# NilanEkanayake/TiTok-Video

Hardware: AMD Instinct MI355X
Metric: video clips/sec encode+decode (whole node) (higher is better)
Workload: dtype bf16

## Files before the change

include/titok_hip.h:

```cpp
#ifndef TITOK_HIP_H
#define TITOK_HIP_H

#include <stdint.h>

#ifdef __cplusplus
extern "C" {
#endif

#define TTV_OK 0
#define TTV_ERR_INVALID 1
#define TTV_ERR_LAUNCH 2
#define TTV_ERR_UNSUPPORTED 3

#define TTV_BF16 0
#define TTV_F32 1

#define TTV_ENCODER 0
#define TTV_DECODER 1

#define TTV_MAX_FSQ 8
#define TTV_MAX_TOKEN 64
#define TTV_MAX_CLIPS_PER_LAUNCH 64

const char* ttv_error_string(void);
// ... 143 lines not shown
typedef struct ttv_tower_weights {
  const void* proj_in_w;
  const void* proj_in_b;
  const float* mask_token;
  const float* ln_pre_t;
  const float* ln_pre_p;
  const float* ln_post;
  const void* proj_out_w;
  const void* proj_out_b;
  const ttv_layer_weights* layers;
  const void* proj_out_pn;
  int32_t f32_split3;
} ttv_tower_weights;

typedef struct ttv_batch {
  int32_t n_clips;
  int32_t total_rows;
  int32_t sum_tokens;
  int32_t sum_patches;
  int32_t max_patches_per_clip;
  int32_t n_qblocks;
  const int32_t* cu_seqlens;
  const int32_t* latent_rows;
  const int32_t* patch_rows;
  const int32_t* clip_desc;
  const int32_t* qblocks;
  const float* rope_cs;
  const int32_t* blocks64;
  const int32_t* row_seq;
  int32_t n_blocks64;
  int32_t qblocks_paired;
  int32_t qblocks_all_full;
  const int32_t* items64;
  int32_t n_items64;
  const int32_t* rope_ids;
  const float* rope_base;
  const int32_t* qblocks_latent;
  int32_t n_qblocks_latent;
  const int32_t* qblocks_patch;
  int32_t n_qblocks_patch;
} ttv_batch;

int ttv_rope_table_build(const float* base_cos, const float* base_sin, int n_ids, int n_freqs, const int32_t* clip_desc,
                         const int32_t* cu_seqlens, const int32_t* row_seq, float* rope_cs, int total_rows, void* stream);

int64_t ttv_tower_workspace_bytes(const ttv_tower_dims* dims, const ttv_batch* batch);

int ttv_encoder_forward(const ttv_tower_dims* dims, const ttv_tower_weights* w, const ttv_batch* batch,
                        const void* const* clips, const ttv_fsq_params* fsq, float* z, void* codes, int32_t* indices,
                        float* bounded, void* workspace, int64_t workspace_bytes, void* stream);

int ttv_decoder_forward(const ttv_tower_dims* dims, const ttv_tower_weights* w, const ttv_batch* batch, const void* codes,
                        void* const* clips_out, void* workspace, int64_t workspace_bytes, void* stream);

typedef struct ttv_layer_weights_t {
  const void* to_qkv_t;
  const void* out_proj_t;
  const void* w12_t;
  const void* w3_t;
} ttv_layer_weights_t;
typedef struct ttv_tower_weights_t {
  const void* proj_in_t;
  const void* proj_out_t;
  const ttv_layer_weights_t* layers;
} ttv_tower_weights_t;
typedef struct ttv_layer_grads {
  float* pre_ln; float* to_qkv; float* out_proj; float* ffd_norm; float* w12; float* w3; float* attn_post_ln; float* ffd_post_ln;
} ttv_layer_grads;
typedef struct ttv_tower_grads {
  float* proj_in_w; float* proj_in_b; float* mask_token; float* ln_pre_t; float* ln_pre_p; float* ln_post; float* proj_out_w;
  float* proj_out_b;
  const ttv_layer_grads* layers;
  void** layer_done_events;
} ttv_tower_grads;

int64_t ttv_tower_tape_bytes(const ttv_tower_dims* dims, const ttv_batch* batch);
int64_t ttv_tower_bwd_workspace_bytes(const ttv_tower_dims* dims, const ttv_batch* batch);
int ttv_encoder_forward_train(const ttv_tower_dims* dims, const ttv_tower_weights* w, const ttv_batch* batch, const void* const* clips,
                              float* z, void* tape, int64_t tape_bytes, void* stream);
int ttv_encoder_backward(const ttv_tower_dims* dims, const ttv_tower_weights* w, const ttv_tower_weights_t* wt, const ttv_batch* batch,
                         const float* dz, void* tape, const ttv_tower_grads* grads, void* const* dclips, void* workspace,
                         int64_t workspace_bytes, void* stream);
int ttv_decoder_forward_train(const ttv_tower_dims* dims, const ttv_tower_weights* w, const ttv_batch* batch, const void* codes,
                              void* const* clips_out, void* tape, int64_t tape_bytes, void* workspace, int64_t workspace_bytes,
                              void* stream);
int ttv_decoder_backward(const ttv_tower_dims* dims, const ttv_tower_weights* w, const ttv_tower_weights_t* wt, const ttv_batch* batch,
                         const void* codes, const void* const* dclips_out, void* tape, const ttv_tower_grads* grads, float* dcodes,
                         void* workspace, int64_t workspace_bytes, void* stream);
int ttv_fsq_backward(const ttv_fsq_params* p, const float* z, const void* dcodes, int dcodes_dtype, float* dz, int rows, void* stream);

int ttv_opt_grad_sumsq(const void* table, const int32_t* chunks, int n_chunks, int dtype, float* partials, void* stream);
int ttv_opt_adamw_step(const void* table, const int32_t* chunks, int n_chunks, int dtype, const float* partials, int n_partials, float lr,
                       float beta1, float beta2, float one_minus_beta1, float one_minus_beta2, float eps, float weight_decay,
                       float bias_correction1, float bias_correction2_sqrt, float max_norm, float* out_norm, void* stream);

int ttv_opt_param_norms(const void* table, const int32_t* chunks, int n_chunks, int n_entries, const float* partials, float* norms,
                        void* stream);

int ttv_opt_ema_update(const void* table, const int32_t* chunks, int n_chunks, int dtype, float weight, void* stream);
int ttv_opt_ema_exchange(const void* table, const int32_t* chunks, int n_chunks, int dtype, int mode, void* stream);

int64_t ttv_linear_wgrad_workspace_bytes(int L, int N, int K);
int ttv_linear_wgrad(const void* dy, int lddy, const void* x, int ldx, float* dw, int lddw, int L, int N, int K, int dtype,
                     void* workspace, int64_t workspace_bytes, void* stream);
int ttv_rmsnorm_backward_chain(const void* x, int ldx, const void* dy, int lddy, const float* gain1, float* dgain1, float* dx, int lddx,
                               const float* y, int ldy, const float* gain2, float* dgain2, float out_scale, void* cast_out, int ldc, int rows,
// ... 109 lines not shown
  const void* pool_proj_w; const void* pool_proj_b;
  const float* pool_norm2_w; const float* pool_norm2_b;
  const void* pool_fc1_w; const void* pool_fc1_b;
  const void* pool_fc2_w; const void* pool_fc2_b;
} ttv_vjepa_weights;

int ttv_jedi_preprocess(void* const* clips, const int32_t* dims, int n_clips, int dtype, void* out, void* stream);
int64_t ttv_vjepa_workspace_bytes(int n);
int ttv_vjepa_features(const ttv_vjepa_weights* w, const void* x, int n, float* feats, int finetuned, void* workspace,
                       int64_t workspace_bytes, void* stream);

#define TTV_VJEPA_EPI_STORE 0
#define TTV_VJEPA_EPI_GELU 1
#define TTV_VJEPA_EPI_RESID 2
int ttv_vjepa_layernorm(const float* x, int ldx, int rows, int width, const float* w1, const float* b1, float eps1, const float* w2,
                        const float* b2, float eps2, float* y32, int ld32, void* y16, int ld16, void* stream);
int ttv_vjepa_linear(const void* x, int ldx, const void* w, int ldw, const void* bias, int M, int N, int K, int epilogue,
                     const float* resid, int ldr, int resid_rows, void* y, int ldy, void* stream);
int ttv_vjepa_pool_attention(const void* q, const void* kv, int n, int rows, void* out, void* stream);

#define TTV_KC_ATTENTION 1
#define TTV_KC_GEMM_QKV 2
#define TTV_KC_GEMM_GEGLU 3
#define TTV_KC_GEMM_RESID 4
#define TTV_KC_GEMM_STORE 5
#define TTV_KC_RMSNORM 6
#define TTV_KC_PATCH 7
#define TTV_KC_ROWS 8
int ttv_prof_begin(int kernel_class, int max_records);
enum {
  TTV_DBG_NO_STORES = 1,
  TTV_DBG_K256_NO_PANEL_DMA = 2,
  TTV_DBG_MLP_NO_WEIGHT_DMA = 2,
  TTV_DBG_K256_NO_TILE_RELOAD = 4,
  TTV_DBG_MLP_NO_GEGLU = 4,
  TTV_DBG_K256_NO_EPILOGUE_MATH = 8,
  TTV_DBG_MLP_TILES8 = 8,
  TTV_DBG_MLP_NO_P2 = 16,
  TTV_DBG_MLP_PAIRS_ONLY = 32,
  TTV_DBG_MLP_TILES4 = 64,
  TTV_DBG_GEMM_TILE160 = 128,
  TTV_DBG_GEMM_TILE128 = 256,
  TTV_DBG_GEMM_T256 = 512,
  TTV_DBG_MLP_TILES9 = 512,
  TTV_DBG_GEMM_NO_T256 = 1024,
  TTV_DBG_MX_UNFUSED_QUANT = 2048,
  TTV_DBG_SPLIT3_NO_IMAGES = 4096,
  TTV_DBG_SPLIT3_NO_DMA = 8192,
  TTV_DBG_K256_GENERAL = 16384,
  TTV_DBG_QKV256_OFF = 32768,
  TTV_DBG_QKV256_WS = 131072,
  TTV_DBG_ENC_ALL_ROWS = 524288,
  TTV_DBG_ATTN_NO_SWP = 1048576,
  TTV_DBG_DEC_ALL_BLOCKS = 2097152
};
int ttv_debug_set(int flags);
int ttv_debug_stamps(void* device_buffer);
int ttv_prof_end(double* total_ms, int* count);

#ifdef __cplusplus
}
#endif
#endif
```

titok_video_amd/_lib.py:

```python
from __future__ import annotations

import ctypes as C
import os
import threading

import torch

from . import switches

TTV_BF16, TTV_F32 = 0, 1
TTV_ENCODER, TTV_DECODER = 0, 1
TTV_MAX_FSQ = 8
TTV_MAX_TOKEN = 64
TTV_MAX_CLIPS_PER_LAUNCH = 64
TTV_DISC_HEAD_GENERATOR, TTV_DISC_HEAD_DISCRIMINATOR = 0, 1

DBG_NO_STORES = 1
DBG_K256_NO_PANEL_DMA = 2
DBG_MLP_NO_WEIGHT_DMA = 2
DBG_K256_NO_TILE_RELOAD = 4
DBG_MLP_NO_GEGLU = 4
DBG_K256_NO_EPILOGUE_MATH = 8
DBG_MLP_TILES8 = 8
DBG_MLP_NO_P2 = 16
DBG_MLP_PAIRS_ONLY = 32
DBG_MLP_TILES4 = 64
DBG_GEMM_TILE160 = 128
DBG_GEMM_TILE128 = 256
DBG_GEMM_T256 = 512
DBG_MLP_TILES9 = 512
DBG_GEMM_NO_T256 = 1024
DBG_MX_UNFUSED_QUANT = 2048
DBG_SPLIT3_NO_IMAGES = 4096
DBG_SPLIT3_NO_DMA = 8192
DBG_K256_GENERAL = 16384
DBG_QKV256_OFF = 32768
DBG_QKV256_WS = 131072
DBG_ENC_ALL_ROWS = 524288
DBG_ATTN_NO_SWP = 1048576
DBG_DEC_ALL_BLOCKS = 2097152

_HERE = os.path.dirname(os.path.abspath(__file__))
LIB_PATH = switches.text("TTV_LIB_PATH") or os.path.join(_HERE, "libtitok_hip.so")

i32, i64, f32, vp = C.c_int32, C.c_int64, C.c_float, C.c_void_p


class FsqParams(C.Structure):
    _fields_ = [("n", i32), ("levels", i32 * TTV_MAX_FSQ), ("basis", i32 * TTV_MAX_FSQ),
                ("half_l", f32 * TTV_MAX_FSQ), ("offset", f32 * TTV_MAX_FSQ), ("shift", f32 * TTV_MAX_FSQ),
                ("half_width", f32 * TTV_MAX_FSQ)]


class TowerDims(C.Structure):
    _fields_ = [("kind", i32), ("dtype", i32), ("width", i32), ("layers", i32), ("q_heads", i32), ("kv_heads", i32),
                ("head_dim", i32), ("inner", i32), ("patch_t", i32), ("patch_h", i32), ("patch_w", i32),
                ("pix_channels", i32), ("token_size", i32), ("eps", f32), ("alpha", f32)]


class NextQkv(C.Structure):
    _fields_ = [("qkv", vp), ("ld", i32), ("rope_cs", vp), ("rows", i32), ("rope_q_end", i32), ("rope_k_begin", i32), ("rope_k_end", i32)]


class LayerWeights(C.Structure):
    _fields_ = [("pre_ln", vp), ("to_qkv", vp), ("out_proj", vp), ("ffd_norm", vp), ("w12", vp), ("w3", vp),
                ("attn_post_ln", vp), ("ffd_post_ln", vp), ("to_qkv_pn", vp), ("w12_pn", vp), ("mlp_pack", vp), ("mlp_pack_qkv_rows", i32), ("qkv_q_prescaled", i32),
                ("to_qkv_qs", vp), ("to_qkv_f8", vp), ("to_qkv_f8_scale", vp), ("w12_f8", vp), ("w12_f8_scale", vp),
                ("to_qkv_mx", vp), ("w12_mx", vp), ("out_proj_f8", vp), ("out_proj_f8_scale", vp), ("out_proj_mx", vp),
                ("w3_f8", vp), ("w3_f8_scale", vp), ("w3_mx", vp)]


class TowerWeights(C.Structure):
    _fields_ = [("proj_in_w", vp), ("proj_in_b", vp), ("mask_token", vp), ("ln_pre_t", vp), ("ln_pre_p", vp),
                ("ln_post", vp), ("proj_out_w", vp), ("proj_out_b", vp), ("layers", C.POINTER(LayerWeights)), ("proj_out_pn", vp),
                ("f32_split3", i32)]


class Batch(C.Structure):
    _fields_ = [("n_clips", i32), ("total_rows", i32), ("sum_tokens", i32), ("sum_patches", i32),
                ("max_patches_per_clip", i32), ("n_qblocks", i32), ("cu_seqlens", vp), ("latent_rows", vp),
                ("patch_rows", vp), ("clip_desc", vp), ("qblocks", vp), ("rope_cs", vp), ("blocks64", vp), ("row_seq", vp),
                ("n_blocks64", i32), ("qblocks_paired", i32), ("qblocks_all_full", i32), ("items64", vp), ("n_items64", i32),
                ("rope_ids", vp), ("rope_base", vp), ("qblocks_latent", vp), ("n_qblocks_latent", i32), ("qblocks_patch", vp),
                ("n_qblocks_patch", i32)]


class LayerWeightsT(C.Structure):
    _fields_ = [("to_qkv_t", vp), ("out_proj_t", vp), ("w12_t", vp), ("w3_t", vp)]


class TowerWeightsT(C.Structure):
    _fields_ = [("proj_in_t", vp), ("proj_out_t", vp), ("layers", C.POINTER(LayerWeightsT))]


class LayerGrads(C.Structure):
    _fields_ = [("pre_ln", vp), ("to_qkv", vp), ("out_proj", vp), ("ffd_norm", vp), ("w12", vp), ("w3", vp),
                ("attn_post_ln", vp), ("ffd_post_ln", vp)]


class TowerGrads(C.Structure):
    _fields_ = [("proj_in_w", vp), ("proj_in_b", vp), ("mask_token", vp), ("ln_pre_t", vp), ("ln_pre_p", vp), ("ln_post", vp),
                ("proj_out_w", vp), ("proj_out_b", vp), ("layers", C.POINTER(LayerGrads)), ("layer_done_events", C.POINTER(vp))]


class LpipsWeights(C.Structure):
    _fields_ = [("w", vp * 13), ("wd", vp * 13), ("b", vp * 13), ("lin", vp * 5)]


TTV_I3D_CONVS = 58
TTV_I3D_FEATURES = 400


class I3dWeights(C.Structure):
    _fields_ = [("w", vp * TTV_I3D_CONVS), ("scale", vp * TTV_I3D_CONVS), ("shift", vp * TTV_I3D_CONVS)]


TTV_VJEPA_WIDTH = 1024
TTV_VJEPA_TOKENS = 1568
TTV_VJEPA_PATCH_K = 1536
TTV_VJEPA_EPI_STORE, TTV_VJEPA_EPI_GELU, TTV_VJEPA_EPI_RESID = 0, 1, 2


class VjepaLayer(C.Structure):
    _fields_ = [("norm1_w", vp), ("norm1_b", vp), ("qkv_w", vp), ("qkv_b", vp), ("proj_w", vp), ("proj_b", vp), ("norm2_w", vp),
                ("norm2_b", vp), ("fc1_w", vp), ("fc1_b", vp), ("fc2_w", vp), ("fc2_b", vp)]


class VjepaWeights(C.Structure):
    _fields_ = [("width", i32), ("heads", i32), ("depth", i32), ("patch_w", vp), ("patch_b", vp), ("pos_embed", vp),
                ("layers", C.POINTER(VjepaLayer)), ("norm_w", vp), ("norm_b", vp), ("query_tokens", vp), ("pool_q", vp),
                ("pool_norm1_w", vp), ("pool_norm1_b", vp), ("pool_kv_w", vp), ("pool_kv_b", vp), ("pool_proj_w", vp),
                ("pool_proj_b", vp), ("pool_norm2_w", vp), ("pool_norm2_b", vp), ("pool_fc1_w", vp), ("pool_fc1_b", vp),
                ("pool_fc2_w", vp), ("pool_fc2_b", vp)]


_lib = None
_lock = threading.Lock()

SYMBOLS = {
    "ttv_error_string": (C.c_char_p, []),
    "ttv_version": (C.c_int, []),
    "ttv_fsq_forward": (C.c_int, [C.POINTER(FsqParams), vp, C.c_int, C.c_int, vp, C.c_int, vp, vp, vp]),
    "ttv_fsq_indices_to_codes": (C.c_int, [C.POINTER(FsqParams), vp, C.c_int, vp, C.c_int, vp]),
    "ttv_vq_codebook_norms": (C.c_int, [vp, C.c_int, C.c_int, C.c_int, C.c_int, vp, vp]),
    "ttv_vq_workspace_bytes": (C.c_int64, [C.c_int]),
    "ttv_vq_l2_argmin": (C.c_int, [vp, C.c_int, C.c_int, vp, C.c_int, vp, C.c_int, C.c_int, C.c_int, vp, vp, vp, C.c_int64, vp]),
    "ttv_vq_lookup": (C.c_int, [vp, C.c_int, C.c_int, vp, C.c_int, C.c_int, vp, C.c_int, vp]),
    "ttv_vq_lookup_backward": (C.c_int, [vp, C.c_int, C.c_int, vp, C.c_int, C.c_int, vp, C.c_int, vp]),
    "ttv_vq_train_workspace_bytes": (C.c_int64, [C.c_int, C.c_int]),
    "ttv_vq_commit_forward": (C.c_int, [vp, C.c_int, C.c_int, vp, C.c_int, vp, C.c_int, C.c_int, C.c_int, vp, vp, C.c_int64, vp]),
    "ttv_vq_commit_backward": (C.c_int, [vp, C.c_int, vp, C.c_int, vp, C.c_int, C.c_int, C.c_int, C.c_int, C.c_double, vp, C.c_int, vp]),
    "ttv_vq_ema_stats": (C.c_int, [vp, C.c_int, C.c_int, vp, C.c_int, C.c_int, C.c_int, vp, f32, C.c_uint64, vp, C.c_int, C.c_int, vp, vp, C.c_int64, vp]),
    "ttv_vq_ema_update": (C.c_int, [vp, vp, vp, vp, vp, C.c_int, vp, vp, C.c_int, C.c_int, f32, f32, f32, f32, vp, C.c_int64, vp]),
    "ttv_quant_rows_fp8": (C.c_int, [vp, C.c_int, C.c_int, vp, f32, vp, C.c_int, vp, C.c_int, C.c_int, vp]),
    "ttv_linear_fp8": (C.c_int, [vp, C.c_int, vp, vp, C.c_int, vp, vp, C.c_int, C.c_int, C.c_int, C.c_int, C.c_int, vp, C.c_int, C.c_int, vp]),
    "ttv_split3_pack": (C.c_int, [vp, C.c_int, vp, C.c_int, C.c_int, C.c_int, vp]),
    "ttv_linear_split3": (C.c_int, [vp, C.c_int, vp, C.c_int, vp, vp, C.c_int, C.c_int, C.c_int, C.c_int, vp]),
    "ttv_mx_scale_bytes_per_row": (C.c_int64, [C.c_int]),
    "ttv_quant_mx_fp8": (C.c_int, [vp, C.c_int, C.c_int, vp, C.c_int, vp, vp, C.c_int, C.c_int, vp]),
    "ttv_linear_fp8_mx": (C.c_int, [vp, C.c_int, vp, vp, vp, C.c_int, vp, vp, vp, C.c_int, C.c_int, C.c_int, C.c_int, C.c_int, vp, C.c_int, C.c_int,
                                    vp, C.c_int, f32, vp]),
    "ttv_rmsnorm": (C.c_int, [vp, C.c_int, C.c_int, vp, vp, C.c_int, C.c_int, vp, vp, C.c_int, C.c_int, f32, vp]),
    "ttv_rope_apply": (C.c_int, [vp, C.c_int, C.c_int, C.c_int, C.c_int, vp, vp]),
    "ttv_linear": (C.c_int, [vp, C.c_int, vp, C.c_int, vp, vp, vp, C.c_int, C.c_int, C.c_int, C.c_int, C.c_int, vp]),
    "ttv_linear_qkv_rope": (C.c_int, [vp, C.c_int, vp, C.c_int, vp, C.c_int, C.c_int, C.c_int, C.c_int, vp, C.c_int, vp]),
    "ttv_linear_geglu": (C.c_int, [vp, C.c_int, vp, C.c_int, vp, C.c_int, C.c_int, C.c_int, C.c_int, C.c_int, vp]),
    "ttv_linear_residual": (C.c_int, [vp, C.c_int, vp, C.c_int, vp, C.c_int, f32, vp, C.c_int, C.c_int, C.c_int, C.c_int,
                                      C.c_int, C.c_int, vp]),
    "ttv_linear_residual_norm": (C.c_int, [vp, C.c_int, vp, C.c_int, vp, C.c_int, f32, vp, f32, vp, C.c_int, C.c_int, C.c_int,
                                           C.c_int, C.c_int, vp]),
    "ttv_mlp_pack_bytes": (C.c_int64, [C.c_int, C.c_int]),
    "ttv_mlp_pack": (C.c_int, [vp, vp, vp, vp, C.c_int, C.c_int, C.c_int, C.c_int, vp, vp]),
    "ttv_layer_tail_fused": (C.c_int, [vp, C.c_int, vp, f32, vp, C.c_int, vp, C.c_int, vp, C.c_int, vp, f32, f32, C.c_int, C.c_int,
                                       C.c_int, vp, vp]),
    "ttv_mlp_fused": (C.c_int, [vp, C.c_int, vp, C.c_int, vp, C.c_int, vp, f32, f32, C.c_int, C.c_int, C.c_int, vp]),
    "ttv_fill_const_rows": (C.c_int, [vp, C.c_int, C.c_int, vp, C.c_int, C.c_int, vp, vp, f32, vp]),
    "ttv_decoder_embed": (C.c_int, [vp, C.c_int, vp, vp, vp, vp, vp, C.c_int, C.c_int, vp, C.c_int, C.c_int, f32, vp]),
    "ttv_attention": (C.c_int, [vp, C.c_int, vp, C.c_int, vp, vp, C.c_int, C.c_int, C.c_int, C.c_int, C.c_int, C.c_int, vp]),
    "ttv_attention64": (C.c_int, [vp, C.c_int, vp, C.c_int, vp, vp, C.c_int, C.c_int, C.c_int, C.c_int, C.c_int, C.c_int, vp]),
    "ttv_patch_gather": (C.c_int, [C.POINTER(vp), vp, C.c_int, C.c_int, C.c_int, C.c_int, C.c_int, C.c_int, vp, C.c_int,
                                   C.c_int, C.c_int, vp]),
    "ttv_patch_scatter": (C.c_int, [vp, C.c_int, vp, C.c_int, C.c_int, C.c_int, C.c_int, C.c_int, C.c_int, C.POINTER(vp),
                                    C.c_int, C.c_int, vp]),
    "ttv_tower_workspace_bytes": (i64, [C.POINTER(TowerDims), C.POINTER(Batch)]),
    "ttv_encoder_forward": (C.c_int, [C.POINTER(TowerDims), C.POINTER(TowerWeights), C.POINTER(Batch), C.POINTER(vp),
                                      C.POINTER(FsqParams), vp, vp, vp, vp, vp, i64, vp]),
    "ttv_decoder_forward": (C.c_int, [C.POINTER(TowerDims), C.POINTER(TowerWeights), C.POINTER(Batch), vp, C.POINTER(vp),
                                      vp, i64, vp]),
    "ttv_tower_tape_bytes": (i64, [C.POINTER(TowerDims), C.POINTER(Batch)]),
    "ttv_tower_bwd_workspace_bytes": (i64, [C.POINTER(TowerDims), C.POINTER(Batch)]),
    "ttv_encoder_forward_train": (C.c_int, [C.POINTER(TowerDims), C.POINTER(TowerWeights), C.POINTER(Batch), C.POINTER(vp), vp, vp,
                                            i64, vp]),
    "ttv_encoder_backward": (C.c_int, [C.POINTER(TowerDims), C.POINTER(TowerWeights), C.POINTER(TowerWeightsT), C.POINTER(Batch), vp,
                                       vp, C.POINTER(TowerGrads), C.POINTER(vp), vp, i64, vp]),
    "ttv_decoder_forward_train": (C.c_int, [C.POINTER(TowerDims), C.POINTER(TowerWeights), C.POINTER(Batch), vp, C.POINTER(vp), vp,
                                            i64, vp, i64, vp]),
    "ttv_decoder_backward": (C.c_int, [C.POINTER(TowerDims), C.POINTER(TowerWeights), C.POINTER(TowerWeightsT), C.POINTER(Batch), vp,
                                       C.POINTER(vp), vp, C.POINTER(TowerGrads), vp, vp, i64, vp]),
    "ttv_fsq_backward": (C.c_int, [C.POINTER(FsqParams), vp, vp, C.c_int, vp, C.c_int, vp]),
    "ttv_rmsnorm_backward_chain": (C.c_int, [vp, C.c_int, vp, C.c_int, vp, vp, vp, C.c_int, vp, C.c_int, vp, vp, C.c_float, vp, C.c_int,
                                              C.c_int, C.c_int, C.c_float, C.c_int, vp]),
    "ttv_opt_grad_sumsq": (C.c_int, [vp, vp, C.c_int, C.c_int, vp, vp]),
    "ttv_opt_adamw_step": (C.c_int, [vp, vp, C.c_int, C.c_int, vp, C.c_int] + [C.c_float] * 10 + [vp, vp]),
    "ttv_opt_param_norms": (C.c_int, [vp, vp, C.c_int, C.c_int, vp, vp, vp]),
    "ttv_opt_ema_update": (C.c_int, [vp, vp, C.c_int, C.c_int, C.c_float, vp]),
    "ttv_opt_ema_exchange": (C.c_int, [vp, vp, C.c_int, C.c_int, C.c_int, vp]),
    "ttv_linear_wgrad_workspace_bytes": (C.c_int64, [C.c_int, C.c_int, C.c_int]),
    "ttv_linear_wgrad": (C.c_int, [vp, C.c_int, vp, C.c_int, vp, C.c_int, C.c_int, C.c_int, C.c_int, C.c_int, vp, C.c_int64, vp]),
    "ttv_rmsnorm_backward": (C.c_int, [vp, C.c_int, vp, C.c_int, vp, vp, C.c_int, vp, C.c_int, C.c_int, f32, C.c_int, vp]),
    "ttv_attention_backward": (C.c_int, [vp, C.c_int, vp, C.c_int, vp, C.c_int, vp, vp, vp, vp, C.c_int, vp, vp, C.c_int, vp, C.c_int,
                                         C.c_int, C.c_int, C.c_int, vp, vp]),
    "ttv_attention_lse": (C.c_int, [vp, C.c_int, vp, C.c_int, vp, vp, C.c_int, C.c_int, C.c_int, C.c_int, C.c_int, C.c_int, vp, vp]),
    "ttv_codebook_histogram": (C.c_int, [vp, C.c_int, vp, C.c_int, vp]),
    "ttv_rope_table_build": (C.c_int, [vp, vp, C.c_int, C.c_int, vp, vp, vp, vp, C.c_int, vp]),
    "ttv_l1_loss": (C.c_int, [vp, vp, vp, vp, C.c_int, C.c_int, vp, vp]),
    "ttv_clip_from_u8": (C.c_int, [vp, C.c_int, C.c_int, C.c_int, vp, C.c_int, vp]),
    "ttv_clip_resample_u8": (C.c_int, [vp, vp, vp, C.c_int, C.c_int, vp]),
    "ttv_recon_panels_u8": (C.c_int, [vp, vp, vp, C.c_int, C.c_int, vp, vp]),
    "ttv_sq_err_accumulate": (C.c_int, [vp, vp, vp, C.c_int, C.c_int, C.c_int, vp, vp]),
    "ttv_ssim_workspace_bytes": (C.c_int64, [vp, C.c_int]),
    "ttv_ssim_accumulate": (C.c_int, [vp, vp, vp, C.c_int, C.c_int, C.c_int, vp, vp, C.c_int64, vp]),
    "ttv_lpips_tape_bytes": (C.c_int64, [C.c_int, C.c_int, C.c_int, C.c_int]),
    "ttv_lpips_workspace_bytes": (C.c_int64, [C.c_int, C.c_int, C.c_int, C.c_int]),
    "ttv_lpips_forward": (C.c_int, [C.POINTER(LpipsWeights), vp, vp, C.c_int, C.c_int, C.c_int, C.c_int, vp, vp, vp, vp, C.c_int64, vp]),
    "ttv_lpips_backward": (C.c_int, [C.POINTER(LpipsWeights), vp, C.c_int, C.c_int, C.c_int, C.c_int, vp, vp, vp, vp, C.c_int64, vp]),
    "ttv_lpips_eval_workspace_bytes": (C.c_int64, [C.c_int, C.c_int, C.c_int, C.c_int]),
    "ttv_lpips_eval_accumulate": (C.c_int, [C.POINTER(LpipsWeights), vp, vp, vp, C.c_int, C.c_int, C.c_int, C.c_int, C.c_int, vp, vp, vp,
                                            C.c_int64, vp]),
    "ttv_lpips_conv_workspace_bytes": (C.c_int64, [C.c_int] * 6),
    "ttv_lpips_conv3x3": (C.c_int, [vp, C.c_int, C.c_int, C.c_int, C.c_int, C.c_int, vp, vp, C.c_int, vp, vp, C.c_int, vp, C.c_int64, vp]),
    "ttv_lpips_maxpool": (C.c_int, [vp, C.c_int, C.c_int, C.c_int, C.c_int, vp, C.c_int, vp]),
    "ttv_lpips_maxpool_backward": (C.c_int, [vp, vp, vp, C.c_int, C.c_int, C.c_int, C.c_int, vp, C.c_int, vp]),
    "ttv_lpips_crops_forward": (C.c_int, [vp, vp, vp, C.c_int, vp, C.c_int, C.c_int, vp, vp, C.c_int, vp]),
    "ttv_lpips_crops_backward": (C.c_int, [vp, vp, vp, C.c_int, vp, C.c_int, C.c_int, vp, C.c_int, vp]),
    "ttv_gp_noise_add": (C.c_int, [vp, C.c_int, vp, C.c_int, C.c_int, C.c_uint64, C.c_uint64, f32, C.c_int, vp]),
    "ttv_disc_head": (C.c_int, [vp, vp, C.c_int, C.c_int, C.c_int, C.c_int, C.c_int, f32, f32, vp, vp, vp]),
    "ttv_i3d_workspace_bytes": (C.c_int64, [C.c_int]),
    "ttv_fvd_preprocess": (C.c_int, [vp, vp, C.c_int, C.c_int, C.c_int, vp, vp]),
    "ttv_i3d_features": (C.c_int, [C.POINTER(I3dWeights), vp, C.c_int, vp, vp, C.c_int64, vp]),
    "ttv_i3d_conv3d": (C.c_int, [vp] + [C.c_int] * 7 + [vp, vp, vp, C.c_int, C.c_int, vp, C.c_int, C.c_int, vp]),
    "ttv_i3d_maxpool3d": (C.c_int, [vp] + [C.c_int] * 11 + [vp, vp]),
# ... 66 lines not shown
```

titok_video_amd/csrc/ttv_api.hip:

```cpp
#include <stdarg.h>
#include <stdio.h>
#include <stdlib.h>
#include <string.h>

#include "ttv_common.h"
#include "ttv_kernels.h"

static thread_local char g_err[512] = "";

void ttv_set_error(const char* fmt, ...) {
  va_list ap;
  va_start(ap, fmt);
  vsnprintf(g_err, sizeof(g_err), fmt, ap);
  va_end(ap);
}

int g_ttv_prof_class = 0;
bool ttv_sw_enc_latent_last() { static const bool v = ttv_env_flag("TTV_ENC_LATENT_LAST", true); return v; }
bool ttv_enc_latent_rows_only(const ttv_tower_dims* d, const ttv_batch* b) {
  return ttv_sw_enc_latent_last() && !(g_ttv_debug & TTV_DBG_ENC_ALL_ROWS) && d->kind == TTV_ENCODER && b->latent_rows && b->sum_tokens > 0 &&
         b->sum_tokens < b->total_rows;
}
bool ttv_sw_keel_f32sum() { static const bool v = ttv_env_flag("TTV_KEEL_F32SUM", false); return v; }
bool ttv_sw_fused_patch() { static const bool v = ttv_env_flag("TTV_FUSED_PATCH", true); return v; }
bool ttv_sw_attn_pipe() { static const bool v = ttv_env_flag("TTV_ATTN_PIPE", false); return v; }
float ttv_sw_attn_thr() { static const float v = ttv_env_float("TTV_ATTN_THR", 8.0f); return v; }
thread_local int g_ttv_debug = 0;
long long* g_ttv_stamps = nullptr;
static hipEvent_t* g_prof_start = nullptr;
static hipEvent_t* g_prof_stop = nullptr;
static int g_prof_cap = 0, g_prof_n = 0;

TtvProfScope::TtvProfScope(int cls, hipStream_t stream) : slot(-1), s(stream) {
  if (g_ttv_prof_class != 0 && cls == g_ttv_prof_class && g_prof_n < g_prof_cap) {
    slot = g_prof_n++;
    (void)hipEventRecord(g_prof_start[slot], s);
  }
}
TtvProfScope::~TtvProfScope() {
  if (slot >= 0) (void)hipEventRecord(g_prof_stop[slot], s);
}

struct TowerWs {
  char *x, *xn, *qkv, *ao, *h, *pa, *pb;
  char *xl, *aol;
  char *f8, *f8mx;
  float* y32;
  float* rstd;
  int64_t total;
};

static TowerWs carve(const ttv_tower_dims* d, const ttv_batch* b, char* base) {
  const int64_t e = dtype_bytes(d->dtype);
  const int64_t L = b->total_rows, P = b->sum_patches;
  const int64_t g = (int64_t)d->kv_heads * d->head_dim;
  const int64_t pd = patch_dim(d);
  int64_t off = 0;
  TowerWs w;
  auto take = [&](int64_t bytes) { char* p = base ? base + off : nullptr; off += align256(bytes); return p; };
  w.x = take(L * d->width * e);
  w.xn = take(L * d->width * e);
  w.qkv = take(L * (2 * d->width + 2 * g) * e);
  w.ao = take(L * d->width * e);
  w.y32 = (float*)take(L * d->width * 4);
  w.h = take(L * d->inner * e);
  w.pa = take(P * pd * e);
  w.pb = take(P * d->width * e);
  w.rstd = (float*)take(L * 4);
  w.xl = take((int64_t)b->sum_tokens * d->width * e);
  w.aol = take((int64_t)b->sum_tokens * d->width * e);
  w.f8 = w.f8mx = nullptr;
  if (d->dtype == TTV_BF16 && d->width != 256 && d->width % 128 == 0) {
    const int64_t wide = d->width > d->inner ? d->width : d->inner;
    w.f8 = take(L * wide);
    w.f8mx = take(L * (wide / 128 + 4) * 4);
  }
  w.total = off;
  return w;
// ... 34 lines not shown
  const int L = b->total_rows, dm = d->width, g = d->kv_heads * d->head_dim, dt = d->dtype, nq = 2 * dm + 2 * g, I = d->inner;
  const float alpha = keel_alpha(d, i);
  static const bool fused_env = ttv_env_flag("TTV_MX_FUSED_QUANT", true);
  const bool fused_q = fused_env && !(g_ttv_debug & TTV_DBG_MX_UNFUSED_QUANT);
  if (!rstd_valid) TTV_TRY(ttvk_row_rstd(ws.x, dt, dm, ws.rstd, L, dm, d->eps, s));
  if (!xq_valid) TTV_TRY(ttvk_quant_mx_fp8(ws.x, dt, dm, ws.f8, dm, ws.f8mx, nullptr, L, dm, s));
  xq_valid = false;
  const GemmArgs a = gemm_rope_qk(gemm_args(dt, ws.f8, dm, lw.to_qkv_f8, dm, L, nq, dm, ws.qkv, nq), b->rope_cs, dm, g);
  TTV_TRY(ttvk_gemm_fp8(EPI_QKV_ROPE, a, ws.rstd, lw.to_qkv_f8_scale, s, ws.f8mx, lw.to_qkv_mx));
  const bool q_scaled = lw.qkv_q_prescaled != 0;
  if (fused_q && q_scaled && !c.pair && !c.pipe && d->head_dim == 64) {
    TTV_TRY(ttvk_attention_mxout(ws.qkv, nq, ws.f8, ws.f8mx, (int)ttvk_mx_scale_ld(dm), b->cu_seqlens, b->qblocks, b->n_qblocks, d->q_heads,
                                 d->kv_heads, s));
  } else {
    TTV_TRY(tower_attention(c, q_scaled, b->qblocks, b->n_qblocks, c.pair | (c.pipe ? c.all_full | c.pipe : 0)));
    TTV_TRY(ttvk_quant_mx_fp8(ws.ao, dt, dm, ws.f8, dm, ws.f8mx, nullptr, L, dm, s));
  }
  const GemmArgs o = gemm_resid(gemm_args(dt, ws.f8, dm, lw.out_proj_f8, dm, L, dm, dm, ws.x, dm), ws.x, dm, alpha);
  TTV_TRY(ttvk_gemm_fp8(EPI_RESID_T, o, nullptr, lw.out_proj_f8_scale, s, ws.f8mx, lw.out_proj_mx));
  if (i > 0) {
    TTV_TRY(ttvk_rmsnorm(ws.x, dt, dm, nullptr, ws.x, dt, dm, nullptr, lw.attn_post_ln, L, dm, d->eps, s, ws.rstd, fused_q ? ws.f8 : nullptr,
                         fused_q ? ws.f8mx : nullptr));
    if (!fused_q) TTV_TRY(ttvk_quant_mx_fp8(ws.x, dt, dm, ws.f8, dm, ws.f8mx, nullptr, L, dm, s));
  } else {
    TTV_TRY(ttvk_row_rstd(ws.x, dt, dm, ws.rstd, L, dm, d->eps, s));
    TTV_TRY(ttvk_quant_mx_fp8(ws.x, dt, dm, ws.f8, dm, ws.f8mx, nullptr, L, dm, s));
  }
  GemmArgs f = gemm_args(dt, ws.f8, dm, lw.w12_f8, dm, L, I, dm, ws.h, I);
  char* const hq = ws.h;
  char* const hq_mx = ws.xn;
  const bool h_fused = fused_q && (int64_t)ttvk_mx_scale_ld(I) <= (int64_t)dm * 2;
  if (h_fused) { f.yq = hq; f.yq_mx = hq_mx; }
  TTV_TRY(ttvk_gemm_fp8(EPI_GEGLU, f, ws.rstd, lw.w12_f8_scale, s, ws.f8mx, lw.w12_mx));
  if (!h_fused) TTV_TRY(ttvk_quant_mx_fp8(ws.h, dt, I, ws.f8, I, ws.f8mx, nullptr, L, I, s));
  const GemmArgs f3 = gemm_resid(gemm_args(dt, h_fused ? hq : ws.f8, I, lw.w3_f8, I, L, dm, I, ws.x, dm), ws.x, dm, alpha);
  TTV_TRY(ttvk_gemm_fp8(EPI_RESID_T, f3, nullptr, lw.w3_f8_scale, s, h_fused ? hq_mx : ws.f8mx, lw.w3_mx));
  rstd_valid = false;
  if (i > 0) {
    TTV_TRY(ttvk_rmsnorm(ws.x, dt, dm, nullptr, ws.x, dt, dm, nullptr, lw.ffd_post_ln, L, dm, d->eps, s, ws.rstd, fused_q ? ws.f8 : nullptr,
                         fused_q ? ws.f8mx : nullptr));
    rstd_valid = true;
    xq_valid = fused_q;
  }
  return TTV_OK;
}

static bool rows_f8(int dt, int dm, const void* img, const void* row_scale, const void* mx, const void* folded) {
  return dt == TTV_BF16 && img && row_scale && !mx && dm % 128 == 0 && !(dm == 256 && folded);
}

struct PreNormW { const float* gain; const void *w, *w_pn, *w_f8; const float* w_f8_scale; bool f8; };

static int prenorm_proj(const LayerCtx& c, GemmEpilogue epi, const char* x, int rows, const PreNormW& p, int N, char* y, int y_image,
                        bool rstd_valid) {
  const ttv_tower_dims* d = c.d;
  const TowerWs& ws = c.ws;
  const int dm = d->width, dt = d->dtype;
  GemmArgs a = gemm_args(dt, nullptr, dm, nullptr, dm, rows, N, dm, y, N);
  if (epi == EPI_QKV_ROPE) a = gemm_rope_qk(a, c.b->rope_cs, dm, d->kv_heads * d->head_dim);
  if (p.f8) {
    float* const f8_scales = reinterpret_cast<float*>(ws.xn + align256((int64_t)c.b->total_rows * dm));
    TTV_TRY(ttvk_quant_rows_fp8(x, dt, dm, p.gain, d->eps, ws.xn, dm, f8_scales, rows, dm, c.s));
    a.x = ws.xn; a.w = p.w_f8;
    return ttvk_gemm_fp8(epi, a, f8_scales, p.w_f8_scale, c.s);
  }
  const bool fold256 = dt == TTV_BF16 && dm == 256 && p.w_pn;
  const bool fold_gen = c.gen_ok && p.w_pn;
  const bool fold = fold256 || fold_gen;
  if (fold_gen && !rstd_valid) TTV_TRY(ttvk_row_rstd(x, dt, dm, ws.rstd, rows, dm, d->eps, c.s));
  if (!fold) TTV_TRY(ttvk_rmsnorm(x, dt, dm, nullptr, ws.xn, dt, dm, nullptr, p.gain, rows, dm, d->eps, c.s, nullptr, nullptr, nullptr, c.s3img));
  a.split3 = c.split3; a.x_image = c.s3img && !fold; a.y_image = y_image;
  a.prenorm = fold256; a.eps = d->eps;
  a.row_scale = fold_gen ? ws.rstd : nullptr;
  a.x = fold ? x : ws.xn; a.w = fold ? p.w_pn : p.w;
  if (epi == EPI_QKV_ROPE) { a.rope_ids = c.b->rope_ids; a.rope_base = c.b->rope_ids ? c.b->rope_base : nullptr; }
  return ttvk_gemm(epi, a, c.s);
}

static int keel_tail(const LayerCtx& c, GemmArgs o, int layer, const float* post_gain, bool want_rstd, bool& rstd_valid) {
  const ttv_tower_dims* d = c.d;
  const int dm = d->width, dt = d->dtype;
  char* const cx = (char*)o.y;
  o = gemm_resid(o, cx, dm, keel_alpha(d, layer));
  o.split3 = c.split3; o.x_image = c.s3img;
  if (layer == 0) return ttvk_gemm(EPI_RESID_T, o, c.s);
  if (ttvk_gemm_supports_resid_norm(dt, dm, o.K)) {
    o.norm_gain = post_gain; o.eps = d->eps;
    return ttvk_gemm(EPI_RESID_NORM, o, c.s);
  }
  float* const next_rstd = want_rstd ? c.ws.rstd : nullptr;
  if (dt == TTV_BF16 && !ttv_sw_keel_f32sum()) {
    TTV_TRY(ttvk_gemm(EPI_RESID_T, o, c.s));
    TTV_TRY(ttvk_rmsnorm(cx, dt, dm, nullptr, cx, dt, dm, nullptr, post_gain, o.M, dm, d->eps, c.s, next_rstd));
  } else {
    o.y = c.ws.y32;
    TTV_TRY(ttvk_gemm(EPI_RESID_F32, o, c.s));
    TTV_TRY(ttvk_rmsnorm(c.ws.y32, TTV_F32, dm, nullptr, cx, dt, dm, nullptr, post_gain, o.M, dm, d->eps, c.s, next_rstd));
  }
  rstd_valid = want_rstd;
  return TTV_OK;
}

static int run_layers(const ttv_tower_dims* d, const ttv_tower_weights* w, const ttv_batch* b, const TowerWs& ws, hipStream_t s) {
  const int L = b->total_rows, dm = d->width, g = d->kv_heads * d->head_dim, dt = d->dtype;
  const int split3 = (dt == TTV_F32 && w->f32_split3) ? 1 : 0;
  const bool gen_ok = (dt == TTV_BF16 && dm != 256) || split3;
  static const bool s3img_env = ttv_env_flag("TTV_SPLIT3_IMAGES", true);
  const int s3img = (split3 && s3img_env && !(g_ttv_debug & TTV_DBG_SPLIT3_NO_IMAGES)) ? 1 : 0;
  const int nq = 2 * dm + 2 * g;
  const int64_t row_bytes = (int64_t)dm * dtype_bytes(dt);
  bool qkv_ready = false;
  bool rstd_valid = false;
  bool xq_valid = false;
  const bool lat_last = ttv_enc_latent_rows_only(d, b) && b->qblocks_latent && b->n_qblocks_latent > 0;
  static const bool pat_env = ttv_env_flag("TTV_DEC_PATCH_LAST", true);
  const bool pat_last = pat_env && !(g_ttv_debug & TTV_DBG_DEC_ALL_BLOCKS) && d->kind == TTV_DECODER && d->layers >= 2 && b->qblocks_patch &&
                        b->n_qblocks_patch > 0 && !split3 && !b->qblocks_paired;
  bool compacted = false;
  const LayerCtx ctx = {d, b, ws, s, split3, s3img, gen_ok, b->qblocks_paired ? TTV_ATTN_PAIRED : 0, b->qblocks_all_full ? TTV_ATTN_ALLFULL : 0,
                        ttv_sw_attn_pipe() ? TTV_ATTN_PIPE : 0};
  for (int i = 0; i < d->layers; ++i) {
    const ttv_layer_weights& lw = w->layers[i];
    const bool last = i == d->layers - 1;
    if (dt == TTV_BF16 && dm != 256 && dm % 128 == 0 && d->inner % 128 == 0 && !ttv_sw_keel_f32sum() && lw.to_qkv_f8 && lw.to_qkv_mx && lw.w12_f8 &&
        lw.w12_mx && lw.out_proj_f8 && lw.out_proj_mx && lw.w3_f8 && lw.w3_mx &&
        !(lat_last && last)) {
      TTV_TRY(run_layer_mx(ctx, lw, i, rstd_valid, xq_valid));
      qkv_ready = false;
      continue;
    }
    xq_valid = false;
    const bool f8_qkv = rows_f8(dt, dm, lw.to_qkv_f8, lw.to_qkv_f8_scale, lw.to_qkv_mx, lw.to_qkv_pn);
    const bool f8_w12 = rows_f8(dt, dm, lw.w12_f8, lw.w12_f8_scale, lw.w12_mx, lw.w12_pn);
    if (!qkv_ready) {
      const void* w_plain = (dt == TTV_BF16 && lw.to_qkv_qs) ? lw.to_qkv_qs : lw.to_qkv;
      const PreNormW qw = {lw.pre_ln, w_plain, lw.to_qkv_pn, lw.to_qkv_f8, lw.to_qkv_f8_scale, f8_qkv};
      TTV_TRY(prenorm_proj(ctx, EPI_QKV_ROPE, ws.x, L, qw, nq, ws.qkv, s3img ? 2 : 0, rstd_valid));
    }
    const bool q_scaled = dt == TTV_BF16 && (lw.to_qkv_pn ? lw.qkv_q_prescaled != 0 : lw.to_qkv_qs != nullptr);
    rstd_valid = false;
    qkv_ready = false;
    const bool lat_now = lat_last && last;
    if (lat_now)
      TTV_TRY(tower_attention(ctx, q_scaled, b->qblocks_latent, b->n_qblocks_latent, ctx.all_full));
    else if (pat_last && last && dt == TTV_BF16 && !ctx.pipe)
      TTV_TRY(tower_attention(ctx, q_scaled, b->qblocks_patch, b->n_qblocks_patch, ctx.all_full));
    else if (q_scaled && b->items64 && b->n_items64 > 0 && d->head_dim == 64)
      TTV_TRY(ttvk_attention64(ws.qkv, nq, ws.ao, dm, b->cu_seqlens, b->items64, b->n_items64, d->q_heads, d->kv_heads,
                               TTV_ATTN_GATE | TTV_ATTN_QSCALED, s));
    else
      TTV_TRY(tower_attention(ctx, q_scaled, b->qblocks, b->n_qblocks, ctx.pair | ctx.all_full | ctx.pipe));
    char* cx = ws.x;
    char* cao = ws.ao;
    int Lc = L;
    if (lat_now) {
      TTV_TRY(gather_rows(ws.x, ws.xl, b->latent_rows, b->sum_tokens, row_bytes, s));
      TTV_TRY(gather_rows(ws.ao, ws.aol, b->latent_rows, b->sum_tokens, row_bytes, s));
      cx = ws.xl; cao = ws.aol; Lc = b->sum_tokens;
      compacted = true;
    }
    static const bool use_fused_mlp = ttv_env_flag("TTV_FUSED_MLP", true);
    static const bool use_fused_qkv = ttv_env_flag("TTV_FUSED_QKV", false);
    const float alpha = keel_alpha(d, i);
    if (use_fused_mlp && ttvk_mlp_fused_supported(dt, dm, d->inner) && lw.mlp_pack) {
      MlpNextQkv nx = {};
      const bool back = use_fused_qkv && !last && lw.mlp_pack_qkv_rows == nq && nq % 64 == 0 && dm % 64 == 0 && g % 64 == 0;
      if (back) { nx.qkv = ws.qkv; nx.ld = nq; nx.rope_cs = b->rope_cs; nx.rows = nq; nx.rope_q_end = dm; nx.rope_k_begin = 2 * dm; nx.rope_k_end = 2 * dm + g; }
      TTV_TRY(ttvk_mlp_fused(cao, dm, i == 0 ? nullptr : lw.attn_post_ln, alpha, cx, dm, lw.mlp_pack, d->inner, cx, dm, i == 0 ? nullptr : lw.ffd_post_ln,
                             alpha, d->eps, Lc, back ? &nx : nullptr, s));
      qkv_ready = back;
      continue;
    }
    TTV_TRY(keel_tail(ctx, gemm_args(dt, cao, dm, lw.out_proj, dm, Lc, dm, dm, cx, dm), i, lw.attn_post_ln, gen_ok && lw.w12_pn && !f8_w12, rstd_valid));
    const PreNormW fw = {lw.ffd_norm, lw.w12, lw.w12_pn, lw.w12_f8, lw.w12_f8_scale, f8_w12};
    TTV_TRY(prenorm_proj(ctx, EPI_GEGLU, cx, Lc, fw, d->inner, ws.h, s3img, rstd_valid));
    rstd_valid = false;
    const ttv_layer_weights* nl = last ? nullptr : &w->layers[i + 1];
    const bool next_rstd = gen_ok && nl && nl->to_qkv_pn && !rows_f8(dt, dm, nl->to_qkv_f8, nl->to_qkv_f8_scale, nl->to_qkv_mx, nl->to_qkv_pn);
    TTV_TRY(keel_tail(ctx, gemm_args(dt, ws.h, d->inner, lw.w3, d->inner, Lc, dm, d->inner, cx, dm), i, lw.ffd_post_ln, next_rstd, rstd_valid));
  }
  if (compacted)
    TTV_TRY(scatter_rows(ws.xl, ws.x, b->latent_rows, b->sum_tokens, row_bytes, s));
  return TTV_OK;
}

static bool fused_patch_ok(const ttv_tower_dims* d, const ttv_batch* b, int dt) {
  auto pow2 = [](int v) { return v > 0 && (v & (v - 1)) == 0; };
  return ttv_sw_fused_patch() && dt == TTV_BF16 && d->patch_w == 8 && pow2(d->patch_t) && pow2(d->patch_h) &&
         b->n_clips <= TTV_MAX_CLIPS_PER_LAUNCH && b->row_seq && patch_dim(d) % 64 == 0;
}

extern "C" {

const char* ttv_error_string(void) { return g_err; }
int ttv_version(void) { return 100; }

int ttv_fsq_forward(const ttv_fsq_params* p, const void* z, int z_dtype, int rows, void* codes, int codes_dtype, int32_t* indices,
                    float* bounded, void* stream) {
// ... 225 lines not shown
  TTV_CHECK_ARG(dtype == TTV_BF16 && head_dim == 64, "attention64: bf16, head_dim 64 only");
  return ttvk_attention64(qkvg, ld, out, ldo, cu_seqlens, items, n_items, q_heads, kv_heads, flags, (hipStream_t)stream);
}

int ttv_patch_gather(const void* const* clips, const int32_t* clip_desc, int clip0, int n_clips, int patch_t, int patch_h, int patch_w,
                     int channels, void* patches, int ld, int dtype, int max_patches_per_clip, void* stream) {
  TTV_CHECK_ARG(n_clips == 0 || (clips && clip_desc && patches), "patch_gather: null buffer");
  return ttvk_patch_copy(false, (void* const*)clips, clip_desc, clip0, n_clips, patch_t, patch_h, patch_w, channels, patches, ld, dtype, max_patches_per_clip, (hipStream_t)stream);
}

int ttv_patch_scatter(const void* patches, int ld, const int32_t* clip_desc, int clip0, int n_clips, int patch_t, int patch_h, int patch_w,
                      int channels, void* const* clips, int dtype, int max_patches_per_clip, void* stream) {
  TTV_CHECK_ARG(n_clips == 0 || (clips && clip_desc && patches), "patch_scatter: null buffer");
  return ttvk_patch_copy(true, clips, clip_desc, clip0, n_clips, patch_t, patch_h, patch_w, channels, (void*)patches, ld, dtype, max_patches_per_clip, (hipStream_t)stream);
}

int64_t ttv_tower_workspace_bytes(const ttv_tower_dims* dims, const ttv_batch* batch) {
  if (check_dims(dims, batch) != TTV_OK) return -1;
  return carve(dims, batch, nullptr).total;
}

int ttv_encoder_forward(const ttv_tower_dims* d, const ttv_tower_weights* w, const ttv_batch* b, const void* const* clips,
                        const ttv_fsq_params* fsq, float* z, void* codes, int32_t* indices, float* bounded, void* workspace,
                        int64_t workspace_bytes, void* stream) {
  TTV_TRY(check_dims(d, b));
  TTV_CHECK_ARG(d->kind == TTV_ENCODER, "encoder_forward: dims.kind is not TTV_ENCODER");
  TTV_CHECK_ARG(w && w->layers && clips && workspace, "encoder_forward: null argument");
  TTV_CHECK_ARG(fsq || z, "encoder_forward: neither fsq nor z requested");
  TTV_CHECK_ARG(!fsq || (codes && indices), "encoder_forward: fsq needs codes and indices buffers");
  hipStream_t s = (hipStream_t)stream;
  TowerWs ws = carve(d, b, (char*)workspace);
  TTV_CHECK_ARG(ws.total <= workspace_bytes, "encoder_forward: workspace too small (%lld < %lld)", (long long)workspace_bytes, (long long)ws.total);
  const int dm = d->width, dt = d->dtype, P = b->sum_patches, pd = patch_dim(d);

  const bool gather = fused_patch_ok(d, b, dt) && pd != 256;
  if (!gather) TTV_TRY(patch_copy_all(false, (void* const*)clips, d, b, ws.pa, dt, s));
  GemmArgs a = gemm_args(dt, ws.pa, pd, w->proj_in_w, pd, P, dm, pd, ws.pb, dm);
  a.bias = w->proj_in_b; a.add_scalar = w->mask_token;
  a.split3 = (dt == TTV_F32 && w->f32_split3) ? 1 : 0;
  if (gather) {
    a.gather = 1; a.clips = (void* const*)clips; a.n_clips = b->n_clips; a.clip_desc = b->clip_desc; a.patch_rows = b->patch_rows;
    a.row_seq = b->row_seq; a.patch_t = d->patch_t; a.patch_h = d->patch_h; a.patch_w = d->patch_w;
  }
  TTV_TRY(ttvk_gemm(EPI_STORE, a, s));
  TTV_TRY(ttvk_rmsnorm(ws.pb, dt, dm, nullptr, ws.x, dt, dm, b->patch_rows, w->ln_pre_p, P, dm, d->eps, s));
  TTV_TRY(ttvk_fill_const_rows(ws.x, dt, dm, b->latent_rows, b->sum_tokens, dm, w->mask_token, w->ln_pre_t, d->eps, s));

  TTV_TRY(run_layers(d, w, b, ws, s));

  TTV_TRY(ttvk_enc_tail(ws.x, dt, dm, b->latent_rows, b->sum_tokens, dm, w->ln_post, d->eps, w->proj_out_w, w->proj_out_b, d->token_size, fsq, z, codes, indices, bounded, s));
  return TTV_OK;
}

int ttv_decoder_forward(const ttv_tower_dims* d, const ttv_tower_weights* w, const ttv_batch* b, const void* codes,
                        void* const* clips_out, void* workspace, int64_t workspace_bytes, void* stream) {
  TTV_TRY(check_dims(d, b));
  TTV_CHECK_ARG(d->kind == TTV_DECODER, "decoder_forward: dims.kind is not TTV_DECODER");
  TTV_CHECK_ARG(w && w->layers && codes && clips_out && workspace, "decoder_forward: null argument");
  hipStream_t s = (hipStream_t)stream;
  TowerWs ws = carve(d, b, (char*)workspace);
  TTV_CHECK_ARG(ws.total <= workspace_bytes, "decoder_forward: workspace too small (%lld < %lld)", (long long)workspace_bytes, (long long)ws.total);
  const int dm = d->width, dt = d->dtype, P = b->sum_patches, pd = patch_dim(d);

  TTV_TRY(ttvk_dec_embed(codes, d->token_size, w->proj_in_w, w->proj_in_b, w->mask_token, w->ln_pre_t, ws.x, dt, dm, b->latent_rows, b->sum_tokens, dm, d->eps, s));
  TTV_TRY(ttvk_fill_const_rows(ws.x, dt, dm, b->patch_rows, P, dm, w->mask_token, w->ln_pre_p, d->eps, s));

  TTV_TRY(run_layers(d, w, b, ws, s));

  GemmArgs a = gemm_args(dt, nullptr, dm, w->proj_out_w, dm, P, pd, dm, ws.pa, pd);
  a.split3 = (dt == TTV_F32 && w->f32_split3) ? 1 : 0;
  a.bias = w->proj_out_b;
  if (dt == TTV_BF16 && dm == 256 && w->proj_out_pn && pd % 8 == 0) {
    a.x = ws.x; a.x_rows = b->patch_rows; a.w = w->proj_out_pn; a.prenorm = 1; a.eps = d->eps;
  } else {
    TTV_TRY(ttvk_rmsnorm(ws.x, dt, dm, b->patch_rows, ws.pb, dt, dm, nullptr, w->ln_post, P, dm, d->eps, s));
    a.x = ws.pb;
  }
  if (fused_patch_ok(d, b, dt) && dm == 256) {
    a.clips = clips_out; a.n_clips = b->n_clips; a.clip_desc = b->clip_desc; a.patch_rows = b->patch_rows; a.row_seq = b->row_seq;
    a.patch_t = d->patch_t; a.patch_h = d->patch_h; a.patch_w = d->patch_w;
    return ttvk_gemm(EPI_STORE_PATCH, a, s);
  }
  TTV_TRY(ttvk_gemm(EPI_STORE, a, s));
  return patch_copy_all(true, clips_out, d, b, ws.pa, dt, s);
}

int ttv_rope_table_build(const float* base_cos, const float* base_sin, int n_ids, int n_freqs, const int32_t* clip_desc, const int32_t* cu_seqlens,
                         const int32_t* row_seq, float* rope_cs, int total_rows, void* stream) {
  TTV_CHECK_ARG(total_rows == 0 || (base_cos && base_sin && clip_desc && cu_seqlens && row_seq && rope_cs), "rope_table_build: null buffer");
  TTV_CHECK_ARG(n_freqs >= 1 && 3 * n_freqs <= 32 && n_ids >= 1, "rope_table_build: bad table shape");
  return ttvk_rope_build(base_cos, base_sin, n_ids, n_freqs, clip_desc, cu_seqlens, row_seq, rope_cs, total_rows, (hipStream_t)stream);
}

int ttv_l1_loss(void* const* recon, void* const* target, void* const* grad, const int32_t* sizes, int n_clips, int dtype, float* loss,
                void* stream) {
  return for_clip_groups(n_clips, [&](int c0, int n) {
    return ttvk_l1_loss(recon + c0, target + c0, grad ? grad + c0 : nullptr, sizes + c0, n, n_clips, dtype, loss, (hipStream_t)stream);
  });
}

int ttv_clip_from_u8(const void* frames_thwc, int T, int H, int W, void* clip_cthw, int dtype, void* stream) {
  TTV_CHECK_ARG(frames_thwc && clip_cthw && T > 0 && H > 0 && W > 0, "clip_from_u8: bad argument");
  return ttvk_clip_from_u8(frames_thwc, (long long)T * H * W, clip_cthw, dtype, (hipStream_t)stream);
}

int ttv_clip_resample_u8(void* const* frames_thwc, void* const* clips_cthw, const int32_t* geom, int n_clips, int dtype, void* stream) {
  return ttvk_clip_resample_u8(frames_thwc, clips_cthw, geom, n_clips, dtype, (hipStream_t)stream);
}

int ttv_sq_err_accumulate(void* const* recon, void* const* target, const int32_t* sizes, int n_clips, int dtype, int clamp, double* acc,
                          void* stream) {
  return for_clip_groups(n_clips, [&](int c0, int n) { return ttvk_sq_err(recon + c0, target + c0, sizes + c0, n, dtype, clamp, acc, (hipStream_t)stream); });
}

int64_t ttv_ssim_workspace_bytes(const int32_t* dims, int n_clips) { return ttvk_ssim_workspace_bytes(dims, n_clips); }

int ttv_ssim_accumulate(void* const* recon, void* const* target, const int32_t* dims, int n_clips, int dtype, int clamp, double* acc,
                        void* workspace, int64_t workspace_bytes, void* stream) {
  return ttvk_ssim(recon, target, dims, n_clips, dtype, clamp, acc, workspace, workspace_bytes, (hipStream_t)stream);
}
// ... 156 lines not shown
```

titok_video_amd/csrc/ttv_attn.hip:

```cpp
#include <stdlib.h>

#include "ttv_common.h"
#include "ttv_kernels.h"

#define QB 128
#define KB 64
#ifndef ATTN_LAZY
#define ATTN_LAZY 1
#endif
#ifndef ATTN_DMA_LATE
#define ATTN_DMA_LATE 1
#endif
#ifndef ATTN_PRIO
#define ATTN_PRIO 0
#endif
#define ATTN_LAZY_LOG2 30
#define ATTN_LAZY_BIG 1073741824.0f
typedef float f32x2 __attribute__((ext_vector_type(2)));

typedef __attribute__((address_space(3))) bf16x4 lds_bf16x4;

__device__ __forceinline__ bf16x4 lds_read_tr16(const char* lds_ptr) {
  return __builtin_amdgcn_ds_read_tr16_b64_v4bf16((lds_bf16x4*)(lds_ptr));
}
// ... 1293 lines not shown
      }
#undef S3_VFRAG
    }
  }
#undef S3_GLOAD
#undef S3_LSTORE
#undef S3_DMA_TILE
#undef S3_DMA
  if (!wave_live) return;

  const float l_tot = l_run + __shfl_xor(l_run, 32, 64);
  const float inv_l = 1.0f / l_tot;
  if (qrow < q_lim) {
    float* orow = out + (size_t)(s0 + qrow) * ldo + head * 64;
    const float* grow = gbase + (size_t)qrow * ld;
#pragma unroll
    for (int dt = 0; dt < 2; ++dt)
#pragma unroll
      for (int g = 0; g < 4; ++g) {
        const int d0 = dt * 32 + 8 * g + 4 * h;
        f32x4 v = {o_acc[dt][4 * g] * inv_l, o_acc[dt][4 * g + 1] * inv_l, o_acc[dt][4 * g + 2] * inv_l, o_acc[dt][4 * g + 3] * inv_l};
        if (GATE) {
          const f32x4 gt = *reinterpret_cast<const f32x4*>(grow + d0);
#pragma unroll
          for (int e = 0; e < 4; ++e) v[e] *= 1.0f / (1.0f + expf(-gt[e]));
        }
        if (out_image) {
          uint2 hi, lo;
          split4_f32(__builtin_bit_cast(uint4, v), hi, lo);
          *reinterpret_cast<uint4*>(orow + d0) = make_uint4(hi.x, hi.y, lo.x, lo.y);
        } else {
          *reinterpret_cast<f32x4*>(orow + d0) = v;
        }
      }
  }
}

int ttvk_attention_mxout(const void* qkvg, int ld, void* out_q, void* out_mx, int ld_mx, const int* cu_seqlens, const int* qblocks,
                         int n_qblocks, int q_heads, int kv_heads, hipStream_t s) {
  if (n_qblocks == 0) return TTV_OK;
  TTV_CHECK_ARG(kv_heads > 0 && q_heads % kv_heads == 0, "attention_mxout: q_heads %% kv_heads");
  const int d_model = q_heads * 64, gqa = kv_heads * 64, rep = q_heads / kv_heads;
  TTV_CHECK_ARG(ld >= 2 * d_model + 2 * gqa && ld % 8 == 0 && d_model % 128 == 0 && ld_mx == (int)(4 * ((d_model / 128 + 3) / 4 * 4)),
                "attention_mxout: bad leading dims (d_model %% 128, ld_mx = 4 * round_up(d_model / 128, 4))");
  TTV_CHECK_ARG(qkvg && out_q && out_mx && (uintptr_t)qkvg % 16 == 0 && (uintptr_t)out_q % 8 == 0, "attention_mxout: null / unaligned pointers");
  static const float defer_thr = ttv_sw_attn_thr();
  TtvProfScope prof(TTV_KC_ATTENTION, s);
  hipLaunchKernelGGL((k_attn_bf16<true, 1, true, false, true>), dim3(n_qblocks), dim3(256), 0, s, (const bf16_t*)qkvg, ld, (bf16_t*)nullptr, ld_mx,
                     cu_seqlens, qblocks, n_qblocks, d_model, gqa, rep, 1.0f, (float*)out_mx, (bf16_t*)out_q, defer_thr, g_ttv_stamps);
  TTV_CHECK_LAUNCH("attention_mxout");
  return TTV_OK;
}

int ttvk_attention(const void* qkvg, int ld, void* out, int ldo, const int* cu_seqlens, const int* qblocks, int n_qblocks,
                   int q_heads, int kv_heads, int head_dim, int flags, int dtype, hipStream_t s, float* lse_out, void* out_raw) {
  const int gate_mul = flags & 1, paired = (flags >> 1) & 1, prescaled = (flags >> 2) & 1;
  TTV_CHECK_ARG(!prescaled || dtype == TTV_BF16, "attention: pre-scaled q is a bf16 path option");
  TTV_CHECK_ARG(!out_raw || (dtype == TTV_BF16 && gate_mul), "attention: the second (ungated) output is a bf16 + gate option");
  if (n_qblocks == 0) return TTV_OK;
  TTV_CHECK_ARG(head_dim == 64, "attention: head_dim %d unsupported (the reference fixes 64, utils.py:8)", head_dim);
  TTV_CHECK_ARG(kv_heads > 0 && q_heads % kv_heads == 0, "attention: q_heads %% kv_heads");
  const int d_model = q_heads * 64, gqa = kv_heads * 64, rep = q_heads / kv_heads;
  TTV_CHECK_ARG(ld >= 2 * d_model + 2 * gqa && ld % 8 == 0 && ldo % 4 == 0, "attention: bad leading dims");
  TTV_CHECK_ARG((uintptr_t)qkvg % 16 == 0 && (uintptr_t)out % (dtype == TTV_F32 ? 16 : 8) == 0, "attention: unaligned pointers");
  dim3 grid(n_qblocks);
  const float scale = 0.125f;
  TtvProfScope prof(TTV_KC_ATTENTION, s);
  if (dtype == TTV_BF16) {
    const float c_exp = scale * 1.44269504088896340736f;
    const float c_eff = prescaled ? 1.0f : c_exp;
    static const float defer_thr = ttv_sw_attn_thr();
#define ATTN_LAUNCH(G_, NE_, P_, T_, grid_, threads_)                                                                                   \
  hipLaunchKernelGGL((k_attn_bf16<G_, NE_, (P_) && (NE_) == 1, T_>), grid_, dim3(threads_), 0, s, (const bf16_t*)qkvg, ld, (bf16_t*)out, ldo, \
                     cu_seqlens, qblocks, n_qblocks, d_model, gqa, rep, c_eff, lse_out, (bf16_t*)out_raw, defer_thr, g_ttv_stamps)
#define ATTN_PICK(NE_, grid_, threads_)                                                  \
  do {                                                                                   \
    if (tape) { if (gate_mul) ATTN_LAUNCH(true, NE_, false, true, grid_, threads_); else ATTN_LAUNCH(false, NE_, false, true, grid_, threads_); }  \
    else if (gate_mul) { if (prescaled) ATTN_LAUNCH(true, NE_, true, false, grid_, threads_); else ATTN_LAUNCH(true, NE_, false, false, grid_, threads_); }   \
    else { if (prescaled) ATTN_LAUNCH(false, NE_, true, false, grid_, threads_); else ATTN_LAUNCH(false, NE_, false, false, grid_, threads_); }          \
  } while (0)
    const bool tape = lse_out != nullptr || out_raw != nullptr;
    TTV_CHECK_ARG(!tape || !prescaled, "attention: the training-tape outputs need unscaled q");
    static const bool swp_env = ttv_env_flag("TTV_ATTN_SWP", true);
    if (swp_env && !(flags & TTV_ATTN_PIPE) && (flags & TTV_ATTN_ALLFULL) && prescaled && !paired && !tape && !(g_ttv_debug & TTV_DBG_ATTN_NO_SWP)) {
      return ttvk_attention_swp(qkvg, ld, out, ldo, cu_seqlens, qblocks, n_qblocks, q_heads, kv_heads, gate_mul, s);
    }
    if ((flags & TTV_ATTN_PIPE) && (flags & TTV_ATTN_ALLFULL) && prescaled && !paired && !tape) {
      static const float pipe_thr = ttv_env_float("TTV_ATTN_PIPE_THR", ATTN_PIPE_THR);
      if (gate_mul) hipLaunchKernelGGL((k_attn_pipe<true>), grid, dim3(256), 0, s, (const bf16_t*)qkvg, ld, (bf16_t*)out, ldo, cu_seqlens, qblocks, d_model, gqa, rep, pipe_thr, g_ttv_stamps);
      else hipLaunchKernelGGL((k_attn_pipe<false>), grid, dim3(256), 0, s, (const bf16_t*)qkvg, ld, (bf16_t*)out, ldo, cu_seqlens, qblocks, d_model, gqa, rep, pipe_thr, g_ttv_stamps);
    } else if (paired) {
      const int rows = ttv_cdiv(n_qblocks, 8), pairs = ttv_cdiv(rows, 2);
      dim3 g2(pairs * 8);
      ATTN_PICK(2, g2, 512);
    } else {
      ATTN_PICK(1, grid, 256);
    }
#undef ATTN_PICK
#undef ATTN_LAUNCH
  } else if (dtype == TTV_F32) {
    const float c_exp = scale * 1.44269504088896340736f;
    if (flags & TTV_ATTN_SPLIT3) {
      TTV_CHECK_ARG(!lse_out, "attention: the split-bf16 kernel is an inference path (no tape outputs)");
      const int img = (flags & TTV_ATTN_SPLIT_OUT) ? 1 : 0;
      if (flags & TTV_ATTN_SPLIT_IN) {
        if (gate_mul) hipLaunchKernelGGL((k_attn_split3<true, true>), grid, dim3(256), 0, s, (const float*)qkvg, ld, (float*)out, ldo, cu_seqlens, qblocks, d_model, gqa, rep, c_exp, img);
        else hipLaunchKernelGGL((k_attn_split3<false, true>), grid, dim3(256), 0, s, (const float*)qkvg, ld, (float*)out, ldo, cu_seqlens, qblocks, d_model, gqa, rep, c_exp, img);
      } else if (gate_mul) hipLaunchKernelGGL((k_attn_split3<true>), grid, dim3(256), 0, s, (const float*)qkvg, ld, (float*)out, ldo, cu_seqlens, qblocks, d_model, gqa, rep, c_exp, img);
      else hipLaunchKernelGGL((k_attn_split3<false>), grid, dim3(256), 0, s, (const float*)qkvg, ld, (float*)out, ldo, cu_seqlens, qblocks, d_model, gqa, rep, c_exp, img);
    } else if (gate_mul)
      hipLaunchKernelGGL((k_attn_f32<true>), grid, dim3(256), 0, s, (const float*)qkvg, ld, (float*)out, ldo, cu_seqlens, qblocks, d_model, gqa, rep, c_exp, lse_out);
    else
      hipLaunchKernelGGL((k_attn_f32<false>), grid, dim3(256), 0, s, (const float*)qkvg, ld, (float*)out, ldo, cu_seqlens, qblocks, d_model, gqa, rep, c_exp, lse_out);
  } else {
    ttv_set_error("attention: bad dtype");
    return TTV_ERR_INVALID;
  }
  TTV_CHECK_LAUNCH("attention");
  return TTV_OK;
}
```

titok_video_amd/csrc/ttv_attn_swp.hip:

```cpp
#include <stdlib.h>

#include "ttv_common.h"
#include "ttv_kernels.h"

#define SWP_KB 64
#define SWP_NS 3
#ifndef SWP_OCC
#define SWP_OCC 3
#endif

typedef __attribute__((address_space(3))) bf16x4 swp_lds_bf16x4;
__device__ __forceinline__ bf16x4 swp_read_tr16(const char* lds_ptr) {
  return __builtin_amdgcn_ds_read_tr16_b64_v4bf16((swp_lds_bf16x4*)(lds_ptr));
}

#ifdef SWP_STAMPS
#define SWP_STAMP_DECL unsigned long long st_prev__ = 0, st_acc__[6] = {0, 0, 0, 0, 0, 0}
#define SWP_STAMP_START()                                                                              \
  do {                                                                                                 \
    __builtin_amdgcn_sched_barrier(0);                                                                 \
    asm volatile("s_memtime %0\n\ts_waitcnt lgkmcnt(0)" : "=s"(st_prev__)::"memory");                  \
    __builtin_amdgcn_sched_barrier(0);                                                                 \
  } while (0)
#define SWP_STAMP(seg_)                                                                                \
  do {                                                                                                 \
    unsigned long long t__;                                                                            \
    __builtin_amdgcn_sched_barrier(0);                                                                 \
    asm volatile("s_memtime %0\n\ts_waitcnt lgkmcnt(0)" : "=s"(t__)::"memory");                        \
    __builtin_amdgcn_sched_barrier(0);                                                                 \
    st_acc__[seg_] += t__ - st_prev__;                                                                 \
    st_prev__ = t__;                                                                                   \
  } while (0)
#else
#define SWP_STAMP_DECL
#define SWP_STAMP_START()
#define SWP_STAMP(seg_)
#endif

template <bool GATE>
__global__ __launch_bounds__(256, SWP_OCC) void k_attn_swp(const bf16_t* __restrict__ qkvg, int ld, bf16_t* __restrict__ out, int ldo,
                                                     const int* __restrict__ cu, const int* __restrict__ qblocks, int d_model, int gqa,
                                                     int rep, long long* __restrict__ stamps) {
  __shared__ __attribute__((aligned(16))) uint4 kl[SWP_NS][SWP_KB * 8];
  __shared__ __attribute__((aligned(16))) uint4 vl[SWP_NS][SWP_KB * 8];

#ifdef SWP_STAMPS
  unsigned long long st_entry__;
  asm volatile("s_memtime %0\n\ts_waitcnt lgkmcnt(0)" : "=s"(st_entry__)::"memory");
#endif
  const int tid = threadIdx.x, lane = tid & 63;
  const int wave = __builtin_amdgcn_readfirstlane(tid >> 6);
  const int r = lane & 31, h = lane >> 5;
  const int tix = blockIdx.x;
  const int seq = qblocks[4 * tix], q0 = qblocks[4 * tix + 1], head = qblocks[4 * tix + 2];
  if (seq < 0) return;
  const int s0 = cu[seq], S = cu[seq + 1] - s0;
  const int kvh = head / rep;
  const bf16_t* qbase = qkvg + (size_t)s0 * ld + head * 64;
  const bf16_t* gbase = qkvg + (size_t)s0 * ld + d_model + head * 64;
  const bf16_t* kbase = qkvg + (size_t)s0 * ld + 2 * d_model + kvh * 64;
  const bf16_t* vbase = kbase + gqa;
  const int nkt = (S + SWP_KB - 1) / SWP_KB;

  const uint32_t kl_lds = (uint32_t)(uintptr_t)(__attribute__((address_space(3))) void*)&kl[0][0];
  const uint32_t vl_lds = (uint32_t)(uintptr_t)(__attribute__((address_space(3))) void*)&vl[0][0];
  const int drow = wave * 8 + (lane >> 3);
  const int kc = ((lane & 7) ^ ((drow >> 1) & 7)) * 8;
  const int vc = ((lane & 7) ^ (((drow >> 1) & 1) << 2)) * 8;
  const uint32_t dK = (uint32_t)(drow * ld + kc) * 2u;
  const uint32_t dV = (uint32_t)(drow * ld + vc) * 2u;
#define SWP_DMA16(voff_, base_, dst_)                                                                            \
  do {                                                                                                           \
    unsigned keep__;                                                                                             \
    asm volatile("s_mov_b32 %0, m0\n\ts_mov_b32 m0, %3\n\ts_nop 0\n\tglobal_load_lds_dwordx4 %1, %2\n\ts_mov_b32 m0, %0" \
                 : "=&s"(keep__) : "v"(voff_), "s"(base_), "s"(dst_) : "memory");                                 \
  } while (0)
#define SWP_DMA_TILE(base_, lds_, kt_, slot_, d_, c_)                                                            \
  do {                                                                                                           \
    const int key0__ = (kt_) * SWP_KB;                                                                           \
    if (key0__ >= S) break;                                                                                      \
    const bf16_t* b__ = (base_) + (size_t)key0__ * ld;                                                           \
    const uint32_t dst__ = (lds_) + (slot_) * (SWP_KB * 128) + wave * 1024;                                      \
    if (key0__ + SWP_KB <= S) {                                                                                  \
      const bf16_t* b32__ = b__ + (size_t)32 * ld;                                                               \
      unsigned keep__;                                                                                           \
      asm volatile("s_mov_b32 %0, m0\n\ts_mov_b32 m0, %4\n\ts_nop 0\n\tglobal_load_lds_dwordx4 %1, %2\n\t"         \
                   "s_add_u32 m0, %4, 0x1000\n\ts_nop 0\n\tglobal_load_lds_dwordx4 %1, %3\n\ts_mov_b32 m0, %0"      \
                   : "=&s"(keep__) : "v"(d_), "s"(b__), "s"(b32__), "s"(dst__) : "memory", "scc");                   \
    } else {                                                                                                     \
      const int lim__ = S - 1 - key0__;                                                                          \
      const int g0__ = drow < lim__ ? drow : lim__, g1__ = drow + 32 < lim__ ? drow + 32 : lim__;                \
      SWP_DMA16((uint32_t)(g0__ * ld + (c_)) * 2u, b__, dst__);                                                  \
      SWP_DMA16((uint32_t)(g1__ * ld + (c_)) * 2u, b__, dst__ + 4096);                                           \
    }                                                                                                            \
  } while (0)
#define SWP_DMA_K(kt_, slot_) SWP_DMA_TILE(kbase, kl_lds, kt_, slot_, dK, kc)
#define SWP_DMA_V(kt_, slot_) SWP_DMA_TILE(vbase, vl_lds, kt_, slot_, dV, vc)

  SWP_DMA_K(0, 0);
  SWP_DMA_V(0, 0);
  SWP_DMA_K(1, 1);
  SWP_DMA_K(2, 2);
  SWP_DMA_V(1, 1);
  const int qrow = q0 + wave * 32 + r;
  const int qrc = qrow < S ? qrow : S - 1;
  bf16x8 qf[4];
#pragma unroll
  for (int ks = 0; ks < 4; ++ks) qf[ks] = *reinterpret_cast<const bf16x8*>(qbase + (size_t)qrc * ld + ks * 16 + h * 8);

  const int ksw = (r >> 1) & 7;
  const char* const kbase_lds = reinterpret_cast<const char*>(&kl[0][0]);
  const char* const vbase_lds = reinterpret_cast<const char*>(&vl[0][0]);
  const char* const ka0 = kbase_lds + r * 128 + (((0 * 2 + h) ^ ksw) << 4);
  const char* const ka1 = kbase_lds + r * 128 + (((1 * 2 + h) ^ ksw) << 4);
  const char* const ka2 = kbase_lds + r * 128 + (((2 * 2 + h) ^ ksw) << 4);
  const char* const ka3 = kbase_lds + r * 128 + (((3 * 2 + h) ^ ksw) << 4);
  const int gi = lane & 15, tq = gi >> 2, tp = gi & 3, g16 = (lane >> 4) & 1;
  const int vsw = (tq >> 1) & 1;
  const int vlane = (4 * h + tq) * 128 + (g16 * 2 + (tp >> 1)) * 16 + (tp & 1) * 8;
  const char* const va0 = vbase_lds + vlane + (vsw ? 64 : 0);
  const char* const va1 = vbase_lds + vlane + (vsw ? 0 : 64);
  const f32x16 zero16 = {0.f, 0.f, 0.f, 0.f, 0.f, 0.f, 0.f, 0.f, 0.f, 0.f, 0.f, 0.f, 0.f, 0.f, 0.f, 0.f};

  f32x16 o0 = zero16, o1 = zero16;
  float l_run = 0.f;
  f32x16 sA0, sA1, sB0, sB1;
  bf16x8 kf00, kf01, kf02, kf03, kf10, kf11, kf12, kf13;
  bf16x8 vf00, vf01, vf02, vf03, vf10, vf11, vf12, vf13;
  bf16x8 pa0, pa1, pa2, pa3, pb0, pb1, pb2, pb3;
  float sum_a, sum_b;

#define SWP_LOADK_H(J_, so_)                                                                                     \
  do {                                                                                                           \
    if ((J_) == 0) {                                                                                             \
      kf00 = *reinterpret_cast<const bf16x8*>(ka0 + (so_));                                                      \
      kf01 = *reinterpret_cast<const bf16x8*>(ka1 + (so_));                                                      \
      kf02 = *reinterpret_cast<const bf16x8*>(ka2 + (so_));                                                      \
      kf03 = *reinterpret_cast<const bf16x8*>(ka3 + (so_));                                                      \
    } else {                                                                                                     \
      kf10 = *reinterpret_cast<const bf16x8*>(ka0 + (so_) + 4096);                                               \
      kf11 = *reinterpret_cast<const bf16x8*>(ka1 + (so_) + 4096);                                               \
      kf12 = *reinterpret_cast<const bf16x8*>(ka2 + (so_) + 4096);                                               \
      kf13 = *reinterpret_cast<const bf16x8*>(ka3 + (so_) + 4096);                                               \
    }                                                                                                            \
  } while (0)
#define SWP_VFRAG(va_, OFF_)                                                                                     \
  ({                                                                                                             \
    const bf16x4 lo__ = swp_read_tr16((va_) + (OFF_)), hi__ = swp_read_tr16((va_) + (OFF_) + 1024);              \
    (bf16x8){lo__[0], lo__[1], lo__[2], lo__[3], hi__[0], hi__[1], hi__[2], hi__[3]};                            \
  })
#define SWP_LOADV_H(J_, so_)                                                                                     \
  do {                                                                                                           \
    if ((J_) == 0) {                                                                                             \
      vf00 = SWP_VFRAG(va0, (so_));        vf10 = SWP_VFRAG(va1, (so_));                                         \
      vf01 = SWP_VFRAG(va0, (so_) + 2048); vf11 = SWP_VFRAG(va1, (so_) + 2048);                                  \
    } else {                                                                                                     \
      vf02 = SWP_VFRAG(va0, (so_) + 4096); vf12 = SWP_VFRAG(va1, (so_) + 4096);                                  \
      vf03 = SWP_VFRAG(va0, (so_) + 6144); vf13 = SWP_VFRAG(va1, (so_) + 6144);                                  \
    }                                                                                                            \
  } while (0)
#define SWP_EXP8(s_, Q_, f_, FIRST_)                                                                             \
  do {                                                                                                           \
    float p__[8];                                                                                                \
    _Pragma("unroll") for (int e__ = 0; e__ < 8; ++e__) p__[e__] = __builtin_amdgcn_exp2f(s_[8 * (Q_) + e__]);   \
    if (FIRST_) { sum_a = p__[0]; sum_b = p__[1]; } else { sum_a += p__[0]; sum_b += p__[1]; }                   \
    _Pragma("unroll") for (int e__ = 2; e__ < 8; e__ += 2) { sum_a += p__[e__]; sum_b += p__[e__ + 1]; }         \
    f_ = (bf16x8){(bf16_t)p__[0], (bf16_t)p__[1], (bf16_t)p__[2], (bf16_t)p__[3], (bf16_t)p__[4], (bf16_t)p__[5],  \
                  (bf16_t)p__[6], (bf16_t)p__[7]};                                                               \
     \
    asm volatile("" : "+v"(f_), "+v"(sum_a), "+v"(sum_b));                                                       \
  } while (0)
#define SWP_MASK(c0_, c1_, kt_)                                                                                  \
  do {                                                                                                           \
    if ((kt_) == nkt - 1 && nkt * SWP_KB > S) {                                                                  \
      int h4__ = 4 * h;                                                                                          \
      asm volatile("" : "+v"(h4__));       \
      _Pragma("unroll") for (int e__ = 0; e__ < 16; ++e__) {                                                     \
        const int key__ = (kt_) * SWP_KB + (e__ & 3) + 8 * (e__ >> 2) + h4__;                                    \
        if (key__ >= S) c0_[e__] = -INFINITY;                                                                    \
        if (key__ + 32 >= S) c1_[e__] = -INFINITY;                                                               \
      }                                                                                                          \
    }                                                                                                            \
  } while (0)
#define SWP_SCORES_H(d_, k0_, k1_, k2_, k3_)                                                                     \
  do {                                                                                                           \
    d_ = __builtin_amdgcn_mfma_f32_32x32x16_bf16(k0_, qf[0], zero16, 0, 0, 0);                                   \
    d_ = __builtin_amdgcn_mfma_f32_32x32x16_bf16(k1_, qf[1], d_, 0, 0, 0);                                       \
    d_ = __builtin_amdgcn_mfma_f32_32x32x16_bf16(k2_, qf[2], d_, 0, 0, 0);                                       \
    d_ = __builtin_amdgcn_mfma_f32_32x32x16_bf16(k3_, qf[3], d_, 0, 0, 0);                                       \
  } while (0)
#define SWP_PV_H(va_, vb_, vc_, vd_, f0_, f1_)                                                                   \
  do {                                                                                                           \
    o0 = __builtin_amdgcn_mfma_f32_32x32x16_bf16(va_, f0_, o0, 0, 0, 0);                                         \
    o1 = __builtin_amdgcn_mfma_f32_32x32x16_bf16(vb_, f0_, o1, 0, 0, 0);                                         \
    o0 = __builtin_amdgcn_mfma_f32_32x32x16_bf16(vc_, f1_, o0, 0, 0, 0);                                         \
    o1 = __builtin_amdgcn_mfma_f32_32x32x16_bf16(vd_, f1_, o1, 0, 0, 0);                                         \
  } while (0)
#define SWP_GAPS4(NDS_)                                                                                          \
  do {                                                                                                           \
    _Pragma("unroll") for (int i__ = 0; i__ < 4; ++i__) {                                                        \
      __builtin_amdgcn_sched_group_barrier(0x008, 1, 0);                                                         \
      __builtin_amdgcn_sched_group_barrier(0x100, NDS_, 0);                                                      \
      __builtin_amdgcn_sched_group_barrier(0x400, 2, 0);                                                         \
      __builtin_amdgcn_sched_group_barrier(0x002, 3, 0);                                                         \
    }                                                                                                            \
    __builtin_amdgcn_sched_barrier(0);                                                                           \
  } while (0)

#define SWP_TOP(t_)                                                                                              \
  do {                                                                                                           \
    if ((t_) + 3 < nkt) asm volatile("s_waitcnt vmcnt(4) lgkmcnt(0)" ::: "memory");                              \
    else if ((t_) + 1 < nkt) asm volatile("s_waitcnt vmcnt(2) lgkmcnt(0)" ::: "memory");                         \
    else asm volatile("s_waitcnt vmcnt(0) lgkmcnt(0)" ::: "memory");                                             \
    SWP_STAMP(0);                                                                                                \
    asm volatile("s_barrier" ::: "memory");       \
    SWP_STAMP(1);                                                                                                \
  } while (0)

#define SWP_ITER(t_, so0_, so1_, so2_, cur1_, nxt0_, nxt1_, pc0_, pc1_, pc2_, pc3_, pn0_, pn1_)                  \
  do {                                                                                                           \
    const int tt__ = (t_);                                                                                       \
    SWP_TOP(tt__);                                                                                               \
          \
    SWP_LOADV_H(0, so0_);                                                                                        \
    SWP_SCORES_H(nxt0_, kf00, kf01, kf02, kf03);                                                                 \
    SWP_EXP8(cur1_, 0, pc2_, false);                                                                             \
    SWP_GAPS4(2);                                                                                                \
    SWP_DMA_V(tt__ + 2, (so2_) >> 13);                                                                           \
    __builtin_amdgcn_sched_barrier(0);                                                                           \
    SWP_LOADV_H(1, so0_);                                                                                        \
    SWP_SCORES_H(nxt1_, kf10, kf11, kf12, kf13);                                                                 \
    SWP_EXP8(cur1_, 1, pc3_, false);                                                                             \
    SWP_GAPS4(2);                                                                                                \
    SWP_STAMP(2);                                                                                                \
    l_run += sum_a + sum_b;                                                                                      \
    if (tt__ + 1 == nkt - 1 && nkt * SWP_KB > S) {                                                               \
      asm volatile("s_nop 7\n\ts_nop 7\n\ts_nop 3" ::: "memory");      \
      SWP_MASK(nxt0_, nxt1_, tt__ + 1);                                                                          \
    }                                                                                                            \
    SWP_STAMP(3);                                                                                                \
     \
    SWP_LOADK_H(0, so2_);                                                                                        \
    SWP_PV_H(vf00, vf10, vf01, vf11, pc0_, pc1_);                                                                \
    SWP_EXP8(nxt0_, 0, pn0_, true);                                                                              \
    SWP_GAPS4(1);                                                                                                \
    SWP_DMA_K(tt__ + 4, (so1_) >> 13);                                                                           \
    __builtin_amdgcn_sched_barrier(0);                                                                           \
    SWP_LOADK_H(1, so2_);                                                                                        \
    SWP_PV_H(vf02, vf12, vf03, vf13, pc2_, pc3_);                                                                \
    SWP_EXP8(nxt0_, 1, pn1_, false);                                                                             \
    SWP_GAPS4(1);                                                                                                \
    SWP_STAMP(4);                                                                                                \
  } while (0)

  __builtin_amdgcn_s_waitcnt(0x0F70);
  __syncthreads();
  SWP_LOADK_H(0, 0);
  SWP_LOADK_H(1, 0);
  SWP_SCORES_H(sA0, kf00, kf01, kf02, kf03);
  SWP_SCORES_H(sA1, kf10, kf11, kf12, kf13);
  SWP_MASK(sA0, sA1, 0);
  __syncthreads();
  SWP_DMA_K(3, 0);
  SWP_LOADK_H(0, SWP_KB * 128);
  SWP_LOADK_H(1, SWP_KB * 128);
  SWP_EXP8(sA0, 0, pa0, true);
  SWP_EXP8(sA0, 1, pa1, false);
  SWP_STAMP_DECL;
  SWP_STAMP_START();
#ifdef SWP_STAMPS
  const unsigned long long st_loop_start__ = st_prev__;
  unsigned long long st_real0__;
  asm volatile("s_memrealtime %0\n\ts_waitcnt lgkmcnt(0)" : "=s"(st_real0__)::"memory");
#endif

#define SWP_LAST(t_, so0_, cur1_, pc0_, pc1_, pc2_, pc3_)                                                        \
  do {                                                                                                           \
    SWP_TOP(t_);                                                                                                 \
    SWP_LOADV_H(0, so0_);                                                                                        \
    SWP_PV_H(vf00, vf10, vf01, vf11, pc0_, pc1_);                                                                \
    SWP_EXP8(cur1_, 0, pc2_, false);                                                                             \
    SWP_GAPS4(2);                                                                                                \
    SWP_LOADV_H(1, so0_);                                                                                        \
    SWP_EXP8(cur1_, 1, pc3_, false);                                                                             \
    __builtin_amdgcn_sched_barrier(0);                                                                           \
    SWP_STAMP(2);                                                                                                \
    l_run += sum_a + sum_b;                                                                                      \
    SWP_PV_H(vf02, vf12, vf03, vf13, pc2_, pc3_);                                                                \
    SWP_STAMP(4);                                                                                                \
  } while (0)

  {
    int t = 0;
    int so0 = 0, so1 = SWP_KB * 128, so2 = 2 * SWP_KB * 128;
    for (;;) {
      if (t == nkt - 1) break;
      SWP_ITER(t, so0, so1, so2, sA1, sB0, sB1, pa0, pa1, pa2, pa3, pb0, pb1);
      ++t;
      if (t == nkt - 1) {
        sA1 = sB1; pa0 = pb0; pa1 = pb1; so0 = so1;
        break;
      }
      SWP_ITER(t, so1, so2, so0, sB1, sA0, sA1, pb0, pb1, pb2, pb3, pa0, pa1);
      ++t;
      const int so = so0;
      so0 = so2;
      so2 = so1;
      so1 = so;
    }
    SWP_LAST(t, so0, sA1, pa0, pa1, pa2, pa3);
  }
#ifdef SWP_STAMPS
  const unsigned long long st_loop_end__ = st_prev__;
  unsigned long long st_real1__;
  asm volatile("s_memrealtime %0\n\ts_waitcnt lgkmcnt(0)" : "=s"(st_real1__)::"memory");
  st_acc__[5] = st_real1__ - st_real0__;
#endif

  float l_tot = l_run + __shfl_xor(l_run, 32, 64);
  const bool out_of_range = !(l_tot > 8.6736174e-19f && l_tot < 1.1529215e18f);
  if (__syncthreads_or(out_of_range)) {
    float m_run = -INFINITY;
    l_run = 0.f;
    o0 = zero16;
    o1 = zero16;
    for (int kt = 0; kt < nkt; ++kt) {
      __syncthreads();
      SWP_DMA_K(kt, 0);
      SWP_DMA_V(kt, 0);
      __builtin_amdgcn_s_waitcnt(0x0F70);
      __syncthreads();
      SWP_LOADK_H(0, 0);
      SWP_LOADK_H(1, 0);
      SWP_SCORES_H(sA0, kf00, kf01, kf02, kf03);
      SWP_SCORES_H(sA1, kf10, kf11, kf12, kf13);
      SWP_MASK(sA0, sA1, kt);
      float mx = fmaxf(sA0[0], sA1[0]);
#pragma unroll
      for (int e = 1; e < 16; ++e) mx = fmaxf(mx, fmaxf(sA0[e], sA1[e]));
      mx = fmaxf(mx, __shfl_xor(mx, 32, 64));
      const float m_new = fmaxf(m_run, mx);
      const float alpha = __builtin_amdgcn_exp2f(m_run - m_new);
      float ps = 0.f;
#pragma unroll
      for (int e = 0; e < 16; ++e) {
        sA0[e] = __builtin_amdgcn_exp2f(sA0[e] - m_new);
        sA1[e] = __builtin_amdgcn_exp2f(sA1[e] - m_new);
        ps += sA0[e] + sA1[e];
        o0[e] *= alpha;
        o1[e] *= alpha;
      }
      l_run = l_run * alpha + ps;
      m_run = m_new;
#define SWP_PACKS(c_, Q_)                                                                                         \
  ((bf16x8){(bf16_t)c_[8 * Q_ + 0], (bf16_t)c_[8 * Q_ + 1], (bf16_t)c_[8 * Q_ + 2], (bf16_t)c_[8 * Q_ + 3], (bf16_t)c_[8 * Q_ + 4], \
            (bf16_t)c_[8 * Q_ + 5], (bf16_t)c_[8 * Q_ + 6], (bf16_t)c_[8 * Q_ + 7]})
      pa0 = SWP_PACKS(sA0, 0); pa1 = SWP_PACKS(sA0, 1); pa2 = SWP_PACKS(sA1, 0); pa3 = SWP_PACKS(sA1, 1);
#undef SWP_PACKS
      SWP_LOADV_H(0, 0);
      SWP_LOADV_H(1, 0);
      SWP_PV_H(vf00, vf10, vf01, vf11, pa0, pa1);
      SWP_PV_H(vf02, vf12, vf03, vf13, pa2, pa3);
    }
    l_tot = l_run + __shfl_xor(l_run, 32, 64);
  }

  const float inv_l = __builtin_amdgcn_rcpf(l_tot);
  {
    bf16_t* orow = out + (size_t)(s0 + qrc) * ldo + head * 64;
    const bf16_t* grow = gbase + (size_t)qrc * ld;
    const bool store = qrow < S;
#pragma unroll
    for (int dt = 0; dt < 2; ++dt)
#pragma unroll
      for (int gp = 0; gp < 2; ++gp) {
        uint2 pk[2];
#pragma unroll
        for (int gg = 0; gg < 2; ++gg) {
          const int g = 2 * gp + gg;
          const int d0 = dt * 32 + 8 * g + 4 * h;
          const f32x16& oa = dt ? o1 : o0;
          f32x4 v = {oa[4 * g] * inv_l, oa[4 * g + 1] * inv_l, oa[4 * g + 2] * inv_l, oa[4 * g + 3] * inv_l};
          if (GATE) {
            const f32x4 gt = Vec4<bf16_t>::load(grow + d0);
#pragma unroll
            for (int e = 0; e < 4; ++e) v[e] *= __builtin_amdgcn_rcpf(1.0f + __builtin_amdgcn_exp2f(gt[e] * -1.44269504088896340736f));
          }
          const bf16x4 b4 = {(bf16_t)v[0], (bf16_t)v[1], (bf16_t)v[2], (bf16_t)v[3]};
          pk[gg] = __builtin_bit_cast(uint2, b4);
        }
        const auto sx = __builtin_amdgcn_permlane32_swap(pk[0].x, pk[1].x, false, false);
        const auto sy = __builtin_amdgcn_permlane32_swap(pk[0].y, pk[1].y, false, false);
        const uint4 o16 = {sx[0], sy[0], sx[1], sy[1]};
        if (store) *reinterpret_cast<uint4*>(orow + dt * 32 + 16 * gp + 8 * h) = o16;
      }
  }
#ifdef SWP_STAMPS
  if (stamps && blockIdx.x % 37 == 0 && lane == 0) {
    unsigned long long st_end__;
    asm volatile("s_waitcnt vmcnt(0)\n\ts_memtime %0\n\ts_waitcnt lgkmcnt(0)" : "=s"(st_end__)::"memory");
    long long* dst = stamps + ((size_t)(blockIdx.x / 37) * 4 + wave) * 8;
    for (int i = 0; i < 6; ++i) dst[i] = (long long)st_acc__[i];
    dst[6] = (long long)(st_loop_start__ - st_entry__);
    dst[7] = (long long)(st_end__ - st_loop_end__);
  }
#endif
}

int ttvk_attention_swp(const void* qkvg, int ld, void* out, int ldo, const int* cu_seqlens, const int* qblocks, int n_qblocks,
                       int q_heads, int kv_heads, int gate_mul, hipStream_t s) {
  const int d_model = q_heads * 64, gqa = kv_heads * 64, rep = q_heads / kv_heads;
  dim3 grid(n_qblocks);
  if (gate_mul)
    hipLaunchKernelGGL((k_attn_swp<true>), grid, dim3(256), 0, s, (const bf16_t*)qkvg, ld, (bf16_t*)out, ldo, cu_seqlens, qblocks, d_model,
                       gqa, rep, g_ttv_stamps);
  else
    hipLaunchKernelGGL((k_attn_swp<false>), grid, dim3(256), 0, s, (const bf16_t*)qkvg, ld, (bf16_t*)out, ldo, cu_seqlens, qblocks, d_model,
                       gqa, rep, g_ttv_stamps);
  TTV_CHECK_LAUNCH("attention_swp");
  return TTV_OK;
}
```

titok_video_amd/csrc/ttv_gemm.hip:

```cpp
#include <stdlib.h>

#include "ttv_common.h"
#include "ttv_kernels.h"

struct GemmDev {
  const void* x; const void* w; void* y;
  const void* bias; const float* add_scalar; const void* resid; const float* rope_cs;
  int ldx, ldw, ldy, ldr;
  int M, N, K;
  int w_rows;
  float alpha;
  int rope_q_end, rope_k_begin, rope_k_end;
  float eps;
  int debug;
  const float* norm_gain;
  ClipPtrs clips;
  const int* clip_desc; const int* patch_rows; const int* row_seq;
  const int* x_rows;
  const float* row_scale;
  const int* rope_ids; const float* rope_base;
  const float* x_scale; const float* w_scale;
  float* sum_f32; int ld_sum;
  void* y2; int ldy2; const float* norm_gain2;
  int split3;
  int x_image, y_image;
  const uint8_t* x_mx; const uint8_t* w_mx;
  int ld_mx;
  uint8_t* yq; uint8_t* yq_mx; int ld_yq_mx, yq_nkp;
  int clip0, pt_shift, ph_shift;
  long long* stamps;
  int resid_rows;
};

struct PatchDst {
  bf16_t* base;
  int thw, hw, w;
};

__device__ __forceinline__ float gelu_erf(float v) { return 0.5f * v * (1.0f + erff(v * 0.70710678118654752440f)); }
__device__ __forceinline__ float gelu_erf_as(float v) {
  const float x = fabsf(v) * 0.70710678118654752440f;
  const float t = __builtin_amdgcn_rcpf(fmaf(0.3275911f, x, 1.0f));
  const float poly = t * fmaf(t, fmaf(t, fmaf(t, fmaf(t, 1.061405429f, -1.453152027f), 1.421413741f), -0.284496736f), 0.254829592f);
  const float e = __builtin_amdgcn_exp2f(x * x * -1.44269504088896340736f);
  const float erf_abs = fmaf(-poly, e, 1.0f);
  return 0.5f * v * (1.0f + __builtin_copysignf(erf_abs, v));
}

__device__ __forceinline__ uint2 pack_bf16x4(f32x4 v) {
  bf16x4 b = {(bf16_t)v[0], (bf16_t)v[1], (bf16_t)v[2], (bf16_t)v[3]};
  return __builtin_bit_cast(uint2, b);
}

__device__ __forceinline__ uint4 split4_bf16(uint4 v) {
  const float x0 = __uint_as_float(v.x), x1 = __uint_as_float(v.y), x2 = __uint_as_float(v.z), x3 = __uint_as_float(v.w);
  const bf16_t h0 = (bf16_t)x0, h1 = (bf16_t)x1, h2 = (bf16_t)x2, h3 = (bf16_t)x3;
  const bf16_t l0 = (bf16_t)(x0 - (float)h0), l1 = (bf16_t)(x1 - (float)h1), l2 = (bf16_t)(x2 - (float)h2), l3 = (bf16_t)(x3 - (float)h3);
  const bf16x4 hv = {h0, h1, h2, h3}, lv = {l0, l1, l2, l3};
  const uint2 hp = __builtin_bit_cast(uint2, hv), lp = __builtin_bit_cast(uint2, lv);
  return make_uint4(hp.x, hp.y, lp.x, lp.y);
}

template <int EPI, typename T, int NI, int NJ>
__device__ __forceinline__ void epilogue_tile(const GemmDev& p, const int (&tok)[NJ], const int (&feat)[NI],
                                              f32x4 (&acc)[NI][NJ], f32x4 (&acc2)[NI][NJ], int kq, const PatchDst* pd = nullptr) {
  if (p.debug & TTV_DBG_NO_STORES) {
#pragma unroll
    for (int i = 0; i < NI; ++i)
#pragma unroll
      for (int j = 0; j < NJ; ++j) asm volatile("" ::"v"(acc[i][j][0]), "v"(acc[i][j][3]), "v"(acc2[i][j][1]));
    return;
  }
  int tc[NJ], fc[NI];
  bool tv[NJ], fv[NI];
#pragma unroll
  for (int j = 0; j < NJ; ++j) { tv[j] = tok[j] < p.M; tc[j] = tv[j] ? tok[j] : p.M - 1; }
#pragma unroll
  for (int i = 0; i < NI; ++i) { fv[i] = feat[i] < p.N; fc[i] = fv[i] ? feat[i] : p.N - 4; }

  if (p.row_scale) {
#pragma unroll
    for (int j = 0; j < NJ; ++j) {
      const float rs = p.row_scale[tc[j]];
#pragma unroll
// ... 1709 lines not shown
        const int kc = kb * 4 + kq;
#pragma unroll
        for (int i = 0; i < 4; ++i) {
          const int arow = (DUAL ? (i < 2 ? wf * 32 + i * 16 : 64 + wf * 32 + (i - 2) * 16) : wf * 64 + i * 16) + l15;
          a[i] = __builtin_bit_cast(f32x4, lds[buf][arow * 8 + (kc ^ ((arow >> 1) & 7))]);
        }
#pragma unroll
        for (int j = 0; j < NJ; ++j) {
          const int brow = wt * (16 * NJ) + j * 16 + l15;
          b[j] = __builtin_bit_cast(f32x4, lds[buf][TF * 8 + brow * 8 + (kc ^ ((brow >> 1) & 7))]);
        }
#pragma unroll
        for (int jj = 0; jj < 4; ++jj)
#pragma unroll
          for (int i = 0; i < 4; ++i)
#pragma unroll
            for (int j = 0; j < NJ; ++j) acc[i][j] = __builtin_amdgcn_mfma_f32_16x16x4f32(a[i][jj], b[j][jj], acc[i][j], 0, 0, 0);
      }
    }
    __builtin_amdgcn_s_waitcnt(0x0F70);
    __syncthreads();
  }
#undef GS_STAGE
#undef GS_DMA

  int tok[NJ];
#pragma unroll
  for (int j = 0; j < NJ; ++j) tok[j] = tbase + wt * (16 * NJ) + j * 16 + l15;
  if (DUAL) {
    int feat[2];
    f32x4 ax[2][NJ], ag[2][NJ];
#pragma unroll
    for (int i = 0; i < 2; ++i) {
      feat[i] = fbase + wf * 32 + i * 16 + kq * 4;
#pragma unroll
      for (int j = 0; j < NJ; ++j) { ax[i][j] = acc[i][j]; ag[i][j] = acc[i + 2][j]; }
    }
    epilogue_tile<EPI, float, 2, NJ>(p, tok, feat, ax, ag, kq);
  } else {
    int feat[4];
#pragma unroll
    for (int i = 0; i < 4; ++i) feat[i] = fbase + wf * 64 + i * 16 + kq * 4;
    epilogue_tile<EPI, float, 4, NJ>(p, tok, feat, acc, acc, kq);
  }
}

static int gemm_token_tile(int M, int nf, int debug) {
  if (debug & TTV_DBG_GEMM_TILE160) return 160;
  if (debug & TTV_DBG_GEMM_TILE128) return 128;
  const long cost128 = (long)ttv_cdiv(nf * ttv_cdiv(M, 128), 512) * 128, cost160 = (long)ttv_cdiv(nf * ttv_cdiv(M, 160), 512) * 160;
  return cost160 < cost128 ? 160 : 128;
}

template <int EPI>
static int launch(const GemmDev& d, int dtype, bool prenorm, hipStream_t s) {
  if (dtype == TTV_BF16 && d.K == 256 && d.N % 8 == 0 && !((d.debug & TTV_DBG_K256_GENERAL) && !prenorm && EPI != EPI_STORE_PATCH)) {
    const int fo = (EPI == EPI_GEGLU) ? 32 : 64;
    const int n_panels = ttv_cdiv(d.N, fo), n_tiles = ttv_cdiv(d.M, K256_TT);
    const int total = n_panels * n_tiles;
    static const int grid_env = ttv_env_int("TTV_K256_GRID", 0);
    int grid = total < 512 ? total : 512;
    if (grid_env > 0) grid = total < grid_env ? total : grid_env;
    else if (total > 512)
      for (int g = 512; g >= 416; --g)
        if (total % g == 0) { grid = g; break; }
    static const int qkv256_env = ttv_env_int("TTV_QKV256", 1);
    if constexpr (EPI == EPI_QKV_ROPE) {
      const int n_groups = (n_panels + 3) / 4;
      if (qkv256_env && !(d.debug & TTV_DBG_QKV256_OFF) && d.N % 64 == 0 && d.rope_q_end % 64 == 0 && d.rope_k_begin % 64 == 0 && d.rope_k_end % 64 == 0 &&
          !d.row_scale && !d.bias && !d.add_scalar && (uint64_t)d.w_rows * (uint64_t)d.ldw * 2u < (1ull << 32)) {
        if ((qkv256_env >= 2 || (d.debug & TTV_DBG_QKV256_WS)) && n_groups <= 32) {
          const int tgs = ttv_cdiv(d.M, 32), per_xcd = ttv_cdiv(tgs, 8);
          int q = n_groups * ttv_cdiv(per_xcd, 8);
          q = q > 32 ? 32 : q;
          if (prenorm) hipLaunchKernelGGL((k_qkv256ws<true>), dim3(8 * q), dim3(512), 0, s, d, n_panels, n_groups);
          else hipLaunchKernelGGL((k_qkv256ws<false>), dim3(8 * q), dim3(512), 0, s, d, n_panels, n_groups);
          TTV_CHECK_LAUNCH("qkv256ws");
          return TTV_OK;
        }
        if (prenorm) hipLaunchKernelGGL((k_qkv256<true>), dim3(grid), dim3(256), 0, s, d, n_panels, total);
        else hipLaunchKernelGGL((k_qkv256<false>), dim3(grid), dim3(256), 0, s, d, n_panels, total);
        TTV_CHECK_LAUNCH("qkv256");
        return TTV_OK;
      }
    }
    if (prenorm) hipLaunchKernelGGL((k_gemm_k256<EPI, true>), dim3(grid), dim3(256), 0, s, d, n_panels, total);
    else hipLaunchKernelGGL((k_gemm_k256<EPI, false>), dim3(grid), dim3(256), 0, s, d, n_panels, total);
    TTV_CHECK_LAUNCH("gemm_k256");
    return TTV_OK;
  }
  if (prenorm || EPI == EPI_STORE_PATCH) {
    ttv_set_error("gemm: folded pre-norm / patch scatter need the bf16 K=256 kernel");
    return TTV_ERR_UNSUPPORTED;
  }
  if (dtype == TTV_BF16) {
    const int ft = (EPI == EPI_GEGLU) ? 64 : TF;
    const int nf = ttv_cdiv(d.N, ft), nt = ttv_cdiv(d.M, TT), nt160 = ttv_cdiv(d.M, 160);
    const bool t160 = gemm_token_tile(d.M, nf, d.debug) == 160;
    static const bool use_dma = ttv_env_flag("TTV_GEMM_DMA", true);
    const bool dma_ok = use_dma && d.K % BK == 0 && (uint64_t)d.M * (uint64_t)d.ldx * 2u < (1ull << 32) && (uint64_t)d.w_rows * (uint64_t)d.ldw * 2u < (1ull << 32);
    static const int t256_env = ttv_env_int("TTV_GEMM_T256", -1);
    if constexpr (EPI == EPI_STORE || EPI == EPI_QKV_ROPE || EPI == EPI_GEGLU || EPI == EPI_RESID_T || EPI == EPI_RESID_F32) {
      const int fo = (EPI == EPI_GEGLU) ? 128 : T256_F;
      const long tiles256 = (long)ttv_cdiv(d.N, fo) * ttv_cdiv(d.M, T256_T);
      const bool forced = (d.debug & TTV_DBG_GEMM_T256) || t256_env == 1;
      const bool ok256 = dma_ok && d.N % fo == 0 && d.K >= 2 * BK && !(d.debug & TTV_DBG_GEMM_NO_T256) && (forced || tiles256 >= 256);
      if (ok256 && (forced || (t256_env < 0 && T256_DEFAULT))) {
        hipLaunchKernelGGL((k_gemm_bf16_t256<EPI>), dim3((unsigned)tiles256), dim3(512), 0, s, d, ttv_cdiv(d.N, fo));
        TTV_CHECK_LAUNCH("gemm_t256");
        return TTV_OK;
      }
    }
    if (t160) {
      if (dma_ok) hipLaunchKernelGGL((k_gemm_bf16_dma<EPI, 5>), dim3(nf * nt160), dim3(256), 0, s, d, nf);
      else hipLaunchKernelGGL((k_gemm_bf16<EPI, false, 5>), dim3(nf * nt160), dim3(256), 0, s, d, nf);
    } else {
      if (dma_ok) hipLaunchKernelGGL((k_gemm_bf16_dma<EPI, 4>), dim3(nf * nt), dim3(256), 0, s, d, nf);
      else hipLaunchKernelGGL((k_gemm_bf16<EPI>), dim3(nf * nt), dim3(256), 0, s, d, nf);
    }
  } else {
    if ((uint64_t)d.M * (uint64_t)d.ldx >= (1ull << 31) || (uint64_t)d.w_rows * (uint64_t)d.ldw >= (1ull << 31)) {
      ttv_set_error("gemm (fp32): operand too large for 32-bit element offsets");
      return TTV_ERR_UNSUPPORTED;
    }
    const int nf = ttv_cdiv(d.N, (EPI == EPI_GEGLU) ? 64 : F_TF), nt = ttv_cdiv(d.M, F_TT), nt160 = ttv_cdiv(d.M, 160);
    const bool t160 = gemm_token_tile(d.M, nf, d.debug) == 160;
    static const bool s3dma_env = ttv_env_flag("TTV_SPLIT3_DMA", true);
    const bool s3dma = d.split3 && d.x_image && s3dma_env && !(d.debug & TTV_DBG_SPLIT3_NO_DMA) && d.K % 32 == 0 && d.ldx % 4 == 0 && d.ldw % 4 == 0 &&
                       (uint64_t)d.M * (uint64_t)d.ldx * 4u < (1ull << 32) && (uint64_t)d.w_rows * (uint64_t)d.ldw * 4u < (1ull << 32);
    if (s3dma) {
      if (t160) hipLaunchKernelGGL((k_gemm_split_dma<EPI, 5>), dim3(nf * nt160), dim3(256), 0, s, d, nf);
      else hipLaunchKernelGGL((k_gemm_split_dma<EPI, 4>), dim3(nf * nt), dim3(256), 0, s, d, nf);
    } else if (d.split3) {
      if (t160) hipLaunchKernelGGL((k_gemm_f32<EPI, true, 5>), dim3(nf * nt160), dim3(256), 0, s, d, nf);
      else hipLaunchKernelGGL((k_gemm_f32<EPI, true, 4>), dim3(nf * nt), dim3(256), 0, s, d, nf);
    } else if (s3dma_env && !(d.debug & TTV_DBG_SPLIT3_NO_DMA) && d.K % 32 == 0 && d.ldx % 4 == 0 && d.ldw % 4 == 0 &&
               (uint64_t)d.M * (uint64_t)d.ldx * 4u < (1ull << 32) && (uint64_t)d.w_rows * (uint64_t)d.ldw * 4u < (1ull << 32)) {
// ... 36 lines not shown
  const int ft = (epi == EPI_GEGLU) ? 64 : TF;
  const int nf = ttv_cdiv(d.N, ft), nt = ttv_cdiv(d.M, TT), nt160 = ttv_cdiv(d.M, 160);
  const bool t160 = gemm_token_tile(d.M, nf, 0) == 160;
  const int kc = epi == EPI_STORE ? TTV_KC_GEMM_STORE : epi == EPI_QKV_ROPE ? TTV_KC_GEMM_QKV : epi == EPI_GEGLU ? TTV_KC_GEMM_GEGLU : TTV_KC_GEMM_RESID;
  TtvProfScope prof(kc, s);
#define F8_LAUNCH(E_, MX_)                                                                                         \
  do {                                                                                                              \
    if (t160) hipLaunchKernelGGL((k_gemm_fp8_dma<E_, 5, MX_>), dim3(nf * nt160), dim3(256), 0, s, d, nf);           \
    else hipLaunchKernelGGL((k_gemm_fp8_dma<E_, 4, MX_>), dim3(nf * nt), dim3(256), 0, s, d, nf);                   \
  } while (0)
  if (mx) {
    if (epi == EPI_STORE) F8_LAUNCH(EPI_STORE, true); else if (epi == EPI_QKV_ROPE) F8_LAUNCH(EPI_QKV_ROPE, true);
    else if (epi == EPI_GEGLU) F8_LAUNCH(EPI_GEGLU, true); else F8_LAUNCH(EPI_RESID_T, true);
  } else {
    if (epi == EPI_STORE) F8_LAUNCH(EPI_STORE, false); else if (epi == EPI_QKV_ROPE) F8_LAUNCH(EPI_QKV_ROPE, false); else F8_LAUNCH(EPI_GEGLU, false);
  }
#undef F8_LAUNCH
  TTV_CHECK_LAUNCH("gemm_fp8");
  return TTV_OK;
}

bool ttvk_gemm_supports_resid_norm(int dtype, int N, int K) { return dtype == TTV_BF16 && N == 256 && K % 8 == 0; }

int ttvk_gemm(GemmEpilogue epi, const GemmArgs& a, hipStream_t s) {
  if (a.M == 0 || a.N == 0) return TTV_OK;
  const int esz = dtype_bytes(a.dtype);
  const int vec = 16 / esz;
  TTV_CHECK_ARG(a.dtype == TTV_BF16 || a.dtype == TTV_F32, "gemm: bad dtype %d", a.dtype);
  TTV_CHECK_ARG(a.K > 0 && a.K % vec == 0, "gemm: K=%d must be a multiple of %d", a.K, vec);
  TTV_CHECK_ARG(a.N % 4 == 0, "gemm: N=%d must be a multiple of 4", a.N);
  TTV_CHECK_ARG(a.ldx % vec == 0 && a.ldw % vec == 0 && a.ldy % vec == 0, "gemm: leading dims must keep 16-byte row alignment");
  TTV_CHECK_ARG(((uintptr_t)a.x % 16 == 0) && ((uintptr_t)a.w % 16 == 0) && ((uintptr_t)a.y % 16 == 0), "gemm: pointers must be 16-byte aligned");
  GemmDev d;
  d.x = a.x; d.w = a.w; d.y = a.y; d.bias = a.bias; d.add_scalar = a.add_scalar; d.resid = a.resid; d.rope_cs = a.rope_cs; d.rope_ids = a.rope_ids; d.rope_base = a.rope_base;
  d.ldx = a.ldx; d.ldw = a.ldw; d.ldy = a.ldy; d.ldr = a.ldr;
  d.M = a.M; d.N = a.N; d.K = a.K; d.alpha = a.alpha;
  d.w_rows = (epi == EPI_GEGLU) ? 2 * a.N : a.N;
  d.rope_q_end = a.rope_q_end; d.rope_k_begin = a.rope_k_begin; d.rope_k_end = a.rope_k_end;
  d.eps = a.eps;
  d.debug = g_ttv_debug;
  d.sum_f32 = a.sum_f32; d.ld_sum = a.ld_sum; d.y2 = a.y2; d.ldy2 = a.ldy2; d.norm_gain2 = a.norm_gain2;
  d.split3 = (a.split3 && a.dtype == TTV_F32) ? 1 : 0;
  d.x_image = d.split3 && a.x_image; d.y_image = d.split3 ? a.y_image : 0;
  TTV_CHECK_ARG(!d.y_image || (d.y_image == 1 && (epi == EPI_STORE || epi == EPI_GEGLU)) || (d.y_image == 2 && epi == EPI_QKV_ROPE),
                "gemm: a split-image output is a STORE / GEGLU option (y_image 1) or the to_qkv layout (y_image 2)");
  d.x_mx = d.w_mx = nullptr; d.ld_mx = 0;
  d.norm_gain = a.norm_gain;
  d.clip_desc = a.clip_desc; d.patch_rows = a.patch_rows; d.row_seq = a.row_seq; d.clip0 = 0; d.pt_shift = d.ph_shift = 0;
  d.x_rows = a.x_rows;
  d.x_scale = nullptr; d.w_scale = nullptr;
  d.row_scale = a.row_scale;
  d.stamps = g_ttv_stamps;
  d.resid_rows = a.resid_rows;
  TTV_CHECK_ARG(!a.row_scale || ((a.dtype == TTV_BF16 || a.split3) && (epi == EPI_STORE || epi == EPI_QKV_ROPE || epi == EPI_GEGLU)),
                "gemm: row_scale is a STORE / QKV_ROPE / GEGLU option of the bf16 and the split-bf16 kernels");
  TTV_CHECK_ARG(!a.x_rows || (a.dtype == TTV_BF16 && a.K == 256 && a.N % 8 == 0 && epi != EPI_RESID_NORM), "gemm: x_rows needs the bf16 K=256 kernel");
  if (epi == EPI_STORE_PATCH || a.gather) {
    auto lg2 = [](int v) { int s = 0; while ((1 << s) < v) ++s; return (1 << s) == v ? s : -1; };
    TTV_CHECK_ARG(a.dtype == TTV_BF16 && (a.gather || a.K == 256) && a.patch_w == 8 && lg2(a.patch_t) >= 0 && lg2(a.patch_h) >= 0,
                  "gemm: patch gather/scatter needs bf16, patch_w == 8 and power-of-two patch_t / patch_h (scatter: K == 256)");
    TTV_CHECK_ARG(!a.gather || (epi == EPI_STORE && a.K % 64 == 0 && a.K != 256), "gemm: patch gather is an EPI_STORE option of the general-K kernel");
    TTV_CHECK_ARG(a.clips && a.n_clips > 0 && a.n_clips <= TTV_MAX_CLIPS_PER_LAUNCH && a.clip_desc && a.patch_rows && a.row_seq,
                  "gemm: patch scatter needs clips (<= %d), clip_desc, patch_rows and row_seq", TTV_MAX_CLIPS_PER_LAUNCH);
    for (int i = 0; i < a.n_clips; ++i) d.clips.p[i] = a.clips[i];
    d.pt_shift = lg2(a.patch_t); d.ph_shift = lg2(a.patch_h);
  }
  const bool pn = a.prenorm != 0;
  const int kc = (epi == EPI_STORE || epi == EPI_STORE_PATCH) ? TTV_KC_GEMM_STORE : epi == EPI_QKV_ROPE ? TTV_KC_GEMM_QKV : epi == EPI_GEGLU ? TTV_KC_GEMM_GEGLU : TTV_KC_GEMM_RESID;
  TtvProfScope prof(kc, s);
  switch (epi) {
    case EPI_STORE:
      if (a.gather) {
        const int nf = ttv_cdiv(d.N, TF), nt = ttv_cdiv(d.M, TT), nt160 = ttv_cdiv(d.M, 160);
        if (gemm_token_tile(d.M, nf, d.debug) == 160)
          hipLaunchKernelGGL((k_gemm_bf16<EPI_STORE, true, 5>), dim3(nf * nt160), dim3(256), 0, s, d, nf);
        else
          hipLaunchKernelGGL((k_gemm_bf16<EPI_STORE, true>), dim3(nf * nt), dim3(256), 0, s, d, nf);
        TTV_CHECK_LAUNCH("gemm_gather");
        return TTV_OK;
      }
      return launch<EPI_STORE>(d, a.dtype, pn, s);
    case EPI_STORE_PATCH: return launch<EPI_STORE_PATCH>(d, a.dtype, pn, s);
    case EPI_QKV_ROPE:
      TTV_CHECK_ARG(a.rope_cs && a.rope_q_end % 128 == 0 && a.rope_k_begin % 128 == 0 && a.rope_k_end % 128 == 0, "gemm: rotary ranges must be multiples of 128 columns");
      return launch<EPI_QKV_ROPE>(d, a.dtype, pn, s);
    case EPI_GEGLU: return launch<EPI_GEGLU>(d, a.dtype, pn, s);
    case EPI_RESID_T:
      TTV_CHECK_ARG(a.resid && a.ldr % 4 == 0, "gemm: residual missing");
      return launch<EPI_RESID_T>(d, a.dtype, pn, s);
    case EPI_RESID_F32:
      TTV_CHECK_ARG(a.resid && a.ldr % 4 == 0, "gemm: residual missing");
      return launch<EPI_RESID_F32>(d, a.dtype, pn, s);
    case EPI_BIAS_PLAIN:
    case EPI_BIAS_GELU:
    case EPI_BIAS_RESID_F32R: {
      TTV_CHECK_ARG(a.dtype == TTV_BF16 && a.K % BK == 0 && a.bias && (uintptr_t)a.bias % 8 == 0, "gemm: V-JEPA epilogues need bf16, K %% 64 == 0 and a bias");
      TTV_CHECK_ARG(!a.add_scalar && !a.row_scale, "gemm: V-JEPA epilogues take no scalar / row scale");
      TTV_CHECK_ARG(epi != EPI_BIAS_RESID_F32R || (a.resid && a.ldr % 4 == 0 && (uintptr_t)a.resid % 16 == 0 && a.resid_rows >= 0),
                    "gemm: fp32 residual missing or unaligned");
      TTV_CHECK_ARG((uint64_t)a.M * (uint64_t)a.ldx * 2u < (1ull << 32) && (uint64_t)a.N * (uint64_t)a.ldw * 2u < (1ull << 32),
                    "gemm: operand too large for 32-bit byte offsets");
      if (d.N % T256_F == 0 && d.K >= 2 * BK) {
        const int nf = d.N / T256_F, nt = ttv_cdiv(d.M, T256_T);
        if (epi == EPI_BIAS_PLAIN) hipLaunchKernelGGL((k_gemm_bf16_t256<EPI_BIAS_PLAIN>), dim3(nf * nt), dim3(512), 0, s, d, nf);
        else if (epi == EPI_BIAS_GELU) hipLaunchKernelGGL((k_gemm_bf16_t256<EPI_BIAS_GELU>), dim3(nf * nt), dim3(512), 0, s, d, nf);
        else hipLaunchKernelGGL((k_gemm_bf16_t256<EPI_BIAS_RESID_F32R>), dim3(nf * nt), dim3(512), 0, s, d, nf);
// ... 31 lines not shown
```

titok_video_amd/csrc/ttv_kernels.h:

```cpp
#pragma once
#include <hip/hip_runtime.h>
#include <stdint.h>

#include "../../include/titok_hip.h"

int ttvk_rmsnorm(const void* in, int in_dtype, int ld_in, const int* src_rows, void* out, int out_dtype, int ld_out,
                 const int* dst_rows, const float* gain, int rows, int d, float eps, hipStream_t s, float* next_rstd = nullptr,
                 void* mx_q = nullptr, void* mx_s = nullptr,
                 int split_image = 0);
int ttvk_row_rstd(const void* in, int dtype, int ld_in, float* rstd, int rows, int d, float eps, hipStream_t s);
int ttvk_copy_rows(const void* src, int64_t ld_src_bytes, const int* src_rows, void* dst, int64_t ld_dst_bytes, const int* dst_rows, int rows,
                   int row_bytes, hipStream_t s);
int ttvk_fill_const_rows(void* x, int dtype, int ld, const int* rows_map, int rows, int d, const float* mask_token,
                         const float* gain, float eps, hipStream_t s);
int ttvk_dec_embed(const void* codes, int C, const void* w, const void* bias, const float* mask_token, const float* gain,
                   void* x, int dtype, int ld, const int* rows_map, int rows, int d, float eps, hipStream_t s);
int ttvk_fsq_forward(const ttv_fsq_params* p, const void* z, int z_dtype, int rows, void* codes, int codes_dtype, int* indices,
                     float* bounded, hipStream_t s);
int ttvk_fsq_indices_to_codes(const ttv_fsq_params* p, const int* indices, int rows, void* codes, int codes_dtype, hipStream_t s);
int ttvk_enc_tail(const void* x, int dtype, int ld, const int* rows_map, int rows, int d, const float* gain, float eps,
                  const void* w, const void* bias, int C, const ttv_fsq_params* fsq, float* z_out, void* codes, int* indices,
                  float* bounded, hipStream_t s);
int ttvk_patch_copy(bool scatter, void* const* clips, const int* clip_desc, int clip0, int n_clips, int pt, int ph, int pw,
                    int C, void* patches, int ld, int dtype, int max_patches, hipStream_t s);
// ... 4 lines not shown

int ttvk_split3_pack(const float* w, int ldw, void* out, int ldo, int rows, int K, hipStream_t s);
int64_t ttvk_mx_scale_ld(int d);
int ttvk_quant_mx_fp8(const void* in, int in_dtype, int ld_in, void* out, int ld_out, void* mx, float* row_scales, int rows, int d, hipStream_t s);

int ttvk_clip_from_u8(const void* frames, long long n_pix, void* clip, int dtype, hipStream_t s);

int ttvk_clip_resample_u8(void* const* src, void* const* dst, const int32_t* geom, int n_clips, int dtype, hipStream_t s);

enum GemmEpilogue {
  EPI_STORE = 0,
  EPI_QKV_ROPE,
  EPI_GEGLU,
  EPI_RESID_T,
  EPI_RESID_F32,
  EPI_RESID_NORM,
  EPI_STORE_PATCH,
  EPI_BIAS_PLAIN,
  EPI_BIAS_GELU,
  EPI_BIAS_RESID_F32R,
};

struct GemmArgs {
  const void* x; int ldx;
  const void* w; int ldw;
  int M, N, K;
  void* y; int ldy;
  const void* bias;
  const float* add_scalar;
  const void* resid; int ldr;
  float alpha;
  const float* rope_cs;
  const int* rope_ids; const float* rope_base;
  int rope_q_end, rope_k_begin, rope_k_end;
  int dtype;
  const float* norm_gain;
  float* sum_f32; int ld_sum;
  void* y2; int ldy2; const float* norm_gain2;
  void* yq; void* yq_mx;
  int split3;
  int x_image, y_image;
  int prenorm;
  const float* row_scale;
  const int* x_rows;
  float eps;
  int gather;
  void* const* clips;
  int n_clips;
  const int* clip_desc;
  const int* patch_rows;
  const int* row_seq;
  int patch_t, patch_h, patch_w;
  int resid_rows;
};
struct ClipPtrs { void* p[TTV_MAX_CLIPS_PER_LAUNCH]; };
int ttvk_gemm(GemmEpilogue epi, const GemmArgs& a, hipStream_t s);
int ttvk_gemm_fp8(GemmEpilogue epi, const GemmArgs& a, const float* x_scale, const float* w_scale, hipStream_t s, const void* x_mx = nullptr,
                  const void* w_mx = nullptr);
bool ttvk_gemm_supports_resid_norm(int dtype, int N, int K);

int ttvk_attention(const void* qkvg, int ld, void* out, int ldo, const int* cu_seqlens, const int* qblocks, int n_qblocks,
                   int q_heads, int kv_heads, int head_dim, int flags, int dtype, hipStream_t s, float* lse_out = nullptr,
                   void* out_raw = nullptr);

int ttvk_attention_swp(const void* qkvg, int ld, void* out, int ldo, const int* cu_seqlens, const int* qblocks, int n_qblocks,
                       int q_heads, int kv_heads, int gate_mul, hipStream_t s);
int ttvk_attention_mxout(const void* qkvg, int ld, void* out_q, void* out_mx, int ld_mx, const int* cu_seqlens, const int* qblocks,
                         int n_qblocks, int q_heads, int kv_heads, hipStream_t s);

int ttvk_attention64(const void* qkvg, int ld, void* out, int ldo, const int* cu_seqlens, const int* items, int n_items, int q_heads,
                     int kv_heads, int flags, hipStream_t s);

int ttvk_vq_norms(const void* cb, int dtype, int ld, int N, int C, float* cnorm, hipStream_t s);
int64_t ttvk_vq_workspace_bytes(int rows);
int ttvk_vq_l2_argmin(const void* z, int dtype, int ldz, const void* cb, int ldc, const float* cnorm, int rows, int N, int C, int* indices,
                      float* best_dist, void* workspace, int64_t workspace_bytes, hipStream_t s);
int ttvk_vq_lookup(const void* cb, int dtype, int ldc, const int* indices, int rows, int C, void* codes, int ldo, hipStream_t s);
int ttvk_vq_lookup_bwd(const void* dcodes, int dtype, int ld, const int* indices, int rows, int C, float* dcb, int ldc, hipStream_t s);

int64_t ttvk_vq_train_workspace_bytes(int rows, int N);
int ttvk_vq_commit_forward(const void* z, int dtype, int ldz, const void* cb, int ldc, const int* idx, int rows, int N, int C, float* loss,
                           void* workspace, int64_t workspace_bytes, hipStream_t s);
int ttvk_vq_commit_backward(const void* g, int ldg, const void* z, int ldz, const void* e, int lde, int dtype, int rows, int C, double scale,
                            void* dz, int ldd, hipStream_t s);
int ttvk_vq_ema_stats(const void* z, int dtype, int ldz, const int* idx, int rows, int N, int C, const float* cluster_size, float dead_threshold,
                      uint64_t seed, const int64_t* ema_step, int rank, int world_size, float* stats, void* workspace, int64_t workspace_bytes,
                      hipStream_t s);
int ttvk_vq_ema_update(const float* stats, float* cluster_size, float* embed_avg, float* codebook, void* copy, int copy_dtype, float* cnorm,
                       int64_t* ema_step, int N, int C, float decay, float one_minus_decay, float eps, float dead_threshold, void* workspace,
                       int64_t workspace_bytes, hipStream_t s);

bool ttvk_mlp_fused_supported(int dtype, int width, int inner);
struct MlpNextQkv {
  void* qkv; int ld;
  const float* rope_cs;
  int rows;
  int rope_q_end, rope_k_begin, rope_k_end;
};
int64_t ttvk_mlp_pack_bytes(int inner, int next_qkv_rows);
int ttvk_mlp_pack(const void* w12_folded, const void* w3, const void* wo, const void* next_qkv_folded, int next_qkv_rows, int inner,
                  void* packed, hipStream_t s);
int ttvk_mlp_fused(const void* ao, int ldao, const float* front_gain, float front_alpha, const void* x, int ldx, const void* packed,
                   int inner, void* y, int ldy, const float* post_gain, float alpha, float eps, int M, const MlpNextQkv* nq, hipStream_t s);

int ttvk_l1_loss(void* const* recon, void* const* target, void* const* grad, const int* sizes, int n_clips, int total_clips, int dtype,
                 float* loss, hipStream_t s);
int ttvk_sq_err(void* const* recon, void* const* target, const int* sizes, int n_clips, int dtype, int clamp, double* acc2, hipStream_t s);
int ttvk_rmsnorm_bwd_chain(const void* x, int ldx, const void* dy, int lddy, const float* gain1, float* dgain1, float* dx, int lddx,
                           const void* y, int y_dt, int ldy, const float* gain2, float* dgain2, float out_scale, void* cast_out, int ldc, int rows,
                           int d, float eps, int dt, hipStream_t s);
int ttvk_rmsnorm_bwd(const void* x, int x_dt, int ldx, const int* xr, const void* dy, int dy_dt, int lddy, const int* dyr,
                     const float* gain, void* dx, int dx_dt, int lddx, const int* dxr, int acc, float* dgain, int rows, int d, float eps,
                     hipStream_t s);
int ttvk_colsum(const void* a, int dt, int lda, const int* rows_map, int rows, int n, float* out, hipStream_t s);
int ttvk_sumall(const void* a, int dt, int lda, const int* rows_map, int rows, int n, const float* colw, float scale, float* out, hipStream_t s);
int ttvk_gate_fwd(const void* a, int lda, const void* gate, int ldg, void* ag, int ldo, int rows, int d, int dt, hipStream_t s);
int ttvk_gate_bwd(const void* dag, int ldd, const void* a, int lda, const void* gate, int ldg, void* da, int ldda, void* dgate, int lddg,
                  int rows, int d, int dt, float* delta, hipStream_t s);
int ttvk_geglu_fwd(const void* u, int ldu, void* h, int ldh, int rows, int I, int dt, hipStream_t s);
// ... 119 lines not shown
```

titok_video_amd/csrc/ttv_qkv256.inc:

```
#ifdef QKV_STAMPS
#define QK_STAMP_DECL unsigned long long qst_prev__ = 0, qst_acc__[8] = {0, 0, 0, 0, 0, 0, 0, 0}
#define QK_STAMP_START()                                                                                     \
  do {                                                                                                       \
    __builtin_amdgcn_sched_barrier(0);                                                                       \
    asm volatile("s_memtime %0\n\ts_waitcnt lgkmcnt(0)" : "=s"(qst_prev__)::"memory");                       \
    __builtin_amdgcn_sched_barrier(0);                                                                       \
  } while (0)
#define QK_STAMP(seg_)                                                                                       \
  do {                                                                                                       \
    unsigned long long t__;                                                                                  \
    __builtin_amdgcn_sched_barrier(0);                                                                       \
    asm volatile("s_memtime %0\n\ts_waitcnt lgkmcnt(0)" : "=s"(t__)::"memory");                              \
    __builtin_amdgcn_sched_barrier(0);                                                                       \
    qst_acc__[seg_] += t__ - qst_prev__;                                                                     \
    qst_prev__ = t__;                                                                                        \
  } while (0)
#else
#define QK_STAMP_DECL
#define QK_STAMP_START()
#define QK_STAMP(seg_)
#endif
typedef unsigned qk_u32x4 __attribute__((ext_vector_type(4)));
typedef unsigned qk_u32x2 __attribute__((ext_vector_type(2)));
template <bool PRENORM>
// ... 125 lines not shown
      }                                                                                                      \
      __builtin_amdgcn_sched_barrier(0);                                                                     \
      if (ks__ + 1 < 16) {                                                                                   \
        af__[(ks__ + 1) & 1][0] = QK_AFRAG(buf_, 0, ks__ + 1);                                               \
        af__[(ks__ + 1) & 1][1] = QK_AFRAG(buf_, 1, ks__ + 1);                                               \
      }                                                                                                      \
      cur_[0] = __builtin_amdgcn_mfma_f32_32x32x16_bf16(af__[ks__ & 1][0], bfr[ks__], ks__ ? cur_[0] : zero16, 0, 0, 0); \
      cur_[1] = __builtin_amdgcn_mfma_f32_32x32x16_bf16(af__[ks__ & 1][1], bfr[ks__], ks__ ? cur_[1] : zero16, 0, 0, 0); \
      if (MODE_) {                                                                                           \
        if ((ks__ & 1) == 0) QK_ROT(prev_, MODE_ == 2, ks__ >> 1); else QK_PACK(ks__ >> 1);                  \
      } else if (PRENORM) {                                                                                  \
        const bf16x8 v__ = bfr[ks__];                                                                        \
        ss0__ = __builtin_amdgcn_fdot2_f32_bf16((bf16x2){v__[0], v__[1]}, (bf16x2){v__[0], v__[1]}, ss0__, false); \
        ss1__ = __builtin_amdgcn_fdot2_f32_bf16((bf16x2){v__[2], v__[3]}, (bf16x2){v__[2], v__[3]}, ss1__, false); \
        ss0__ = __builtin_amdgcn_fdot2_f32_bf16((bf16x2){v__[4], v__[5]}, (bf16x2){v__[4], v__[5]}, ss0__, false); \
        ss1__ = __builtin_amdgcn_fdot2_f32_bf16((bf16x2){v__[6], v__[7]}, (bf16x2){v__[6], v__[7]}, ss1__, false); \
        asm volatile("" : "+v"(ss0__), "+v"(ss1__));                                                         \
      }                                                                                                      \
      if (ks__ + 1 < 16) __builtin_amdgcn_sched_group_barrier(0x100, 2, 0);                                  \
      __builtin_amdgcn_sched_group_barrier(0x008, 1, 0);                                                     \
      if (MODE_) { if ((ks__ & 1) || MODE_ != 2) __builtin_amdgcn_sched_group_barrier(0x002, 2, 0); else __builtin_amdgcn_sched_group_barrier(0x002, 4, 0); } \
      else if (PRENORM) __builtin_amdgcn_sched_group_barrier(0x002, 2, 0);                                   \
      __builtin_amdgcn_sched_group_barrier(0x008, 1, 0);                                                     \
      if (MODE_) { if ((ks__ & 1) || MODE_ != 2) __builtin_amdgcn_sched_group_barrier(0x002, 2, 0); else __builtin_amdgcn_sched_group_barrier(0x002, 4, 0); } \
      else if (PRENORM) __builtin_amdgcn_sched_group_barrier(0x002, 2, 0);                                   \
      __builtin_amdgcn_sched_barrier(0);                                                                     \
      if (MODE_ && (ks__ & 3) == 3) {                                                                        \
        QK_STORE_CHUNK(ks__ >> 2, pend_panel);                                                               \
        __builtin_amdgcn_sched_barrier(0);                                                                   \
      }                                                                                                      \
    }                                                                                                        \
    if (MODE_ == 0) {                                                                                        \
      if (PRENORM) {                                                                                         \
        float ss__ = ss0__ + ss1__;                                                                          \
        ss__ = pair32_sum(ss__);                                                                    \
        rstd = 1.0f / sqrtf(ss__ * (1.0f / 256.0f) + p.eps);                                                 \
      }                                                                                                      \
      _Pragma("unroll") for (int t__ = 0; t__ < 2; ++t__)                                                    \
        _Pragma("unroll") for (int g__ = 0; g__ < 4; ++g__)                                                  \
          _Pragma("unroll") for (int e__ = 0; e__ < 2; ++e__)                                                \
            rcs[t__][g__][e__] = make_float2(rcs[t__][g__][e__].x * rstd, rcs[t__][g__][e__].y * rstd);      \
    }                                                                                                        \
  } while (0)

#define QK_STEP(cur_, prev_, it_)                                                                            \
  do {                                                                                                       \
    const int it__ = (it_);                                                                                  \
    const int buf__ = (it__ - it0) & 1;                                                                      \
    const int tile__ = it__ / n_panels, panel__ = it__ - tile__ * n_panels;                                  \
    if (tile__ != cur_tile) {                                                                                \
      cur_tile = tile__;                                                                                     \
       \
                                                                               \
      const int t0__ = tile__ * K256_TT + wave * 32;                                                         \
      int ntk__ = t0__ + r;                                                                                  \
      const bool nok__ = ntk__ < p.M;                                                                        \
      ntk__ = nok__ ? ntk__ : p.M - 1;                                                                       \
      const bf16_t* xr__ = X + (size_t)(p.x_rows ? p.x_rows[ntk__] : ntk__) * p.ldx + h * 8;                 \
      _Pragma("unroll") for (int ks__ = 0; ks__ < 16; ++ks__) bfr[ks__] = *reinterpret_cast<const bf16x8*>(xr__ + ks__ * 16); \
      uint2 nidp__ = make_uint2(0u, 0u);                                                                     \
      if (p.rope_ids) nidp__ = *reinterpret_cast<const uint2*>(p.rope_ids + 2 * (size_t)ntk__);              \
      if (pend == 2) QK_EPILOGUE(prev_, true, pend_panel); else if (pend == 1) QK_EPILOGUE(prev_, false, pend_panel); \
      pend = 0;                                                                                              \
       \
       \
       \
      _Pragma("unroll") for (int ks__ = 0; ks__ < 16; ++ks__) asm volatile("" : "+v"(bfr[ks__]));            \
      tk = ntk__; tok_ok = nok__; idp = nidp__;                                                              \
      wave_full = t0__ + 32 <= p.M;                                                                          \
      ytok = reinterpret_cast<char*>((bf16_t*)p.y + (size_t)tk * p.ldy) + h * 16;                            \
      rstd = 1.f;                                                                                            \
    }                                                                                                        \
    QK_STAMP(0);                                                                                             \
    if (it__ == it0) {                                                                                       \
      asm volatile("s_waitcnt vmcnt(0)" ::: "memory");                                                       \
      __syncthreads();                                                                                       \
    }                                                                                                        \
    QK_STAMP(1);                                                                                             \
    const bool has_next__ = it__ + 1 < it1;                                                                  \
    const char* nsrc__ = QK_PANEL_SRC((it__ + 1) % n_panels);                                                \
    const uint32_t ndst__ = QK_PANEL_DST(buf__ ^ 1);                                                         \
    const int f_first__ = panel__ * 64;                                                                      \
    const int rot__ = (f_first__ < p.rope_q_end || (f_first__ >= p.rope_k_begin && f_first__ < p.rope_k_end)) ? 2 : 1; \
    bool counted__ = false;                                                                                  \
    if (pend == 2) {                                                                                         \
      if (buf__) QK_BODY(cur_, prev_, 1, 2); else QK_BODY(cur_, prev_, 0, 2);                                \
      counted__ = wave_full && !(p.debug & TTV_DBG_NO_STORES);                                                               \
      QK_STAMP(2);                                                                                           \
    } else if (pend == 1) {                                                                                  \
      if (buf__) QK_BODY(cur_, prev_, 1, 1); else QK_BODY(cur_, prev_, 0, 1);                                \
      counted__ = wave_full && !(p.debug & TTV_DBG_NO_STORES);                                                               \
      QK_STAMP(2);                                                                                           \
    } else {                                                                                                 \
      if (buf__) QK_BODY(cur_, prev_, 1, 0); else QK_BODY(cur_, prev_, 0, 0);                                \
      QK_STAMP(3);                                                                                           \
    }                                                                                                        \
     \
    if (counted__) asm volatile("s_waitcnt vmcnt(3)" ::: "memory");                                          \
    else asm volatile("s_waitcnt vmcnt(0)" ::: "memory");                                                    \
    QK_STAMP(4);                                                                                             \
    __builtin_amdgcn_s_barrier();                                                                            \
    QK_STAMP(5);                                                                                             \
    pend = rot__;                                                                                            \
    pend_panel = panel__;                                                                                    \
  } while (0)

  f32x16 accA[2], accB[2];
// ... 39 lines not shown
```

titok_video_amd/model/base/blocks.py:

```python
from __future__ import annotations

import ctypes as C
import math
from typing import List, Optional, Sequence

import torch
import torch.nn as nn

from ... import _lib, switches
from ...plan import BatchPlan, get_plan, host_ints
from .utils import LinearWeight, RMSNormWeight, geglu_inner_dim, get_model_dims


class _AttnParams(nn.Module):

    def __init__(self, dim: int, heads: Sequence[int]):
        super().__init__()
        q_heads, kv_heads = heads
        gqa = (dim // q_heads) * kv_heads
        self.pre_ln = RMSNormWeight(dim)
        self.to_qkv = LinearWeight(dim, 2 * gqa + 2 * dim, bias=False)
        self.out_proj = LinearWeight(dim, dim, bias=False)


# ... 345 lines not shown
                wq = folded_tensor(next_attn.to_qkv.weight, next_attn.pre_ln.weight, q_rows=tower.width)
                rows = int(wq.shape[0])
            inner = int(w3.shape[1])
            out = torch.empty(_lib.lib().ttv_mlp_pack_bytes(inner, rows), dtype=torch.uint8, device=device)
            _lib.check(_lib.lib().ttv_mlp_pack(w12f.data_ptr(), w3c.data_ptr(), woc.data_ptr(), wq.data_ptr() if wq is not None else None,
                                               rows, inner, tower.width, _lib.TTV_BF16, out.data_ptr(), _lib.stream_ptr(device)),
                       "mlp_pack")
            keep.extend([w12f, w3c, woc, wq, out])
            return out.data_ptr(), rows

        perm = tower._patch_perm_on(device)
        if tower.kind == _lib.TTV_ENCODER:
            w_in = tower.proj_in.weight.detach().to(device)[:, perm]
            b_out, w_out = tower.proj_out.bias, tower.proj_out.weight
        else:
            w_in = tower.proj_in.weight
            w_out = tower.proj_out.weight.detach().to(device)[perm, :]
            b_out = tower.proj_out.bias.detach().to(device)[perm]
        ml = tower.model_layers
        n = tower.num_layers
        self.layers = (_lib.LayerWeights * n)()
        for i in range(n):
            a, f = ml.attn_layer[i], ml.ffd_layer[i]
            pack_ptr, pack_rows = mlp_packed(f.w12.weight, f.norm.weight, f.w3.weight, a.out_proj.weight,
                                             ml.attn_layer[i + 1] if i + 1 < n else None)
            if use_mx:
                qkv8, qkv8s, qkvmx = f8_mx(a.to_qkv.weight, a.pre_ln.weight, q_rows=tower.width)
                w128, w128s, w12mx = f8_mx(f.w12.weight, f.norm.weight)
                wo8, wo8s, womx = f8_mx(a.out_proj.weight)
                w38, w38s, w3mx = f8_mx(f.w3.weight)
            else:
                qkv8, qkv8s = f8_rows(a.to_qkv.weight, q_rows=tower.width)
                w128, w128s = f8_rows(f.w12.weight)
                qkvmx = w12mx = wo8 = wo8s = womx = w38 = w38s = w3mx = None
            self.layers[i] = _lib.LayerWeights(
                to_qkv_f8=qkv8, to_qkv_f8_scale=qkv8s, w12_f8=w128, w12_f8_scale=w128s,
                to_qkv_mx=qkvmx, w12_mx=w12mx, out_proj_f8=wo8, out_proj_f8_scale=wo8s, out_proj_mx=womx,
                w3_f8=w38, w3_f8_scale=w38s, w3_mx=w3mx,
                pre_ln=gain(a.pre_ln.weight), to_qkv=lin(a.to_qkv.weight, True), out_proj=lin(a.out_proj.weight, True),
                ffd_norm=gain(f.norm.weight), w12=lin(f.w12.weight, True), w3=lin(f.w3.weight, True),
                attn_post_ln=gain(ml.attn_post_ln[i - 1].weight) if i > 0 else None,
                ffd_post_ln=gain(ml.ffd_post_ln[i - 1].weight) if i > 0 else None,
                to_qkv_pn=folded(a.to_qkv.weight, a.pre_ln.weight, q_rows=tower.width), w12_pn=folded(f.w12.weight, f.norm.weight),
                mlp_pack=pack_ptr, mlp_pack_qkv_rows=pack_rows, qkv_q_prescaled=self.q_prescaled, to_qkv_qs=lin_qs(a.to_qkv.weight))
        self.struct = _lib.TowerWeights(
            proj_in_w=lin(w_in, tower.kind == _lib.TTV_ENCODER), proj_in_b=lin(tower.proj_in.bias), mask_token=gain(tower.mask_token),
            ln_pre_t=gain(tower.ln_pre_t.weight), ln_pre_p=gain(tower.ln_pre_p.weight), ln_post=gain(tower.ln_post.weight),
            proj_out_w=lin(w_out, tower.kind == _lib.TTV_DECODER), proj_out_b=lin(b_out), layers=self.layers,
            f32_split3=1 if self.f32_split3 else 0,
            proj_out_pn=folded(w_out, tower.ln_post.weight) if (tower.kind == _lib.TTV_DECODER and fold) else None)
        self.keep = keep
        self.kind, self.n_layers = tower.kind, n
        self._t = None
        if self.device.type == "cuda":
            self.build_stream = torch.cuda.current_stream(self.device)
            self.ready = torch.cuda.Event()
            self.ready.record(self.build_stream)

    def use_on_current_stream(self) -> None:
        if self.ready is None:
            return
        cur = torch.cuda.current_stream(self.device)
        if cur != self.build_stream and cur.cuda_stream not in self.reader_streams:
            cur.wait_event(self.ready)
        self.reader_streams[cur.cuda_stream] = cur

    def transposed(self) -> "_lib.TowerWeightsT":
        if self._t is None:
            lt = self.lin_tensors
            arr = (_lib.LayerWeightsT * self.n_layers)()
            keep = []

            def tr(t):
                u = t.t().contiguous()
                keep.append(u)
                return u.data_ptr()
            for i in range(self.n_layers):
                q, o, w12, w3 = lt[4 * i: 4 * i + 4]
                arr[i] = _lib.LayerWeightsT(to_qkv_t=tr(q), out_proj_t=tr(o), w12_t=tr(w12), w3_t=tr(w3))
            proj_in_w, proj_out_w = lt[4 * self.n_layers], lt[4 * self.n_layers + 2]
            st = _lib.TowerWeightsT(proj_in_t=tr(proj_in_w) if self.kind == _lib.TTV_ENCODER else None,
                                    proj_out_t=tr(proj_out_w) if self.kind == _lib.TTV_DECODER else None, layers=arr)
            self._t = (st, arr, keep)
        return self._t[0]


class TiTokEncoder(_Tower):
    kind = _lib.TTV_ENCODER

    def __init__(self, model_size="tiny", patch_size=(4, 8, 8), in_channels=3, out_channels=5):
        super().__init__()
        mlp_ratio = self._setup(model_size, patch_size, in_channels, out_channels)
        self.in_channels = in_channels
        scale = self.width ** -0.5
        self.proj_in = LinearWeight(in_channels * math.prod(self.patch), self.width)
        self.mask_token = nn.Parameter(scale * torch.randn(1, 1))
        self.ln_pre_t = RMSNormWeight(self.width)
        self.ln_pre_p = RMSNormWeight(self.width)
        self.model_layers = ResidualAttentionBlock(self.width, self.heads, mlp_ratio, self.num_layers)
        self.ln_post = RMSNormWeight(self.width)
        self.proj_out = LinearWeight(self.width, self.token_size, bias=True)

    def run(self, videos: Sequence[torch.Tensor], token_counts, grids=None, fsq_params=None, want_z=True,
            want_bounded=False):
        v0 = videos[0]
        _lib.require_gpu(v0, "TiTokEncoder")
        device, dtype = v0.device, v0.dtype
        code = _lib.dtype_code(dtype)
        counts = host_ints(token_counts)
        pix = [tuple(v.shape[1:]) for v in videos] if grids is None else host_ints(grids)
        for v, g in zip(videos, pix):
            if v.dtype != dtype or v.device != device or tuple(v.shape[1:]) != tuple(g) or v.shape[0] != self.pix_channels:
                raise ValueError("clips must share dtype/device, be [C,T,H,W] and match `grids`")
        plan = self._plan(pix, counts, device)
        dims = self._dims(code)
        pack = self._packed(dtype, device)
        ws = self._workspace(dims, plan, device)
        clips = [v if v.is_contiguous() else v.contiguous() for v in videos]
# ... 15 lines not shown

    def forward_z(self, videos, token_counts, grids=None) -> torch.Tensor:
        if self._wants_grad(*videos):
            counts = host_ints(token_counts)
            pix = [tuple(v.shape[1:]) for v in videos] if grids is None else [tuple(int(x) for x in g) for g in host_ints(grids)]
            return _EncoderTrainFn.apply(self, counts, pix, len(videos), *videos, *self._param_list())
        return self.run(videos, token_counts, grids, None, want_z=True)["z"]

    def forward(self, videos, token_counts, grids=None):
        return self.forward_z(videos, token_counts, grids).to(videos[0].dtype)


class TiTokDecoder(_Tower):
    kind = _lib.TTV_DECODER

    def __init__(self, model_size="tiny", patch_size=(4, 8, 8), in_channels=5, out_channels=3):
        super().__init__()
        mlp_ratio = self._setup(model_size, patch_size, out_channels, in_channels)
        self.out_channels = out_channels
        scale = self.width ** -0.5
        self.proj_in = LinearWeight(self.token_size, self.width, bias=True)
        self.mask_token = nn.Parameter(scale * torch.randn(1, 1))
        self.ln_pre_t = RMSNormWeight(self.width)
        self.ln_pre_p = RMSNormWeight(self.width)
        self.model_layers = ResidualAttentionBlock(self.width, self.heads, mlp_ratio, self.num_layers)
        self.ln_post = RMSNormWeight(self.width)
        self.proj_out = LinearWeight(self.width, out_channels * math.prod(self.patch))

    def forward(self, tokens: torch.Tensor, token_counts, grids):
        _lib.require_gpu(tokens, "TiTokDecoder")
        if self._wants_grad(tokens):
            counts = host_ints(token_counts)
            pix = [tuple(int(v) for v in g) for g in host_ints(grids)]
            outs = _DecoderTrainFn.apply(self, counts, pix, tokens, *self._param_list())
            return list(outs)
        device, dtype = tokens.device, tokens.dtype
        code = _lib.dtype_code(dtype)
        counts = host_ints(token_counts)
        pix = [tuple(int(v) for v in g) for g in host_ints(grids)]
        plan = self._plan(pix, counts, device)
        if tokens.shape != (plan.sum_tokens, self.token_size):
            raise ValueError(f"tokens must be [{plan.sum_tokens}, {self.token_size}], got {tuple(tokens.shape)}")
        dims = self._dims(code)
        pack = self._packed(dtype, device)
        ws = self._workspace(dims, plan, device)
        tokens = tokens.contiguous()
        sizes = [self.out_channels * t * h * w for (t, h, w) in pix]
        flat = torch.empty(sum(sizes), dtype=dtype, device=device)
        outs, off = [], 0
        for (t, h, w), n in zip(pix, sizes):
            outs.append(flat[off:off + n].view(self.out_channels, t, h, w))
            off += n
        batch = plan.batch_for(self.heads[0], self.heads[1])
        rc = _lib.lib().ttv_decoder_forward(C.byref(dims), C.byref(pack.struct), C.byref(batch), tokens.data_ptr(),
                                            _lib.ptr_array(outs), ws.data_ptr(), ws.numel(), _lib.stream_ptr(device))
        _lib.check(rc, "ttv_decoder_forward")
        return outs


def _train_ctx(tower: _Tower, pix, counts, device, dtype):
    if getattr(tower, "f32_split3", False):
        raise RuntimeError("f32_split3 (split-bf16 arithmetic) is an inference mode: the training towers run plain bf16 / fp32")
    plan = tower._plan(pix, counts, device)
    dims = tower._dims(_lib.dtype_code(dtype))
    batch = plan.batch_for(tower.heads[0], tower.heads[1])
    pack = tower._packed(dtype, device)
    lib = _lib.lib()
    tape = torch.empty(int(lib.ttv_tower_tape_bytes(C.byref(dims), C.byref(batch))), dtype=torch.uint8, device=device)
    return plan, dims, batch, pack, tape


class _EncoderTrainFn(torch.autograd.Function):
    @staticmethod
    def forward(ctx, tower, counts, pix, n_clips, *tensors):
        clips = [c.contiguous() for c in tensors[:n_clips]]
        device, dtype = clips[0].device, clips[0].dtype
        plan, dims, batch, pack, tape = _train_ctx(tower, pix, counts, device, dtype)
        z = torch.empty((plan.sum_tokens, tower.token_size), dtype=torch.float32, device=device)
        rc = _lib.lib().ttv_encoder_forward_train(C.byref(dims), C.byref(pack.struct), C.byref(batch), _lib.ptr_array(clips),
                                                  z.data_ptr(), tape.data_ptr(), tape.numel(), _lib.stream_ptr(device))
        _lib.check(rc, "ttv_encoder_forward_train")
        ctx.tower, ctx.plan, ctx.dims, ctx.batch, ctx.pack, ctx.tape = tower, plan, dims, batch, pack, tape
        ctx.clips = clips
        ctx.n_clips = n_clips
        ctx.clip_grad = [bool(t.requires_grad) for t in tensors[:n_clips]]
        ctx.params = list(tensors[n_clips:])
        return z

    @staticmethod
    def backward(ctx, dz):
        tower, device = ctx.tower, dz.device
        lib = _lib.lib()
        ws = torch.empty(int(lib.ttv_tower_bwd_workspace_bytes(C.byref(ctx.dims), C.byref(ctx.batch))), dtype=torch.uint8, device=device)
        dclips = None
        if any(ctx.clip_grad):
            dclips = [torch.empty_like(c) for c in ctx.clips]
        frozen = dclips is not None and not any(p.requires_grad for p in ctx.params)
        if not frozen:
            flat, gstruct, _lay = tower._grad_buffers(device)
        rc = lib.ttv_encoder_backward(C.byref(ctx.dims), C.byref(ctx.pack.struct), C.byref(ctx.pack.transposed()), C.byref(ctx.batch),
                                      dz.contiguous().float().data_ptr(), ctx.tape.data_ptr(), None if frozen else C.byref(gstruct),
                                      _lib.ptr_array(dclips) if dclips else None, ws.data_ptr(), ws.numel(), _lib.stream_ptr(device))
        _lib.check(rc, "ttv_encoder_backward")
        by_id = {} if frozen else tower._reduce_and_finish(flat)
        clip_grads = [dclips[i] if (dclips and ctx.clip_grad[i]) else None for i in range(ctx.n_clips)]
        param_grads = [by_id.get(id(p)) if p.requires_grad else None for p in ctx.params]
        ctx.tape = None
        return (None, None, None, None, *clip_grads, *param_grads)
# ... 41 lines not shown
```

titok_video_amd/plan.py:

```python
from __future__ import annotations

import ctypes as C
import functools
import math
from typing import List, Optional, Sequence, Tuple

import numpy as np
import torch

from . import _lib, switches

QBLOCK = 128
ATTN_SLOTS = 1024


@functools.lru_cache(maxsize=8)
def _rope_base_table(head_dim: int, nd: int, n_ids: int, theta: float = 10000.0):
    f = head_dim // (2 * nd)
    inv = torch.pow(theta, torch.linspace(0.0, 1.0, f, dtype=torch.float64)) * torch.pi / 2.0
    ids = torch.arange(n_ids, dtype=torch.float32).to(torch.float64)
    ang = ids.view(-1, 1) * inv.view(1, -1)
    fc = torch.polar(torch.ones(1, dtype=torch.float64), ang)
    return fc.real.to(torch.float32).numpy(), fc.imag.to(torch.float32).numpy()

# ... 246 lines not shown
            units = []
            for b in range(len(self.grids)):
                nq = -(-int(self.token_counts[b]) // QBLOCK)
                for kvh in range(kv_heads):
                    units.append([(b, qb * QBLOCK, kvh * rep + r, 0) for qb in range(nq) for r in range(rep)])
            order = sorted(range(len(units)), key=lambda i: len(units[i]), reverse=True)
            lists, weight = [[] for _ in range(8)], [0] * 8
            for i in order:
                x = min(range(8), key=lambda j: weight[j])
                lists[x].extend(units[i])
                weight[x] += len(units[i])
            depth = max(len(l) for l in lists)
            table = np.full((depth, 8, 4), -1, dtype=np.int32)
            for x, l in enumerate(lists):
                if l:
                    table[: len(l), x, :] = np.asarray(l, dtype=np.int32)
            flat = table.reshape(-1, 4)
            last = int(np.max(np.nonzero(flat[:, 0] >= 0)[0])) + 1
            t = _upload(np.ascontiguousarray(flat[:last]), self.device)
            self._attn[key] = t
        return t

    def attention_table_patch(self, q_heads: int, kv_heads: int) -> Optional[torch.Tensor]:
        key = ("patch", int(q_heads), int(kv_heads))
        if key not in self._attn:
            rep = q_heads // kv_heads
            units, dropped = [], 0
            for b in range(len(self.grids)):
                s = self.cu_seqlens[b + 1] - self.cu_seqlens[b]
                nq = -(-s // QBLOCK)
                first = int(self.token_counts[b]) // QBLOCK
                dropped += first
                for kvh in range(kv_heads):
                    units.append([(b, qb * QBLOCK, kvh * rep + r, 0) for qb in range(first, nq) for r in range(rep)])
            t = None
            if dropped and any(units):
                order = sorted(range(len(units)), key=lambda i: len(units[i]), reverse=True)
                lists, weight = [[] for _ in range(8)], [0] * 8
                for i in order:
                    x = min(range(8), key=lambda j: weight[j])
                    lists[x].extend(units[i])
                    weight[x] += len(units[i])
                depth = max(len(l) for l in lists)
                table = np.full((depth, 8, 4), -1, dtype=np.int32)
                for x, l in enumerate(lists):
                    if l:
                        table[: len(l), x, :] = np.asarray(l, dtype=np.int32)
                flat = table.reshape(-1, 4)
                last = int(np.max(np.nonzero(flat[:, 0] >= 0)[0])) + 1
                t = _upload(np.ascontiguousarray(flat[:last]), self.device)
            self._attn[key] = t
        return self._attn[key]

    def attention_table64(self, q_heads: int, kv_heads: int) -> torch.Tensor:
        key = ("w64", int(q_heads), int(kv_heads))
        t = self._attn.get(key)
        if t is None:
            rep = q_heads // kv_heads
            units = []
            for b in range(len(self.grids)):
                s = self.cu_seqlens[b + 1] - self.cu_seqlens[b]
                n64 = -(-s // 64)
                for kvh in range(kv_heads):
                    items = [(kvh * rep + r) | (q << 8) for q in range(n64) for r in range(rep)]
                    items += [-1] * (-len(items) % 4)
                    units.append([(b, kvh, *items[i:i + 4], self.cu_seqlens[b], s) for i in range(0, len(items), 4)])
            order = sorted(range(len(units)), key=lambda i: len(units[i]), reverse=True)
            lists, weight = [[] for _ in range(8)], [0] * 8
            for i in order:
                x = min(range(8), key=lambda j: weight[j])
                lists[x].extend(units[i])
                weight[x] += len(units[i])
            depth = max(len(l) for l in lists)
            table = np.zeros((depth, 8, 8), dtype=np.int32)
            table[:, :, 0] = -1
            for x, l in enumerate(lists):
                if l:
                    table[: len(l), x, :] = np.asarray(l, dtype=np.int32)
            flat = table.reshape(-1, 8)
            last = int(np.max(np.nonzero(flat[:, 0] >= 0)[0])) + 1
            t = _upload(np.ascontiguousarray(flat[:last]), self.device)
            self._attn[key] = t
        return t

    def batch_for(self, q_heads: int, kv_heads: int) -> "_lib.Batch":
        skey = (int(q_heads), int(kv_heads)) + tuple(switches.text(k) for k in ("TTV_ATTN_SPLIT", "TTV_ATTN_PAIRED", "TTV_ATTN64", "TTV_ATTN_TAIL_DIV"))
        cached = self._batch_structs.get(skey)
        if cached is not None:
            return cached
        t = self.attention_table(q_heads, kv_heads)
        paired = 1 if (q_heads // kv_heads) % 2 == 0 and switches.flag("TTV_ATTN_PAIRED", False) else 0
        all_full = 1 if self._attn_all_full.get(t.data_ptr()) else 0
        t64 = self.attention_table64(q_heads, kv_heads) if (q_heads <= 255 and switches.flag("TTV_ATTN64", False)) else None
        tl = self.attention_table_latent(q_heads, kv_heads) if sum(int(k) for k in self.token_counts) > 0 else None
        tp = self.attention_table_patch(q_heads, kv_heads) if all_full else None
        self._batch_structs[skey] = out = _lib.Batch(n_qblocks=int(t.shape[0]), qblocks=t.data_ptr(), qblocks_paired=paired, qblocks_all_full=all_full,
                          items64=t64.data_ptr() if t64 is not None else None, n_items64=int(t64.shape[0]) if t64 is not None else 0,
                          qblocks_latent=tl.data_ptr() if tl is not None else None, n_qblocks_latent=int(tl.shape[0]) if tl is not None else 0,
                          qblocks_patch=tp.data_ptr() if tp is not None else None, n_qblocks_patch=int(tp.shape[0]) if tp is not None else 0,
                          **self._base_fields)
        return out

    def table(self, i: int, n: int) -> torch.Tensor:
        return self.int_tables[self._offs[i]: self._offs[i] + n]

    @property
    def cu_dev(self):
        return self.table(0, len(self.cu_seqlens))

    @property
    def latent_rows_dev(self):
        return self.table(1, self.sum_tokens)

    @property
    def patch_rows_dev(self):
        return self.table(2, self.sum_patches)

    @property
    def clip_desc_dev(self):
        return self.table(3, 8 * len(self.grids))



_plan_cache = {}
_PLAN_CACHE_MAX = 64


def get_plan(pixel_grids, token_counts, patch, device) -> BatchPlan:
    key = (tuple(tuple(int(v) for v in g) for g in pixel_grids), tuple(int(k) for k in token_counts),
           tuple(int(p) for p in patch), str(torch.device(device)))
    plan = _plan_cache.get(key)
    if plan is None:
        if len(_plan_cache) >= _PLAN_CACHE_MAX:
            _plan_cache.pop(next(iter(_plan_cache))).retire()
        plan = BatchPlan(key[0], key[1], key[2], device)
        _plan_cache[key] = plan
    plan.use_on_current_stream()
    return plan


def host_ints(v) -> List[int]:
    if isinstance(v, torch.Tensor):
        return v.detach().to("cpu").tolist()
    return [x.tolist() if hasattr(x, "tolist") else x for x in v]
```

Baseline: 30660.

## Precompute decoder layer-0 patch-row QKV and attention state once per geometry

In the decoder, the patch rows going into layer 0 are identical mask-token rows, so their QKV projection and the K/V attention contribution do not depend on the input. This change builds those patch-row QKV rows and a partial attention state once per uniform batch geometry and caches them. Per call, layer 0 then projects only the latent rows, using a tile remap in the QKV GEMM, and runs a special attention mode that merges the cached state. It adds a persistent cache, a host sync when the cache is built, and a restriction to uniform-geometry bf16 width-256 decoders.

```diff
diff --git a/include/titok_hip.h b/include/titok_hip.h
--- a/include/titok_hip.h
+++ b/include/titok_hip.h
@@ -219,6 +219,21 @@
 
 int ttv_decoder_forward(const ttv_tower_dims* dims, const ttv_tower_weights* w, const ttv_batch* batch, const void* codes,
                         void* const* clips_out, void* workspace, int64_t workspace_bytes, void* stream);
+
+typedef struct ttv_dec_l0_const {
+  const void* rows;
+  int32_t latent_rows;
+  int32_t patch_rows;
+  const float* state;
+  const int32_t* qblocks;
+  int32_t n_qblocks;
+} ttv_dec_l0_const;
+int64_t ttv_dec_l0_const_bytes(const ttv_tower_dims* dims, int patch_rows);
+int ttv_dec_l0_const_build(const ttv_tower_dims* dims, const ttv_tower_weights* w, const int32_t* iota, const float* rope_cs,
+                           const int32_t* rope_ids, const float* rope_base, int patch_rows, void* block, int64_t block_bytes,
+                           int64_t* state_offset, int64_t* flag_offset, void* stream);
+int ttv_decoder_forward_const(const ttv_tower_dims* dims, const ttv_tower_weights* w, const ttv_batch* batch, const void* codes,
+                              void* const* clips_out, void* workspace, int64_t workspace_bytes, const ttv_dec_l0_const* l0, void* stream);
 
 typedef struct ttv_layer_weights_t {
   const void* to_qkv_t;
@@ -434,7 +449,8 @@
   TTV_DBG_QKV256_WS = 131072,
   TTV_DBG_ENC_ALL_ROWS = 524288,
   TTV_DBG_ATTN_NO_SWP = 1048576,
-  TTV_DBG_DEC_ALL_BLOCKS = 2097152
+  TTV_DBG_DEC_ALL_BLOCKS = 2097152,
+  TTV_DBG_DEC_L0_NO_CONST = 4194304
 };
 int ttv_debug_set(int flags);
 int ttv_debug_stamps(void* device_buffer);
diff --git a/titok_video_amd/_lib.py b/titok_video_amd/_lib.py
--- a/titok_video_amd/_lib.py
+++ b/titok_video_amd/_lib.py
@@ -39,6 +39,7 @@
 DBG_ENC_ALL_ROWS = 524288
 DBG_ATTN_NO_SWP = 1048576
 DBG_DEC_ALL_BLOCKS = 2097152
+DBG_DEC_L0_NO_CONST = 4194304
 
 _HERE = os.path.dirname(os.path.abspath(__file__))
 LIB_PATH = switches.text("TTV_LIB_PATH") or os.path.join(_HERE, "libtitok_hip.so")
@@ -83,6 +84,10 @@
                 ("n_blocks64", i32), ("qblocks_paired", i32), ("qblocks_all_full", i32), ("items64", vp), ("n_items64", i32),
                 ("rope_ids", vp), ("rope_base", vp), ("qblocks_latent", vp), ("n_qblocks_latent", i32), ("qblocks_patch", vp),
                 ("n_qblocks_patch", i32)]
+
+
+class DecL0Const(C.Structure):
+    _fields_ = [("rows", vp), ("latent_rows", i32), ("patch_rows", i32), ("state", vp), ("qblocks", vp), ("n_qblocks", i32)]
 
 
 class LayerWeightsT(C.Structure):
@@ -187,6 +192,10 @@
                                       C.POINTER(FsqParams), vp, vp, vp, vp, vp, i64, vp]),
     "ttv_decoder_forward": (C.c_int, [C.POINTER(TowerDims), C.POINTER(TowerWeights), C.POINTER(Batch), vp, C.POINTER(vp),
                                       vp, i64, vp]),
+    "ttv_dec_l0_const_bytes": (i64, [C.POINTER(TowerDims), C.c_int]),
+    "ttv_dec_l0_const_build": (C.c_int, [C.POINTER(TowerDims), C.POINTER(TowerWeights), vp, vp, vp, vp, C.c_int, vp, i64, C.POINTER(i64), C.POINTER(i64), vp]),
+    "ttv_decoder_forward_const": (C.c_int, [C.POINTER(TowerDims), C.POINTER(TowerWeights), C.POINTER(Batch), vp, C.POINTER(vp),
+                                            vp, i64, C.POINTER(DecL0Const), vp]),
     "ttv_tower_tape_bytes": (i64, [C.POINTER(TowerDims), C.POINTER(Batch)]),
     "ttv_tower_bwd_workspace_bytes": (i64, [C.POINTER(TowerDims), C.POINTER(Batch)]),
     "ttv_encoder_forward_train": (C.c_int, [C.POINTER(TowerDims), C.POINTER(TowerWeights), C.POINTER(Batch), C.POINTER(vp), vp, vp,
diff --git a/titok_video_amd/csrc/ttv_api.hip b/titok_video_amd/csrc/ttv_api.hip
--- a/titok_video_amd/csrc/ttv_api.hip
+++ b/titok_video_amd/csrc/ttv_api.hip
@@ -24,6 +24,7 @@
 bool ttv_sw_keel_f32sum() { static const bool v = ttv_env_flag("TTV_KEEL_F32SUM", false); return v; }
 bool ttv_sw_fused_patch() { static const bool v = ttv_env_flag("TTV_FUSED_PATCH", true); return v; }
 bool ttv_sw_attn_pipe() { static const bool v = ttv_env_flag("TTV_ATTN_PIPE", false); return v; }
+static bool sw_dec_l0_const() { static const bool v = ttv_env_flag("TTV_DEC_L0_CONST", true); return v; }
 float ttv_sw_attn_thr() { static const float v = ttv_env_float("TTV_ATTN_THR", 8.0f); return v; }
 thread_local int g_ttv_debug = 0;
 long long* g_ttv_stamps = nullptr;
@@ -164,7 +165,7 @@
 struct PreNormW { const float* gain; const void *w, *w_pn, *w_f8; const float* w_f8_scale; bool f8; };
 
 static int prenorm_proj(const LayerCtx& c, GemmEpilogue epi, const char* x, int rows, const PreNormW& p, int N, char* y, int y_image,
-                        bool rstd_valid) {
+                        bool rstd_valid, int tile_run = 0, int tile_period = 0) {
   const ttv_tower_dims* d = c.d;
   const TowerWs& ws = c.ws;
   const int dm = d->width, dt = d->dtype;
@@ -186,6 +187,7 @@
   a.row_scale = fold_gen ? ws.rstd : nullptr;
   a.x = fold ? x : ws.xn; a.w = fold ? p.w_pn : p.w;
   if (epi == EPI_QKV_ROPE) { a.rope_ids = c.b->rope_ids; a.rope_base = c.b->rope_ids ? c.b->rope_base : nullptr; }
+  a.tile_run = tile_run; a.tile_period = tile_period;
   return ttvk_gemm(epi, a, c.s);
 }
 
@@ -213,7 +215,22 @@
   return TTV_OK;
 }
 
-static int run_layers(const ttv_tower_dims* d, const ttv_tower_weights* w, const ttv_batch* b, const TowerWs& ws, hipStream_t s) {
+static bool dec_l0_const_ok(const LayerCtx& c, const ttv_tower_weights* w, const ttv_dec_l0_const* l0) {
+  const ttv_tower_dims* d = c.d;
+  const ttv_batch* b = c.b;
+  if (!l0 || !l0->rows || !sw_dec_l0_const() || (g_ttv_debug & TTV_DBG_DEC_L0_NO_CONST)) return false;
+  if (d->kind != TTV_DECODER || d->dtype != TTV_BF16 || d->width != 256 || d->head_dim != 64 || c.split3) return false;
+  const int K = l0->latent_rows, P = l0->patch_rows;
+  if (K <= 0 || P <= 0 || K % 128 || P % 128 || (int64_t)b->n_clips * K != b->sum_tokens || (int64_t)b->n_clips * P != b->sum_patches) return false;
+  const ttv_layer_weights& lw = w->layers[0];
+  if (!lw.to_qkv_pn || !lw.qkv_q_prescaled) return false;
+  if (c.pair || c.pipe || !c.all_full || (b->items64 && b->n_items64 > 0)) return false;
+  return ttvk_gemm_qkv_tiles_supported(d->width, d->kv_heads * d->head_dim, d->width) &&
+         ttvk_attention_takes_swp(TTV_ATTN_GATE | TTV_ATTN_QSCALED | TTV_ATTN_ALLFULL);
+}
+
+static int run_layers(const ttv_tower_dims* d, const ttv_tower_weights* w, const ttv_batch* b, const TowerWs& ws, hipStream_t s,
+                      const ttv_dec_l0_const* l0 = nullptr) {
   const int L = b->total_rows, dm = d->width, g = d->kv_heads * d->head_dim, dt = d->dtype;
   const int split3 = (dt == TTV_F32 && w->f32_split3) ? 1 : 0;
   const bool gen_ok = (dt == TTV_BF16 && dm != 256) || split3;
@@ -231,9 +248,11 @@
   bool compacted = false;
   const LayerCtx ctx = {d, b, ws, s, split3, s3img, gen_ok, b->qblocks_paired ? TTV_ATTN_PAIRED : 0, b->qblocks_all_full ? TTV_ATTN_ALLFULL : 0,
                         ttv_sw_attn_pipe() ? TTV_ATTN_PIPE : 0};
+  const bool l0_const = dec_l0_const_ok(ctx, w, l0);
   for (int i = 0; i < d->layers; ++i) {
     const ttv_layer_weights& lw = w->layers[i];
     const bool last = i == d->layers - 1;
+    const bool l0c = l0_const && i == 0;
     if (dt == TTV_BF16 && dm != 256 && dm % 128 == 0 && d->inner % 128 == 0 && !ttv_sw_keel_f32sum() && lw.to_qkv_f8 && lw.to_qkv_mx && lw.w12_f8 &&
         lw.w12_mx && lw.out_proj_f8 && lw.out_proj_mx && lw.w3_f8 && lw.w3_mx &&
         !(lat_last && last)) {
@@ -247,7 +266,8 @@
     if (!qkv_ready) {
       const void* w_plain = (dt == TTV_BF16 && lw.to_qkv_qs) ? lw.to_qkv_qs : lw.to_qkv;
       const PreNormW qw = {lw.pre_ln, w_plain, lw.to_qkv_pn, lw.to_qkv_f8, lw.to_qkv_f8_scale, f8_qkv};
-      TTV_TRY(prenorm_proj(ctx, EPI_QKV_ROPE, ws.x, L, qw, nq, ws.qkv, s3img ? 2 : 0, rstd_valid));
+      if (l0c) TTV_TRY(prenorm_proj(ctx, EPI_QKV_ROPE, ws.x, L, qw, nq, ws.qkv, 0, rstd_valid, l0->latent_rows / 128, (l0->latent_rows + l0->patch_rows) / 128));
+      else TTV_TRY(prenorm_proj(ctx, EPI_QKV_ROPE, ws.x, L, qw, nq, ws.qkv, s3img ? 2 : 0, rstd_valid));
     }
     const bool q_scaled = dt == TTV_BF16 && (lw.to_qkv_pn ? lw.qkv_q_prescaled != 0 : lw.to_qkv_qs != nullptr);
     rstd_valid = false;
@@ -255,7 +275,12 @@
     const bool lat_now = lat_last && last;
     if (lat_now)
       TTV_TRY(tower_attention(ctx, q_scaled, b->qblocks_latent, b->n_qblocks_latent, ctx.all_full));
-    else if (pat_last && last && dt == TTV_BF16 && !ctx.pipe)
+    else if (l0c) {
+      TtvProfScope prof(TTV_KC_ATTENTION, s);
+      const bool own = l0->qblocks && l0->n_qblocks > 0;
+      TTV_TRY(ttvk_attention_swp(ws.qkv, nq, ws.ao, dm, b->cu_seqlens, own ? l0->qblocks : b->qblocks, own ? l0->n_qblocks : b->n_qblocks, d->q_heads,
+                                 d->kv_heads, 1, s, l0->rows, l0->latent_rows, l0->state));
+    } else if (pat_last && last && dt == TTV_BF16 && !ctx.pipe)
       TTV_TRY(tower_attention(ctx, q_scaled, b->qblocks_patch, b->n_qblocks_patch, ctx.all_full));
     else if (q_scaled && b->items64 && b->n_items64 > 0 && d->head_dim == 64)
       TTV_TRY(ttvk_attention64(ws.qkv, nq, ws.ao, dm, b->cu_seqlens, b->items64, b->n_items64, d->q_heads, d->kv_heads,
@@ -587,8 +612,58 @@
   return TTV_OK;
 }
 
+int64_t ttv_dec_l0_const_bytes(const ttv_tower_dims* d, int patch_rows) {
+  if (!d || patch_rows <= 0 || d->dtype != TTV_BF16 || d->width != 256 || d->head_dim != 64 || d->kv_heads <= 0) {
+    ttv_set_error("dec_l0_const_bytes: bf16 decoders of width 256 and head_dim 64 only");
+    return -1;
+  }
+  if (patch_rows % 128) {
+    ttv_set_error("dec_l0_const_bytes: patch_rows must be a multiple of 128");
+    return -1;
+  }
+  const int64_t nq = 2 * (int64_t)d->width + 2 * (int64_t)d->kv_heads * d->head_dim;
+  return align256(patch_rows * nq * 2) + align256(ttvk_attention_swp_state_floats(patch_rows, d->q_heads) * 4 + 4) + align256((int64_t)patch_rows * d->width * 2);
+}
+
+int ttv_dec_l0_const_build(const ttv_tower_dims* d, const ttv_tower_weights* w, const int32_t* iota, const float* rope_cs, const int32_t* rope_ids,
+                           const float* rope_base, int patch_rows, void* block, int64_t block_bytes, int64_t* state_offset, int64_t* flag_offset,
+                           void* stream) {
+  TTV_CHECK_ARG(d && w && w->layers && iota && rope_cs && block && patch_rows > 0, "dec_l0_const_build: null argument");
+  const int64_t need = ttv_dec_l0_const_bytes(d, patch_rows);
+  if (need < 0) return TTV_ERR_UNSUPPORTED;
+  TTV_CHECK_ARG(d->kind == TTV_DECODER && need <= block_bytes && (uintptr_t)block % 256 == 0, "dec_l0_const_build: not a decoder, or block too small / unaligned");
+  const ttv_layer_weights& lw = w->layers[0];
+  if (!lw.to_qkv_pn || !lw.qkv_q_prescaled) {
+    ttv_set_error("dec_l0_const_build: layer 0 needs the folded, q-pre-scaled to_qkv weight");
+    return TTV_ERR_UNSUPPORTED;
+  }
+  hipStream_t s = (hipStream_t)stream;
+  const int dm = d->width, g = d->kv_heads * d->head_dim, nq = 2 * dm + 2 * g, dt = d->dtype;
+  char* const rows = (char*)block;
+  const int64_t state_floats = ttvk_attention_swp_state_floats(patch_rows, d->q_heads);
+  float* const state = (float*)(rows + align256((int64_t)patch_rows * nq * 2));
+  char* const x = (char*)state + align256(state_floats * 4 + 4);
+  if (state_offset) *state_offset = (char*)state - rows;
+  if (flag_offset) *flag_offset = (char*)(state + state_floats) - rows;
+  TTV_TRY(ttvk_fill_const_rows(x, dt, dm, iota, patch_rows, dm, w->mask_token, w->ln_pre_p, d->eps, s));
+  GemmArgs a = gemm_rope_qk(gemm_args(dt, x, dm, lw.to_qkv_pn, dm, patch_rows, nq, dm, rows, nq), rope_cs, dm, g);
+  a.prenorm = 1; a.eps = d->eps;
+  a.rope_ids = rope_ids; a.rope_base = rope_ids ? rope_base : nullptr;
+  TTV_TRY(ttvk_gemm(EPI_QKV_ROPE, a, s));
+  if (hipMemsetAsync(state + state_floats, 0, 4, s) != hipSuccess) {
+    ttv_set_error("dec_l0_const_build: hipMemsetAsync failed");
+    return TTV_ERR_LAUNCH;
+  }
+  return ttvk_attention_swp_dump(rows, nq, patch_rows, d->q_heads, d->kv_heads, state, s);
+}
+
 int ttv_decoder_forward(const ttv_tower_dims* d, const ttv_tower_weights* w, const ttv_batch* b, const void* codes,
                         void* const* clips_out, void* workspace, int64_t workspace_bytes, void* stream) {
+  return ttv_decoder_forward_const(d, w, b, codes, clips_out, workspace, workspace_bytes, nullptr, stream);
+}
+
+int ttv_decoder_forward_const(const ttv_tower_dims* d, const ttv_tower_weights* w, const ttv_batch* b, const void* codes,
+                              void* const* clips_out, void* workspace, int64_t workspace_bytes, const ttv_dec_l0_const* l0, void* stream) {
   TTV_TRY(check_dims(d, b));
   TTV_CHECK_ARG(d->kind == TTV_DECODER, "decoder_forward: dims.kind is not TTV_DECODER");
   TTV_CHECK_ARG(w && w->layers && codes && clips_out && workspace, "decoder_forward: null argument");
@@ -600,7 +675,7 @@
   TTV_TRY(ttvk_dec_embed(codes, d->token_size, w->proj_in_w, w->proj_in_b, w->mask_token, w->ln_pre_t, ws.x, dt, dm, b->latent_rows, b->sum_tokens, dm, d->eps, s));
   TTV_TRY(ttvk_fill_const_rows(ws.x, dt, dm, b->patch_rows, P, dm, w->mask_token, w->ln_pre_p, d->eps, s));
 
-  TTV_TRY(run_layers(d, w, b, ws, s));
+  TTV_TRY(run_layers(d, w, b, ws, s, l0));
 
   GemmArgs a = gemm_args(dt, nullptr, dm, w->proj_out_w, dm, P, pd, dm, ws.pa, pd);
   a.split3 = (dt == TTV_F32 && w->f32_split3) ? 1 : 0;
diff --git a/titok_video_amd/csrc/ttv_attn.hip b/titok_video_amd/csrc/ttv_attn.hip
--- a/titok_video_amd/csrc/ttv_attn.hip
+++ b/titok_video_amd/csrc/ttv_attn.hip
@@ -1369,6 +1369,12 @@
   return TTV_OK;
 }
 
+bool ttvk_attention_takes_swp(int flags) {
+  static const bool swp_env = ttv_env_flag("TTV_ATTN_SWP", true);
+  return swp_env && !(flags & TTV_ATTN_PIPE) && (flags & TTV_ATTN_ALLFULL) && (flags & TTV_ATTN_QSCALED) && !(flags & TTV_ATTN_PAIRED) &&
+         !(g_ttv_debug & TTV_DBG_ATTN_NO_SWP);
+}
+
 int ttvk_attention(const void* qkvg, int ld, void* out, int ldo, const int* cu_seqlens, const int* qblocks, int n_qblocks,
                    int q_heads, int kv_heads, int head_dim, int flags, int dtype, hipStream_t s, float* lse_out, void* out_raw) {
   const int gate_mul = flags & 1, paired = (flags >> 1) & 1, prescaled = (flags >> 2) & 1;
@@ -1398,8 +1404,7 @@
   } while (0)
     const bool tape = lse_out != nullptr || out_raw != nullptr;
     TTV_CHECK_ARG(!tape || !prescaled, "attention: the training-tape outputs need unscaled q");
-    static const bool swp_env = ttv_env_flag("TTV_ATTN_SWP", true);
-    if (swp_env && !(flags & TTV_ATTN_PIPE) && (flags & TTV_ATTN_ALLFULL) && prescaled && !paired && !tape && !(g_ttv_debug & TTV_DBG_ATTN_NO_SWP)) {
+    if (ttvk_attention_takes_swp(flags) && !tape) {
       return ttvk_attention_swp(qkvg, ld, out, ldo, cu_seqlens, qblocks, n_qblocks, q_heads, kv_heads, gate_mul, s);
     }
     if ((flags & TTV_ATTN_PIPE) && (flags & TTV_ATTN_ALLFULL) && prescaled && !paired && !tape) {
diff --git a/titok_video_amd/csrc/ttv_attn_swp.hip b/titok_video_amd/csrc/ttv_attn_swp.hip
--- a/titok_video_amd/csrc/ttv_attn_swp.hip
+++ b/titok_video_amd/csrc/ttv_attn_swp.hip
@@ -37,12 +37,13 @@
 #define SWP_STAMP(seg_)
 #endif
 
-template <bool GATE>
-__global__ __launch_bounds__(256, SWP_OCC) void k_attn_swp(const bf16_t* __restrict__ qkvg, int ld, bf16_t* __restrict__ out, int ldo,
-                                                     const int* __restrict__ cu, const int* __restrict__ qblocks, int d_model, int gqa,
-                                                     int rep, long long* __restrict__ stamps) {
-  __shared__ __attribute__((aligned(16))) uint4 kl[SWP_NS][SWP_KB * 8];
-  __shared__ __attribute__((aligned(16))) uint4 vl[SWP_NS][SWP_KB * 8];
+#define SWP_STATE (33 * 256)
+template <bool GATE, int MODE>
+__device__ __forceinline__ void swp_body(const bf16_t* __restrict__ qkvg, int ld, bf16_t* __restrict__ out, int ldo,
+                                         const int* __restrict__ cu, const int* __restrict__ qblocks, int d_model, int gqa,
+                                         int rep, long long* __restrict__ stamps, const bf16_t* __restrict__ rows2, int kwin,
+                                         float* state, uint4 (*kl)[SWP_KB * 8], uint4 (*vl)[SWP_KB * 8]) {
+  constexpr bool TWO = MODE == 1 || MODE == 3;
 
 #ifdef SWP_STAMPS
   unsigned long long st_entry__;
@@ -52,15 +53,24 @@
   const int wave = __builtin_amdgcn_readfirstlane(tid >> 6);
   const int r = lane & 31, h = lane >> 5;
   const int tix = blockIdx.x;
-  const int seq = qblocks[4 * tix], q0 = qblocks[4 * tix + 1], head = qblocks[4 * tix + 2];
+  const int seq = MODE == 2 ? 0 : qblocks[4 * tix];
+  const int q0 = MODE == 2 ? (tix / (d_model >> 6)) * 128 : qblocks[4 * tix + 1];
+  const int head = MODE == 2 ? tix % (d_model >> 6) : qblocks[4 * tix + 2];
   if (seq < 0) return;
-  const int s0 = cu[seq], S = cu[seq + 1] - s0;
+  const int s0 = MODE == 2 ? 0 : cu[seq], S = MODE == 2 ? kwin : cu[seq + 1] - s0;
+  constexpr bool cached = MODE == 3;
+  int Sk = cached ? kwin : S;
   const int kvh = head / rep;
-  const bf16_t* qbase = qkvg + (size_t)s0 * ld + head * 64;
-  const bf16_t* gbase = qkvg + (size_t)s0 * ld + d_model + head * 64;
-  const bf16_t* kbase = qkvg + (size_t)s0 * ld + 2 * d_model + kvh * 64;
+  const bf16_t* const seq1 = qkvg + (size_t)s0 * ld;
+  const bf16_t* const seq2 = TWO ? rows2 - (ptrdiff_t)kwin * ld : seq1;
+  const bf16_t* const qsrc = (TWO && q0 >= kwin) ? seq2 : seq1;
+  const bf16_t* qbase = qsrc + head * 64;
+  const bf16_t* gbase = qsrc + d_model + head * 64;
+  const bf16_t* kbase = seq1 + 2 * d_model + kvh * 64;
   const bf16_t* vbase = kbase + gqa;
-  const int nkt = (S + SWP_KB - 1) / SWP_KB;
+  const bf16_t* kbase2 = seq2 + 2 * d_model + kvh * 64;
+  const bf16_t* vbase2 = kbase2 + gqa;
+  int nkt = (Sk + SWP_KB - 1) / SWP_KB;
 
   const uint32_t kl_lds = (uint32_t)(uintptr_t)(__attribute__((address_space(3))) void*)&kl[0][0];
   const uint32_t vl_lds = (uint32_t)(uintptr_t)(__attribute__((address_space(3))) void*)&vl[0][0];
@@ -75,27 +85,27 @@
     asm volatile("s_mov_b32 %0, m0\n\ts_mov_b32 m0, %3\n\ts_nop 0\n\tglobal_load_lds_dwordx4 %1, %2\n\ts_mov_b32 m0, %0" \
                  : "=&s"(keep__) : "v"(voff_), "s"(base_), "s"(dst_) : "memory");                                 \
   } while (0)
-#define SWP_DMA_TILE(base_, lds_, kt_, slot_, d_, c_)                                                            \
+#define SWP_DMA_TILE(base_, base2_, lds_, kt_, slot_, d_, c_)                                                    \
   do {                                                                                                           \
     const int key0__ = (kt_) * SWP_KB;                                                                           \
-    if (key0__ >= S) break;                                                                                      \
-    const bf16_t* b__ = (base_) + (size_t)key0__ * ld;                                                           \
+    if (key0__ >= Sk) break;                                                                                     \
+    const bf16_t* b__ = ((TWO && key0__ >= kwin) ? (base2_) : (base_)) + (size_t)key0__ * ld;                    \
     const uint32_t dst__ = (lds_) + (slot_) * (SWP_KB * 128) + wave * 1024;                                      \
-    if (key0__ + SWP_KB <= S) {                                                                                  \
+    if (key0__ + SWP_KB <= Sk) {                                                                                 \
       const bf16_t* b32__ = b__ + (size_t)32 * ld;                                                               \
       unsigned keep__;                                                                                           \
       asm volatile("s_mov_b32 %0, m0\n\ts_mov_b32 m0, %4\n\ts_nop 0\n\tglobal_load_lds_dwordx4 %1, %2\n\t"         \
                    "s_add_u32 m0, %4, 0x1000\n\ts_nop 0\n\tglobal_load_lds_dwordx4 %1, %3\n\ts_mov_b32 m0, %0"      \
                    : "=&s"(keep__) : "v"(d_), "s"(b__), "s"(b32__), "s"(dst__) : "memory", "scc");                   \
     } else {                                                                                                     \
-      const int lim__ = S - 1 - key0__;                                                                          \
+      const int lim__ = Sk - 1 - key0__;                                                                         \
       const int g0__ = drow < lim__ ? drow : lim__, g1__ = drow + 32 < lim__ ? drow + 32 : lim__;                \
       SWP_DMA16((uint32_t)(g0__ * ld + (c_)) * 2u, b__, dst__);                                                  \
       SWP_DMA16((uint32_t)(g1__ * ld + (c_)) * 2u, b__, dst__ + 4096);                                           \
     }                                                                                                            \
   } while (0)
-#define SWP_DMA_K(kt_, slot_) SWP_DMA_TILE(kbase, kl_lds, kt_, slot_, dK, kc)
-#define SWP_DMA_V(kt_, slot_) SWP_DMA_TILE(vbase, vl_lds, kt_, slot_, dV, vc)
+#define SWP_DMA_K(kt_, slot_) SWP_DMA_TILE(kbase, kbase2, kl_lds, kt_, slot_, dK, kc)
+#define SWP_DMA_V(kt_, slot_) SWP_DMA_TILE(vbase, vbase2, vl_lds, kt_, slot_, dV, vc)
 
   SWP_DMA_K(0, 0);
   SWP_DMA_V(0, 0);
@@ -172,13 +182,13 @@
   } while (0)
 #define SWP_MASK(c0_, c1_, kt_)                                                                                  \
   do {                                                                                                           \
-    if ((kt_) == nkt - 1 && nkt * SWP_KB > S) {                                                                  \
+    if ((kt_) == nkt - 1 && nkt * SWP_KB > Sk) {                                                                 \
       int h4__ = 4 * h;                                                                                          \
       asm volatile("" : "+v"(h4__));       \
       _Pragma("unroll") for (int e__ = 0; e__ < 16; ++e__) {                                                     \
         const int key__ = (kt_) * SWP_KB + (e__ & 3) + 8 * (e__ >> 2) + h4__;                                    \
-        if (key__ >= S) c0_[e__] = -INFINITY;                                                                    \
-        if (key__ + 32 >= S) c1_[e__] = -INFINITY;                                                               \
+        if (key__ >= Sk) c0_[e__] = -INFINITY;                                                                   \
+        if (key__ + 32 >= Sk) c1_[e__] = -INFINITY;                                                              \
       }                                                                                                          \
     }                                                                                                            \
   } while (0)
@@ -234,7 +244,7 @@
     SWP_GAPS4(2);                                                                                                \
     SWP_STAMP(2);                                                                                                \
     l_run += sum_a + sum_b;                                                                                      \
-    if (tt__ + 1 == nkt - 1 && nkt * SWP_KB > S) {                                                               \
+    if (tt__ + 1 == nkt - 1 && nkt * SWP_KB > Sk) {                                                              \
       asm volatile("s_nop 7\n\ts_nop 7\n\ts_nop 3" ::: "memory");      \
       SWP_MASK(nxt0_, nxt1_, tt__ + 1);                                                                          \
     }                                                                                                            \
@@ -317,9 +327,35 @@
   st_acc__[5] = st_real1__ - st_real0__;
 #endif
 
+  if constexpr (MODE == 2 || MODE == 3) {
+    const int item = (MODE == 2 ? q0 : q0 - kwin) / 128 * (d_model >> 6) + head;
+    float* const st = state + (size_t)item * SWP_STATE;
+    if (MODE == 2) {
+#pragma unroll
+      for (int j = 0; j < 4; ++j) {
+        *reinterpret_cast<f32x4*>(st + (j * 256 + tid) * 4) = (f32x4){o0[4 * j], o0[4 * j + 1], o0[4 * j + 2], o0[4 * j + 3]};
+        *reinterpret_cast<f32x4*>(st + ((4 + j) * 256 + tid) * 4) = (f32x4){o1[4 * j], o1[4 * j + 1], o1[4 * j + 2], o1[4 * j + 3]};
+      }
+      st[8 * 1024 + tid] = l_run;
+      const float lt = l_run + __shfl_xor(l_run, 32, 64);
+      if (!(lt > 8.6736174e-19f && lt < 1.1529215e18f)) *reinterpret_cast<int*>(state + (size_t)gridDim.x * SWP_STATE) = 1;
+      return;
+    }
+    if (cached) {
+#pragma unroll
+      for (int j = 0; j < 4; ++j) {
+        const f32x4 c0 = *reinterpret_cast<const f32x4*>(st + (j * 256 + tid) * 4);
+        const f32x4 c1 = *reinterpret_cast<const f32x4*>(st + ((4 + j) * 256 + tid) * 4);
+#pragma unroll
+        for (int e = 0; e < 4; ++e) { o0[4 * j + e] += c0[e]; o1[4 * j + e] += c1[e]; }
+      }
+      l_run += st[8 * 1024 + tid];
+    }
+  }
   float l_tot = l_run + __shfl_xor(l_run, 32, 64);
   const bool out_of_range = !(l_tot > 8.6736174e-19f && l_tot < 1.1529215e18f);
   if (__syncthreads_or(out_of_range)) {
+    if constexpr (MODE == 3) { Sk = S; nkt = (S + SWP_KB - 1) / SWP_KB; }
     float m_run = -INFINITY;
     l_run = 0.f;
     o0 = zero16;
@@ -407,16 +443,45 @@
 #endif
 }
 
+template <bool GATE, int MODE>
+__global__ __launch_bounds__(256, SWP_OCC) void k_attn_swp(const bf16_t* __restrict__ qkvg, int ld, bf16_t* __restrict__ out, int ldo,
+                                                     const int* __restrict__ cu, const int* __restrict__ qblocks, int d_model, int gqa,
+                                                     int rep, long long* __restrict__ stamps, const bf16_t* __restrict__ rows2, int kwin,
+                                                     float* state) {
+  __shared__ __attribute__((aligned(16))) uint4 kl[SWP_NS][SWP_KB * 8];
+  __shared__ __attribute__((aligned(16))) uint4 vl[SWP_NS][SWP_KB * 8];
+  if constexpr (MODE == 3) {
+    if (qblocks[4 * blockIdx.x + 1] >= kwin) swp_body<GATE, 3>(qkvg, ld, out, ldo, cu, qblocks, d_model, gqa, rep, stamps, rows2, kwin, state, kl, vl);
+    else swp_body<GATE, 1>(qkvg, ld, out, ldo, cu, qblocks, d_model, gqa, rep, stamps, rows2, kwin, state, kl, vl);
+  } else {
+    swp_body<GATE, MODE>(qkvg, ld, out, ldo, cu, qblocks, d_model, gqa, rep, stamps, rows2, kwin, state, kl, vl);
+  }
+}
+
 int ttvk_attention_swp(const void* qkvg, int ld, void* out, int ldo, const int* cu_seqlens, const int* qblocks, int n_qblocks,
-                       int q_heads, int kv_heads, int gate_mul, hipStream_t s) {
+                       int q_heads, int kv_heads, int gate_mul, hipStream_t s, const void* rows2, int kwin, const float* state) {
   const int d_model = q_heads * 64, gqa = kv_heads * 64, rep = q_heads / kv_heads;
   dim3 grid(n_qblocks);
-  if (gate_mul)
-    hipLaunchKernelGGL((k_attn_swp<true>), grid, dim3(256), 0, s, (const bf16_t*)qkvg, ld, (bf16_t*)out, ldo, cu_seqlens, qblocks, d_model,
-                       gqa, rep, g_ttv_stamps);
-  else
-    hipLaunchKernelGGL((k_attn_swp<false>), grid, dim3(256), 0, s, (const bf16_t*)qkvg, ld, (bf16_t*)out, ldo, cu_seqlens, qblocks, d_model,
-                       gqa, rep, g_ttv_stamps);
+  TTV_CHECK_ARG(!rows2 || (kwin > 0 && kwin % 128 == 0 && (uintptr_t)rows2 % 16 == 0), "attention_swp: the second source starts at a multiple of 128 rows");
+  TTV_CHECK_ARG(!state || (rows2 && (uintptr_t)state % 16 == 0), "attention_swp: the cached state comes with the second source");
+#define SWP_LAUNCH(G_, M_)                                                                                                       \
+  hipLaunchKernelGGL((k_attn_swp<G_, M_>), grid, dim3(256), 0, s, (const bf16_t*)qkvg, ld, (bf16_t*)out, ldo, cu_seqlens, qblocks, d_model, \
+                     gqa, rep, g_ttv_stamps, (const bf16_t*)rows2, kwin, const_cast<float*>(state))
+  if (state) { if (gate_mul) SWP_LAUNCH(true, 3); else SWP_LAUNCH(false, 3); }
+  else if (rows2) { if (gate_mul) SWP_LAUNCH(true, 1); else SWP_LAUNCH(false, 1); }
+  else if (gate_mul) SWP_LAUNCH(true, 0);
+  else SWP_LAUNCH(false, 0);
+#undef SWP_LAUNCH
   TTV_CHECK_LAUNCH("attention_swp");
   return TTV_OK;
 }
+
+int64_t ttvk_attention_swp_state_floats(int n_rows, int q_heads) { return (int64_t)(n_rows / 128) * q_heads * SWP_STATE; }
+int ttvk_attention_swp_dump(const void* rows, int ld, int n_rows, int q_heads, int kv_heads, float* state, hipStream_t s) {
+  TTV_CHECK_ARG(rows && state && n_rows > 0 && n_rows % 128 == 0 && (uintptr_t)state % 16 == 0 && (uintptr_t)rows % 16 == 0, "attention_swp_dump: whole 128-row blocks");
+  const int d_model = q_heads * 64, gqa = kv_heads * 64, rep = q_heads / kv_heads;
+  hipLaunchKernelGGL((k_attn_swp<false, 2>), dim3(n_rows / 128 * q_heads), dim3(256), 0, s, (const bf16_t*)rows, ld, (bf16_t*)nullptr, 0,
+                     (const int*)nullptr, (const int*)nullptr, d_model, gqa, rep, (long long*)nullptr, (const bf16_t*)nullptr, n_rows, state);
+  TTV_CHECK_LAUNCH("attention_swp_dump");
+  return TTV_OK;
+}
diff --git a/titok_video_amd/csrc/ttv_gemm.hip b/titok_video_amd/csrc/ttv_gemm.hip
--- a/titok_video_amd/csrc/ttv_gemm.hip
+++ b/titok_video_amd/csrc/ttv_gemm.hip
@@ -30,6 +30,7 @@
   int clip0, pt_shift, ph_shift;
   long long* stamps;
   int resid_rows;
+  int tile_run, tile_period;
 };
 
 struct PatchDst {
@@ -1845,11 +1846,18 @@
   return cost160 < cost128 ? 160 : 128;
 }
 
+static int sw_qkv256() { static const int v = ttv_env_int("TTV_QKV256", 1); return v; }
+bool ttvk_gemm_qkv_tiles_supported(int d_model, int gqa_dim, int ldw) {
+  const int N = 2 * d_model + 2 * gqa_dim;
+  return sw_qkv256() == 1 && !(g_ttv_debug & (TTV_DBG_QKV256_OFF | TTV_DBG_QKV256_WS)) && N % 64 == 0 && d_model % 64 == 0 && gqa_dim % 64 == 0 &&
+         (uint64_t)N * (uint64_t)ldw * 2u < (1ull << 32);
+}
+
 template <int EPI>
 static int launch(const GemmDev& d, int dtype, bool prenorm, hipStream_t s) {
   if (dtype == TTV_BF16 && d.K == 256 && d.N % 8 == 0 && !((d.debug & TTV_DBG_K256_GENERAL) && !prenorm && EPI != EPI_STORE_PATCH)) {
     const int fo = (EPI == EPI_GEGLU) ? 32 : 64;
-    const int n_panels = ttv_cdiv(d.N, fo), n_tiles = ttv_cdiv(d.M, K256_TT);
+    const int n_panels = ttv_cdiv(d.N, fo), n_tiles = d.tile_period ? d.M / K256_TT / d.tile_period * d.tile_run : ttv_cdiv(d.M, K256_TT);
     const int total = n_panels * n_tiles;
     static const int grid_env = ttv_env_int("TTV_K256_GRID", 0);
     int grid = total < 512 ? total : 512;
@@ -1857,12 +1865,12 @@
     else if (total > 512)
       for (int g = 512; g >= 416; --g)
         if (total % g == 0) { grid = g; break; }
-    static const int qkv256_env = ttv_env_int("TTV_QKV256", 1);
+    const int qkv256_env = sw_qkv256();
     if constexpr (EPI == EPI_QKV_ROPE) {
       const int n_groups = (n_panels + 3) / 4;
       if (qkv256_env && !(d.debug & TTV_DBG_QKV256_OFF) && d.N % 64 == 0 && d.rope_q_end % 64 == 0 && d.rope_k_begin % 64 == 0 && d.rope_k_end % 64 == 0 &&
           !d.row_scale && !d.bias && !d.add_scalar && (uint64_t)d.w_rows * (uint64_t)d.ldw * 2u < (1ull << 32)) {
-        if ((qkv256_env >= 2 || (d.debug & TTV_DBG_QKV256_WS)) && n_groups <= 32) {
+        if ((qkv256_env >= 2 || (d.debug & TTV_DBG_QKV256_WS)) && n_groups <= 32 && !d.tile_period) {
           const int tgs = ttv_cdiv(d.M, 32), per_xcd = ttv_cdiv(tgs, 8);
           int q = n_groups * ttv_cdiv(per_xcd, 8);
           q = q > 32 ? 32 : q;
@@ -1876,6 +1884,10 @@
         TTV_CHECK_LAUNCH("qkv256");
         return TTV_OK;
       }
+    }
+    if (d.tile_period) {
+      ttv_set_error("gemm: a tile list needs k_qkv256 (ttvk_gemm_qkv_tiles_supported)");
+      return TTV_ERR_UNSUPPORTED;
     }
     if (prenorm) hipLaunchKernelGGL((k_gemm_k256<EPI, true>), dim3(grid), dim3(256), 0, s, d, n_panels, total);
     else hipLaunchKernelGGL((k_gemm_k256<EPI, false>), dim3(grid), dim3(256), 0, s, d, n_panels, total);
@@ -2018,6 +2030,12 @@
   d.row_scale = a.row_scale;
   d.stamps = g_ttv_stamps;
   d.resid_rows = a.resid_rows;
+  d.tile_run = d.tile_period = 0;
+  if (a.tile_period) {
+    TTV_CHECK_ARG(epi == EPI_QKV_ROPE && a.dtype == TTV_BF16 && a.K == 256 && a.tile_run > 0 && a.tile_run < a.tile_period &&
+                  a.M % (K256_TT * a.tile_period) == 0, "gemm: a tile list is a to_qkv option of the bf16 K=256 kernel, M a whole number of periods");
+    d.tile_run = a.tile_run; d.tile_period = a.tile_period;
+  }
   TTV_CHECK_ARG(!a.row_scale || ((a.dtype == TTV_BF16 || a.split3) && (epi == EPI_STORE || epi == EPI_QKV_ROPE || epi == EPI_GEGLU)),
                 "gemm: row_scale is a STORE / QKV_ROPE / GEGLU option of the bf16 and the split-bf16 kernels");
   TTV_CHECK_ARG(!a.x_rows || (a.dtype == TTV_BF16 && a.K == 256 && a.N % 8 == 0 && epi != EPI_RESID_NORM), "gemm: x_rows needs the bf16 K=256 kernel");
diff --git a/titok_video_amd/csrc/ttv_kernels.h b/titok_video_amd/csrc/ttv_kernels.h
--- a/titok_video_amd/csrc/ttv_kernels.h
+++ b/titok_video_amd/csrc/ttv_kernels.h
@@ -80,19 +80,25 @@
   const int* row_seq;
   int patch_t, patch_h, patch_w;
   int resid_rows;
+  int tile_run, tile_period;
 };
 struct ClipPtrs { void* p[TTV_MAX_CLIPS_PER_LAUNCH]; };
 int ttvk_gemm(GemmEpilogue epi, const GemmArgs& a, hipStream_t s);
 int ttvk_gemm_fp8(GemmEpilogue epi, const GemmArgs& a, const float* x_scale, const float* w_scale, hipStream_t s, const void* x_mx = nullptr,
                   const void* w_mx = nullptr);
 bool ttvk_gemm_supports_resid_norm(int dtype, int N, int K);
+bool ttvk_gemm_qkv_tiles_supported(int d_model, int gqa_dim, int ldw);
 
 int ttvk_attention(const void* qkvg, int ld, void* out, int ldo, const int* cu_seqlens, const int* qblocks, int n_qblocks,
                    int q_heads, int kv_heads, int head_dim, int flags, int dtype, hipStream_t s, float* lse_out = nullptr,
                    void* out_raw = nullptr);
 
+bool ttvk_attention_takes_swp(int flags);
 int ttvk_attention_swp(const void* qkvg, int ld, void* out, int ldo, const int* cu_seqlens, const int* qblocks, int n_qblocks,
-                       int q_heads, int kv_heads, int gate_mul, hipStream_t s);
+                       int q_heads, int kv_heads, int gate_mul, hipStream_t s, const void* rows2 = nullptr, int kwin = 0,
+                       const float* state = nullptr);
+int64_t ttvk_attention_swp_state_floats(int n_rows, int q_heads);
+int ttvk_attention_swp_dump(const void* rows, int ld, int n_rows, int q_heads, int kv_heads, float* state, hipStream_t s);
 int ttvk_attention_mxout(const void* qkvg, int ld, void* out_q, void* out_mx, int ld_mx, const int* cu_seqlens, const int* qblocks,
                          int n_qblocks, int q_heads, int kv_heads, hipStream_t s);
 
diff --git a/titok_video_amd/csrc/ttv_qkv256.inc b/titok_video_amd/csrc/ttv_qkv256.inc
--- a/titok_video_amd/csrc/ttv_qkv256.inc
+++ b/titok_video_amd/csrc/ttv_qkv256.inc
@@ -201,7 +201,9 @@
       cur_tile = tile__;                                                                                     \
        \
                                                                                \
-      const int t0__ = tile__ * K256_TT + wave * 32;                                                         \
+        \
+      const int ttile__ = p.tile_period ? (tile__ / p.tile_run) * p.tile_period + tile__ % p.tile_run : tile__; \
+      const int t0__ = ttile__ * K256_TT + wave * 32;                                                        \
       int ntk__ = t0__ + r;                                                                                  \
       const bool nok__ = ntk__ < p.M;                                                                        \
       ntk__ = nok__ ? ntk__ : p.M - 1;                                                                       \
diff --git a/titok_video_amd/model/base/blocks.py b/titok_video_amd/model/base/blocks.py
--- a/titok_video_amd/model/base/blocks.py
+++ b/titok_video_amd/model/base/blocks.py
@@ -421,6 +421,7 @@
         self.keep = keep
         self.kind, self.n_layers = tower.kind, n
         self._t = None
+        self._l0_const = {}
         if self.device.type == "cuda":
             self.build_stream = torch.cuda.current_stream(self.device)
             self.ready = torch.cuda.Event()
@@ -433,6 +434,45 @@
         if cur != self.build_stream and cur.cuda_stream not in self.reader_streams:
             cur.wait_event(self.ready)
         self.reader_streams[cur.cuda_stream] = cur
+
+    def dec_l0_const(self, dims: "_lib.TowerDims", plan: BatchPlan) -> Optional["_lib.DecL0Const"]:
+        geo = plan.uniform_geometry()
+        if geo is None or self.kind != _lib.TTV_DECODER or self.device.type != "cuda":
+            return None
+        if geo in self._l0_const:
+            ent = self._l0_const[geo]
+        else:
+            k, p = plan.token_counts[0], plan.grid_sizes[0]
+            need = _lib.lib().ttv_dec_l0_const_bytes(C.byref(dims), p) if (k > 0 and k % 128 == 0 and p % 128 == 0 and self.q_prescaled) else -1
+            ent = None
+            if need > 0:
+                with torch.cuda.stream(self.build_stream):
+                    plan.use_on_current_stream()
+                    block = torch.empty(int(need), dtype=torch.uint8, device=self.device)
+                    iota = torch.arange(p, dtype=torch.int32, device=self.device)
+                    cs, ids, base = plan.clip0_patch_rope()
+                    so, fo = C.c_int64(0), C.c_int64(0)
+                    rc = _lib.lib().ttv_dec_l0_const_build(C.byref(dims), C.byref(self.struct), iota.data_ptr(), cs, ids, base, p,
+                                                           block.data_ptr(), block.numel(), C.byref(so), C.byref(fo), _lib.stream_ptr(self.device))
+                    _lib.check(rc, "ttv_dec_l0_const_build")
+                    out_of_window = int(block[fo.value:fo.value + 4].view(torch.int32).item()) != 0
+                    done = torch.cuda.Event()
+                    done.record(self.build_stream)
+                state = None if out_of_window else block.data_ptr() + so.value
+                ent = dict(rows=block.data_ptr(), latent_rows=k, patch_rows=p, state=state, keep=(block, iota), done=done, seen=set(), structs={})
+            self._l0_const[geo] = ent
+        if ent is None:
+            return None
+        cur = torch.cuda.current_stream(self.device)
+        if cur != self.build_stream and cur.cuda_stream not in ent["seen"]:
+            cur.wait_event(ent["done"])
+            ent["seen"].add(cur.cuda_stream)
+        hit = ent["structs"].get(id(plan))
+        if hit is None:
+            table = plan.attention_table_l0(int(dims.q_heads), int(dims.kv_heads))
+            hit = ent["structs"][id(plan)] = (_lib.DecL0Const(rows=ent["rows"], latent_rows=ent["latent_rows"], patch_rows=ent["patch_rows"],
+                                                              state=ent["state"], qblocks=table.data_ptr(), n_qblocks=int(table.shape[0])), plan)
+        return hit[0]
 
     def transposed(self) -> "_lib.TowerWeightsT":
         if self._t is None:
@@ -554,8 +594,10 @@
             outs.append(flat[off:off + n].view(self.out_channels, t, h, w))
             off += n
         batch = plan.batch_for(self.heads[0], self.heads[1])
-        rc = _lib.lib().ttv_decoder_forward(C.byref(dims), C.byref(pack.struct), C.byref(batch), tokens.data_ptr(),
-                                            _lib.ptr_array(outs), ws.data_ptr(), ws.numel(), _lib.stream_ptr(device))
+        l0 = pack.dec_l0_const(dims, plan)
+        rc = _lib.lib().ttv_decoder_forward_const(C.byref(dims), C.byref(pack.struct), C.byref(batch), tokens.data_ptr(),
+                                                  _lib.ptr_array(outs), ws.data_ptr(), ws.numel(), C.byref(l0) if l0 is not None else None,
+                                                  _lib.stream_ptr(device))
         _lib.check(rc, "ttv_decoder_forward")
         return outs
 
diff --git a/titok_video_amd/plan.py b/titok_video_amd/plan.py
--- a/titok_video_amd/plan.py
+++ b/titok_video_amd/plan.py
@@ -322,6 +322,37 @@
             self._attn[key] = t
         return self._attn[key]
 
+    def attention_table_l0(self, q_heads: int, kv_heads: int) -> torch.Tensor:
+        key = ("l0", int(q_heads), int(kv_heads))
+        t = self._attn.get(key)
+        if t is None:
+            rep = q_heads // kv_heads
+            lat, pat = [], []
+            for b in range(len(self.grids)):
+                s = self.cu_seqlens[b + 1] - self.cu_seqlens[b]
+                nq, first = -(-s // QBLOCK), int(self.token_counts[b]) // QBLOCK
+                for kvh in range(kv_heads):
+                    lat.append([(b, qb * QBLOCK, kvh * rep + r, 0) for qb in range(first) for r in range(rep)])
+                    pat.append([(b, qb * QBLOCK, kvh * rep + r, 0) for qb in range(first, nq) for r in range(rep)])
+            order = sorted(range(len(lat)), key=lambda i: len(lat[i]) + len(pat[i]), reverse=True)
+            first_l, then_l, weight = [[] for _ in range(8)], [[] for _ in range(8)], [0] * 8
+            for i in order:
+                x = min(range(8), key=lambda j: weight[j])
+                first_l[x].extend(lat[i])
+                then_l[x].extend(pat[i])
+                weight[x] += len(lat[i]) + len(pat[i])
+            lists = [a + b for a, b in zip(first_l, then_l)]
+            depth = max(len(l) for l in lists)
+            table = np.full((depth, 8, 4), -1, dtype=np.int32)
+            for x, l in enumerate(lists):
+                if l:
+                    table[: len(l), x, :] = np.asarray(l, dtype=np.int32)
+            flat = table.reshape(-1, 4)
+            last = int(np.max(np.nonzero(flat[:, 0] >= 0)[0])) + 1
+            t = _upload(np.ascontiguousarray(flat[:last]), self.device)
+            self._attn[key] = t
+        return t
+
     def attention_table64(self, q_heads: int, kv_heads: int) -> torch.Tensor:
         key = ("w64", int(q_heads), int(kv_heads))
         t = self._attn.get(key)
@@ -371,6 +402,18 @@
                           **self._base_fields)
         return out
 
+    def uniform_geometry(self) -> Optional[tuple]:
+        g, k = self.grids[0], self.token_counts[0]
+        if any(gb != g for gb in self.grids) or any(kb != k for kb in self.token_counts):
+            return None
+        return (g, k, self.n_rope_ids)
+
+    def clip0_patch_rope(self) -> Tuple[int, Optional[int], Optional[int]]:
+        k = self.token_counts[0]
+        ids = self._base_fields.get("rope_ids")
+        return (self.rope_cs.data_ptr() + 4 * self.rope_cs.shape[1] * k, ids + 8 * k if ids else None,
+                self._base_fields.get("rope_base") if ids else None)
+
     def table(self, i: int, n: int) -> torch.Tensor:
         return self.int_tables[self._offs[i]: self._offs[i] + n]
 
```

Measured after the change: 31740, median of 6. 1.04x the previous value.
